# DEEPDIP-project/IncompressibleNavierStokes.jl

Measured on AMD Instinct MI355X. Metric: M lattice-cell updates/sec (RK4 step incl. Poisson), 3D TGV fp64, higher is better.
Workload: dtype f64; 1 GPU; TaylorGreenVortex3D 256^3 periodic fp64, RK44 + spectral Poisson, dt=0.001, Re=1e3; decomposition=single GPU, loop=timesteps_ (K steps, one native call)

## Files before the change

include/ins_hip.h:

```cpp
#ifndef INS_HIP_H
#define INS_HIP_H

#include <stdint.h>

#ifdef __cplusplus
extern "C" {
#endif

#define INS_OK 0
#define INS_ERR_INVALID (-1)
#define INS_ERR_HIP (-2)
#define INS_ERR_FFT (-3)
#define INS_ERR_UNSUPPORTED (-4)
#define INS_ERR_NOCONV (-5)
#define INS_ERR_COMM (-6)

#define INS_BC_PERIODIC 0
#define INS_BC_DIRICHLET 1
#define INS_BC_SYMMETRIC 2
#define INS_BC_PRESSURE 3
#define INS_BC_HALO 4

typedef struct ins_grid ins_grid_t;
typedef struct ins_poisson ins_poisson_t;
typedef struct ins_rk ins_rk_t;
typedef struct ins_poisson32 ins_poisson32_t;
typedef struct ins_rk32 ins_rk32_t;
typedef struct ins_comm ins_comm_t;

typedef struct ins_grid_desc {
  int32_t D;
  int32_t N[3];
  const double* dx[3];
  const double* dxu[3];
  const double* A1[3][3];
  const double* A2[3][3];
  int32_t iu_lo[3][3];
  int32_t iu_hi[3][3];
  int32_t ip_lo[3];
  int32_t ip_hi[3];
  int32_t bc[3][2];
  double bc_u[3][2][3];
} ins_grid_desc_t;

int ins_version(void);
int ins_fft_reset_count(void);
const char* ins_last_error(void);
int ins_set_option(const char* name, int64_t value);
int ins_get_option(const char* name, int64_t* value);
int ins_option_count(void);
const char* ins_option_name(int i);
int ins_set_device(int device);
int ins_sync(void* stream);

int ins_grid_create(const ins_grid_desc_t* desc, ins_grid_t** out);
int ins_grid_destroy(ins_grid_t* grid);
int ins_grid_is_uniform_exact(const ins_grid_t* grid);

int ins_apply_bc_u_f64(const ins_grid_t* grid, double* u, int dudt, const double* const* planes, void* stream);
int ins_apply_bc_p_f64(const ins_grid_t* grid, double* p, void* stream);

int ins_scalewithvolume_f64(const ins_grid_t* grid, double* p, void* stream);
int ins_divergence_f64(const ins_grid_t* grid, const double* u, double* div, void* stream);
int ins_pressuregradient_f64(const ins_grid_t* grid, const double* p, double* G, void* stream);
int ins_applypressure_f64(const ins_grid_t* grid, double* u, const double* p, void* stream);
int ins_laplacian_f64(const ins_grid_t* grid, const double* p, double* L, void* stream);
int ins_convection_f64(const ins_grid_t* grid, const double* u, double* F, void* stream);
int ins_diffusion_f64(const ins_grid_t* grid, double visc, const double* u, double* F, void* stream);
int ins_convectiondiffusion_f64(const ins_grid_t* grid, double visc, const double* u, double* F, void* stream);
int ins_momentum_f64(const ins_grid_t* grid, double visc, const double* u, double* F, void* stream);
int ins_kinetic_energy_f64(const ins_grid_t* grid, const double* u, double* ke, int interpolate_first, void* stream);
int ins_total_kinetic_energy_f64(const ins_grid_t* grid, const double* u, int interpolate_first, double* out, void* stream);
int ins_cfl_timestep_f64(const ins_grid_t* grid, double Re, const double* u, double* out, void* stream);
int ins_max_abs_divergence_f64(const ins_grid_t* grid, const double* u, double* out, void* stream);

int ins_poisson_spectral_create(const ins_grid_t* grid, ins_poisson_t** out);
int ins_poisson_cg_create(const ins_grid_t* grid, double abstol, double reltol, int64_t maxiter, ins_poisson_t** out);
int ins_poisson_cg_bordered(ins_poisson_t* ps, int enable);
int ins_poisson_cg_set_comm(ins_poisson_t* ps, ins_comm_t* comm);
int ins_poisson_fdm_create(const ins_grid_t* grid, const double* const* V, const double* const* lam, ins_poisson_t** out);
int ins_poisson_destroy(ins_poisson_t* ps);
int ins_poisson_fft_engine(const ins_poisson_t* ps, int32_t* engine);
int ins_poisson_yz_partitions(const ins_poisson_t* ps, int32_t* partitions);
int ins_poisson_solve_f64(ins_poisson_t* ps, double* p, void* stream);
int ins_poisson_last_info(const ins_poisson_t* ps, int64_t* iterations, double* residual);
int ins_project_f64(const ins_grid_t* grid, ins_poisson_t* ps, double* u, double* p, void* stream);

int ins_divergence_adjoint_f64(const ins_grid_t* grid, const double* phi, double* ubar, void* stream);
int ins_pressuregradient_adjoint_f64(const ins_grid_t* grid, const double* phi, double* pbar, void* stream);
int ins_convection_adjoint_f64(const ins_grid_t* grid, const double* u, const double* phibar, double* ubar, void* stream);
int ins_diffusion_adjoint_f64(const ins_grid_t* grid, double visc, const double* phibar, double* ubar, void* stream);
int ins_momentum_pullback_f64(const ins_grid_t* grid, double visc, const double* u, const double* phibar, double* ubar, int accumulate, void* stream);
int ins_apply_bc_u_pullback_f64(const ins_grid_t* grid, double* phibar, void* stream);
int ins_apply_bc_p_pullback_f64(const ins_grid_t* grid, double* phibar, void* stream);
int ins_project_pullback_f64(const ins_grid_t* grid, ins_poisson_t* ps, double* phibar, double* pwork, void* stream);

int ins_filter_face_f64(const ins_grid_t* les, const ins_grid_t* dns, int comp, const double* u, double* v, void* stream);
int ins_filter_volume_f64(const ins_grid_t* les, const ins_grid_t* dns, int comp, const double* u, double* v, void* stream);
int ins_reconstruct_f64(const ins_grid_t* dns, const ins_grid_t* les, int comp, const double* v, double* u, void* stream);
int ins_filter_face_pullback_f64(const ins_grid_t* les, const ins_grid_t* dns, int comp, const double* w, double* ubar, void* stream);
int ins_filter_volume_pullback_f64(const ins_grid_t* les, const ins_grid_t* dns, int comp, const double* w, double* ubar, void* stream);

int ins_rk_create(const ins_grid_t* grid, ins_poisson_t* ps, int nstage, const double* A, const double* c, ins_rk_t** out);
int ins_rk_destroy(ins_rk_t* rk);
int ins_rk_step_f64(ins_rk_t* rk, double visc, double* u, double t, double dt, const double* const* planes, void* stream);
int ins_rk_step_bc_f64(ins_rk_t* rk, double visc, double* u, double t, double dt, const double* const* planes_by_time, void* stream);
int ins_rk_steps_f64(ins_rk_t* rk, double visc, double* u, double t, double dt, int nsteps, void* stream);
int ins_combine_f64(const ins_grid_t* grid, const double* base, double* out, int nterms, const double* coefs,
                    const double* const* ks, void* stream);
int ins_rk_profile_enable(ins_rk_t* rk, int enable);
int ins_rk_profile_read(ins_rk_t* rk, double* momentum_ms, int64_t* momentum_launches);
int ins_rk_set_bodyforce(ins_rk_t* rk, const double* force);

int ins_dbg_stage_rhs_used(const ins_rk_t* rk, int64_t* launches);
int ins_dbg_stage_rhs(ins_rk_t* rk, double visc, const double* u_in, const double* pI, const double* ustart, const double* kterm, double coef_k,
                      double self_in, double coef_self, double* ustar, double* rhs, int32_t* used, void* stream);
int ins_dbg_stage_carry_used(const ins_rk_t* rk, int64_t* launches);
int ins_rk_pressure(const ins_rk_t* rk, double** p);
int ins_rk_stage_force(const ins_rk_t* rk, int i, double** ku);

int ins_vorticity_f64(const ins_grid_t* grid, const double* u, double* w, void* stream);
int ins_interpolate_u_p_f64(const ins_grid_t* grid, const double* u, double* up, void* stream);
int ins_interpolate_w_p_f64(const ins_grid_t* grid, const double* w, double* wp, void* stream);
int ins_dfield_f64(const ins_grid_t* grid, const double* p, double* G, double* d, double eps, void* stream);
int ins_qfield_f64(const ins_grid_t* grid, const double* u, double* Q, void* stream);
int ins_dissipation_from_strain_f64(const ins_grid_t* grid, double visc, const double* u, double* eps_out, void* stream);
int ins_eig2field_f64(const ins_grid_t* grid, const double* u, double* lam, void* stream);
int ins_apply_bc_temp_f64(const ins_grid_t* grid, const int32_t* bc, const double* val, const double* const* planes, double* temp, void* stream);
int ins_convection_diffusion_temp_f64(const ins_grid_t* grid, double a4, const double* u, const double* temp, double* c, void* stream);
int ins_dissipation_f64(const ins_grid_t* grid, double visc, double coef, const double* u, double* diff, double* diss, void* stream);
int ins_gravity_f64(const ins_grid_t* grid, int gdir, double a2, const double* temp, double* F, void* stream);
int ins_smagtensor_f64(const ins_grid_t* grid, double theta, const double* u, double* sigma, void* stream);
int ins_divoftensor_f64(const ins_grid_t* grid, const double* sigma, double* s, void* stream);
int ins_smagorinsky_force_f64(const ins_grid_t* grid, double theta, const double* u, double* sigma, double* s, void* stream);
int ins_smagorinsky_force_needs_sigma(const ins_grid_t* grid);
int ins_tensorbasis_f64(const ins_grid_t* grid, const double* u, double* B, double* V, void* stream);

int ins_tensorbasis_pullback_f64(const ins_grid_t* grid, const double* u, const double* Bbar, const double* Vbar, double* ubar, int accumulate,
                                 void* stream);
int ins_divoftensor_adjoint_f64(const ins_grid_t* grid, const double* sbar, double* sigmabar, void* stream);
int ins_tensorinvariants_f64(const ins_grid_t* grid, const double* u, double* V, void* stream);
int ins_tensorclosure_stress_f64(const ins_grid_t* grid, const double* u, const double* a, double* tau, void* stream);
int ins_tensorclosure_pullback_f64(const ins_grid_t* grid, const double* u, const double* a, const double* taubar, const double* Vbar, double* abar,
                                   double* ubar, int accumulate, void* stream);
int ins_combine_scalar_f64(const ins_grid_t* grid, const double* base, double* out, int nterms, const double* coefs,
                           const double* const* ks, void* stream);

typedef struct ins_temperature_desc {
  double a2;
  double a4;
  double diss_coef;
  int32_t gdir;
  int32_t dodissipation;
  int32_t bc[6];
  double val[6];
} ins_temperature_desc_t;
int ins_rk_set_temperature(ins_rk_t* rk, const ins_temperature_desc_t* desc);
int ins_rk_set_closure(ins_rk_t* rk, int32_t kind, double theta);
int ins_rk_step_ext_f64(ins_rk_t* rk, double visc, double* u, double* temp, double t, double dt, void* stream);

int ins_apply_bc_temp_pullback_f64(const ins_grid_t* grid, const int32_t* bc, double* tempbar, void* stream);
int ins_gravity_adjoint_f64(const ins_grid_t* grid, int gdir, double a2, const double* phibar, double* tempbar, void* stream);
int ins_convection_diffusion_temp_adjoint_f64(const ins_grid_t* grid, double a4, const double* u, const double* temp, const double* cbar,
                                              double* ubar, double* tempbar, void* stream);
int ins_dissipation_adjoint_f64(const ins_grid_t* grid, double visc, double coef, const double* u, const double* cbar, double* ubar, void* stream);
int ins_temperature_pullback_f64(const ins_grid_t* grid, const ins_temperature_desc_t* desc, double visc, const double* u, const double* temp,
                                 const double* Fbar, const double* cbar, double* ubar, double* tempbar, void* stream);

typedef struct ins_spectrum ins_spectrum_t;
int ins_spectrum_create(const ins_grid_t* grid, int nbin, const int64_t* offsets, const int64_t* inds, ins_spectrum_t** out);
int ins_spectrum_create_weighted(const ins_grid_t* grid, int nbin, const int64_t* offsets, const int64_t* inds, const double* weights,
                                 ins_spectrum_t** out);
int ins_spectrum_destroy(ins_spectrum_t* spectrum);
int ins_spectrum_f64(ins_spectrum_t* spectrum, const double* u, double* ehat, void* stream);

typedef struct ins_slab_fft ins_slab_fft_t;
int ins_stage_momentum_f64(const ins_grid_t* grid, double visc, const double* u_in, double* k_out, const double* ustart,
                           double* ustar, int nterms, const double* coefs, const double* const* ks, double coef_self, void* stream);
int ins_stage_momentum_corr_f64(const ins_grid_t* grid, double visc, const double* ustar_prev, const double* p_ext, double* k_out,
                                const double* ustart, double* ustar, int nterms, const double* coefs, const double* const* ks,
                                double coef_self, void* stream);
int ins_stage_momentum_corr_part_f64(const ins_grid_t* grid, double visc, const double* ustar_prev, const double* p_ext, double* k_out,
                                     const double* ustart, double* ustar, int nterms, const double* coefs, const double* const* ks,
                                     double coef_self, double c0m1, double self_in, double* ustart_out, int part, void* stream);
int ins_slab_divergence_f64(const ins_grid_t* grid, const double* u, double* pI, void* stream);
int ins_slab_applypressure_f64(const ins_grid_t* grid, double* u, const double* pI, const double* p_top, void* stream);
int ins_slab_fft_create(const int32_t np[3], const double h[3], int rank, int nranks, ins_slab_fft_t** out);
int ins_slab_fft_destroy(ins_slab_fft_t* fft);
int ins_slab_fft_sizes(const ins_slab_fft_t* fft, int64_t* real_elems, int64_t* complex_elems);
int ins_slab_fft_forward_xy(ins_slab_fft_t* fft, double* pI, double* work, double* sendbuf, void* stream);
int ins_slab_fft_solve_z(ins_slab_fft_t* fft, double* buf, void* stream);
int ins_slab_fft_inverse_xy(ins_slab_fft_t* fft, double* recvbuf, double* work, double* pI, void* stream);

int ins_slab_fft_can_chunk(const ins_slab_fft_t* fft);
int ins_slab_fft_xy_forward_only(ins_slab_fft_t* fft, double* pI, double* work, void* stream);
int ins_slab_fft_pack_chunk(ins_slab_fft_t* fft, double* work, double* sendbuf, int kx0, int kxc, void* stream);
int ins_slab_fft_solve_z_chunk(ins_slab_fft_t* fft, double* buf, int kx0, int kxc, void* stream);
int ins_slab_fft_unpack_chunk(ins_slab_fft_t* fft, double* recvbuf, double* work, int kx0, int kxc, void* stream);
int ins_slab_fft_xy_inverse_only(ins_slab_fft_t* fft, double* work, double* pI, void* stream);
int ins_slab_fft_is_own(const ins_slab_fft_t* fft);
int ins_slab_fft_forward_packed(ins_slab_fft_t* fft, const ins_grid_t* grid, const double* src, int from_u, double* work, double* sendbuf,
                                int cw, void* stream);
int ins_slab_fft_inverse_packed(ins_slab_fft_t* fft, double* recvbuf, double* work, double* pI, int cw, void* stream);

int ins_slab_ztri_edge_elems(const ins_slab_fft_t* S, int64_t* doubles);
int ins_slab_ztri_forward(ins_slab_fft_t* S, const ins_grid_t* grid, const double* src, int from_u, double* work, double* edge, void* stream);
int ins_slab_ztri_finish(ins_slab_fft_t* S, double* work, const double* edges_all, double* pI, void* stream);
int ins_slab_ztri_chunk(const ins_slab_fft_t* S, int c, int nchunks, int64_t* line_lo, int64_t* line_cnt, int64_t* edge_doubles);
int ins_slab_ztri_transform(ins_slab_fft_t* S, const ins_grid_t* grid, const double* src, int from_u, double* work, void* stream);
int ins_slab_ztri_sweep_forward(ins_slab_fft_t* S, double* work, double* edge, int c, int nchunks, void* stream);
int ins_slab_ztri_sweep_backward(ins_slab_fft_t* S, double* work, const double* edges_all, int c, int nchunks, void* stream);
int ins_slab_ztri_inverse(ins_slab_fft_t* S, double* work, double* pI, void* stream);
int ins_slab_xfwd_planes(ins_slab_fft_t* S, const ins_grid_t* grid, const double* u, double* work, int kz0, int nkz, void* stream);

#define INS_COMM_ID_BYTES 128
int ins_comm_unique_id(void* id128);
int ins_comm_create(int nranks, int rank, const void* id128, ins_comm_t** out);
int ins_comm_create_local(int ngpu, const int* devices, ins_comm_t** out);
int ins_comm_group_begin(void);
int ins_comm_group_end(void);
int ins_comm_destroy(ins_comm_t* comm);
int ins_comm_rank(const ins_comm_t* comm, int* rank, int* nranks);
int ins_comm_sendrecv_f64(ins_comm_t* comm, int nsend, const double* const* sendbufs, const int64_t* sendcounts, const int32_t* dsts, int nrecv,
                          double* const* recvbufs, const int64_t* recvcounts, const int32_t* srcs, void* stream);
int ins_halo_exchange_f64(ins_comm_t* comm, const ins_grid_t* slab_grid, double* u, int comp_mask, int down_only, void* stream);
int ins_halo_exchange_scalar_f64(ins_comm_t* comm, const ins_grid_t* slab_grid, double* p, void* stream);
int ins_halo_exchange_p_f64(ins_comm_t* comm, double* p_ext, int64_t plane_elems, int nzl, void* stream);
int ins_ztri_allgather_f64(ins_comm_t* comm, const double* edge, double* edges_all, int64_t count, int direct, void* stream);
int ins_comm_allreduce_f64(ins_comm_t* comm, double* buf, int64_t count, int op, void* stream);
int ins_comm_alltoall_f64(ins_comm_t* comm, const double* send, double* recv, int64_t count, void* stream);

int ins_apply_bc_u_f32(const ins_grid_t* grid, float* u, void* stream);
int ins_apply_bc_p_f32(const ins_grid_t* grid, float* p, void* stream);
int ins_momentum_f32(const ins_grid_t* grid, float visc, const float* u, float* F, void* stream);
int ins_poisson_spectral_create_f32(const ins_grid_t* grid, ins_poisson32_t** out);
int ins_poisson_wrap_f32(const ins_grid_t* grid, ins_poisson_t* ps64, ins_poisson32_t** out);
int ins_poisson_destroy_f32(ins_poisson32_t* ps);
int ins_poisson_solve_f32(ins_poisson32_t* ps, float* p, void* stream);
int ins_project_f32(const ins_grid_t* grid, ins_poisson32_t* ps, float* u, float* p, void* stream);
int ins_rk_create_f32(const ins_grid_t* grid, ins_poisson32_t* ps, int nstage, const double* A, const double* c, ins_rk32_t** out);
int ins_rk_destroy_f32(ins_rk32_t* rk);
int ins_rk_step_f32(ins_rk32_t* rk, float visc, float* u, float dt, void* stream);
int ins_rk_steps_f32(ins_rk32_t* rk, float visc, float* u, float dt, int nsteps, void* stream);
int ins_max_abs_divergence_f32(const ins_grid_t* grid, ins_poisson32_t* ps, const float* u, float* out, void* stream);

int ins_divergence_adjoint_f32(const ins_grid_t* grid, const float* phi, float* ubar, void* stream);
int ins_pressuregradient_adjoint_f32(const ins_grid_t* grid, const float* phi, float* pbar, void* stream);
int ins_momentum_pullback_f32(const ins_grid_t* grid, float visc, const float* u, const float* phibar, float* ubar, int accumulate, void* stream);
int ins_apply_bc_u_pullback_f32(const ins_grid_t* grid, float* phibar, void* stream);
int ins_apply_bc_p_pullback_f32(const ins_grid_t* grid, float* phibar, void* stream);
int ins_project_pullback_f32(const ins_grid_t* grid, ins_poisson32_t* ps, float* phibar, float* pwork, void* stream);

int ins_tensorinvariants_f32(const ins_grid_t* grid, const float* u, float* V, void* stream);
int ins_tensorclosure_stress_f32(const ins_grid_t* grid, const float* u, const float* a, float* tau, void* stream);
int ins_tensorclosure_pullback_f32(const ins_grid_t* grid, const float* u, const float* a, const float* taubar, const float* Vbar, float* abar,
                                   float* ubar, int accumulate, void* stream);
int ins_divoftensor_f32(const ins_grid_t* grid, const float* sigma, float* s, void* stream);
int ins_divoftensor_adjoint_f32(const ins_grid_t* grid, const float* sbar, float* sigmabar, void* stream);

int ins_apply_bc_temp_f32(const ins_grid_t* grid, const int32_t* bc, const float* val, float* temp, void* stream);
int ins_convection_diffusion_temp_f32(const ins_grid_t* grid, float a4, const float* u, const float* temp, float* c, void* stream);
int ins_dissipation_f32(const ins_grid_t* grid, float visc, float coef, const float* u, float* diff, float* diss, void* stream);
int ins_gravity_f32(const ins_grid_t* grid, int gdir, float a2, const float* temp, float* F, void* stream);
int ins_rk_set_temperature_f32(ins_rk32_t* rk, const ins_temperature_desc_t* desc);
int ins_rk_step_ext_f32(ins_rk32_t* rk, float visc, float* u, float* temp, float dt, void* stream);
int ins_rk_steps_ext_f32(ins_rk32_t* rk, float visc, float* u, float* temp, float dt, int nsteps, void* stream);

#ifdef __cplusplus
}
// ... 3 lines not shown
```

incompressiblenavierstokes.jl_amd/_lib.py:

```python
import ctypes as C
import os

_HERE = os.path.dirname(os.path.abspath(__file__))
LIB_PATH = os.environ.get("INS_HIP_LIB") or os.path.join(_HERE, "libinship.so")

INS_BC_PERIODIC, INS_BC_DIRICHLET, INS_BC_SYMMETRIC, INS_BC_PRESSURE, INS_BC_HALO = range(5)

c_double_p = C.POINTER(C.c_double)
vp = C.c_void_p


class GridDesc(C.Structure):

    _fields_ = [
        ("D", C.c_int32),
        ("N", C.c_int32 * 3),
        ("dx", c_double_p * 3),
        ("dxu", c_double_p * 3),
        ("A1", (c_double_p * 3) * 3),
        ("A2", (c_double_p * 3) * 3),
        ("iu_lo", (C.c_int32 * 3) * 3),
        ("iu_hi", (C.c_int32 * 3) * 3),
        ("ip_lo", C.c_int32 * 3),
        ("ip_hi", C.c_int32 * 3),
        ("bc", (C.c_int32 * 2) * 3),
        ("bc_u", ((C.c_double * 3) * 2) * 3),
    ]


SIGNATURES = {
    "ins_version": (C.c_int, []),
    "ins_fft_reset_count": (C.c_int, []),
    "ins_last_error": (C.c_char_p, []),
    "ins_set_option": (C.c_int, [C.c_char_p, C.c_int64]),
    "ins_get_option": (C.c_int, [C.c_char_p, C.POINTER(C.c_int64)]),
    "ins_option_count": (C.c_int, []),
    "ins_option_name": (C.c_char_p, [C.c_int]),
    "ins_set_device": (C.c_int, [C.c_int]),
    "ins_sync": (C.c_int, [vp]),
    "ins_grid_create": (C.c_int, [C.POINTER(GridDesc), C.POINTER(vp)]),
    "ins_grid_destroy": (C.c_int, [vp]),
    "ins_grid_is_uniform_exact": (C.c_int, [vp]),
    "ins_apply_bc_u_f64": (C.c_int, [vp, vp, C.c_int, C.POINTER(vp), vp]),
    "ins_apply_bc_p_f64": (C.c_int, [vp, vp, vp]),
    "ins_scalewithvolume_f64": (C.c_int, [vp, vp, vp]),
    "ins_divergence_f64": (C.c_int, [vp, vp, vp, vp]),
    "ins_pressuregradient_f64": (C.c_int, [vp, vp, vp, vp]),
    "ins_applypressure_f64": (C.c_int, [vp, vp, vp, vp]),
    "ins_laplacian_f64": (C.c_int, [vp, vp, vp, vp]),
    "ins_convection_f64": (C.c_int, [vp, vp, vp, vp]),
    "ins_diffusion_f64": (C.c_int, [vp, C.c_double, vp, vp, vp]),
    "ins_convectiondiffusion_f64": (C.c_int, [vp, C.c_double, vp, vp, vp]),
    "ins_momentum_f64": (C.c_int, [vp, C.c_double, vp, vp, vp]),
    "ins_kinetic_energy_f64": (C.c_int, [vp, vp, vp, C.c_int, vp]),
    "ins_total_kinetic_energy_f64": (C.c_int, [vp, vp, C.c_int, c_double_p, vp]),
    "ins_cfl_timestep_f64": (C.c_int, [vp, C.c_double, vp, c_double_p, vp]),
    "ins_max_abs_divergence_f64": (C.c_int, [vp, vp, c_double_p, vp]),
    "ins_vorticity_f64": (C.c_int, [vp, vp, vp, vp]),
    "ins_interpolate_u_p_f64": (C.c_int, [vp, vp, vp, vp]),
    "ins_interpolate_w_p_f64": (C.c_int, [vp, vp, vp, vp]),
    "ins_dfield_f64": (C.c_int, [vp, vp, vp, vp, C.c_double, vp]),
    "ins_qfield_f64": (C.c_int, [vp, vp, vp, vp]),
    "ins_dissipation_from_strain_f64": (C.c_int, [vp, C.c_double, vp, vp, vp]),
    "ins_eig2field_f64": (C.c_int, [vp, vp, vp, vp]),
    "ins_apply_bc_temp_f64": (C.c_int, [vp, C.POINTER(C.c_int32), c_double_p, C.POINTER(vp), vp, vp]),
    "ins_convection_diffusion_temp_f64": (C.c_int, [vp, C.c_double, vp, vp, vp, vp]),
    "ins_dissipation_f64": (C.c_int, [vp, C.c_double, C.c_double, vp, vp, vp, vp]),
    "ins_gravity_f64": (C.c_int, [vp, C.c_int, C.c_double, vp, vp, vp]),
    "ins_smagtensor_f64": (C.c_int, [vp, C.c_double, vp, vp, vp]),
    "ins_divoftensor_f64": (C.c_int, [vp, vp, vp, vp]),
    "ins_smagorinsky_force_f64": (C.c_int, [vp, C.c_double, vp, vp, vp, vp]),
    "ins_smagorinsky_force_needs_sigma": (C.c_int, [vp]),
    "ins_tensorbasis_f64": (C.c_int, [vp, vp, vp, vp, vp]),
    "ins_combine_scalar_f64": (C.c_int, [vp, vp, vp, C.c_int, c_double_p, C.POINTER(vp), vp]),
    "ins_spectrum_create": (C.c_int, [vp, C.c_int, C.POINTER(C.c_int64), C.POINTER(C.c_int64), C.POINTER(vp)]),
    "ins_spectrum_create_weighted": (C.c_int, [vp, C.c_int, C.POINTER(C.c_int64), C.POINTER(C.c_int64), c_double_p, C.POINTER(vp)]),
    "ins_spectrum_destroy": (C.c_int, [vp]),
    "ins_spectrum_f64": (C.c_int, [vp, vp, vp, vp]),
    "ins_poisson_spectral_create": (C.c_int, [vp, C.POINTER(vp)]),
    "ins_poisson_cg_create": (C.c_int, [vp, C.c_double, C.c_double, C.c_int64, C.POINTER(vp)]),
    "ins_poisson_cg_bordered": (C.c_int, [vp, C.c_int]),
    "ins_poisson_cg_set_comm": (C.c_int, [vp, vp]),
    "ins_poisson_fdm_create": (C.c_int, [vp, C.POINTER(c_double_p), C.POINTER(c_double_p), C.POINTER(vp)]),
    "ins_poisson_destroy": (C.c_int, [vp]),
    "ins_poisson_fft_engine": (C.c_int, [vp, C.POINTER(C.c_int32)]),
    "ins_poisson_yz_partitions": (C.c_int, [vp, C.POINTER(C.c_int32)]),
    "ins_poisson_solve_f64": (C.c_int, [vp, vp, vp]),
    "ins_poisson_last_info": (C.c_int, [vp, C.POINTER(C.c_int64), c_double_p]),
    "ins_project_f64": (C.c_int, [vp, vp, vp, vp, vp]),
    "ins_divergence_adjoint_f64": (C.c_int, [vp, vp, vp, vp]),
    "ins_pressuregradient_adjoint_f64": (C.c_int, [vp, vp, vp, vp]),
    "ins_convection_adjoint_f64": (C.c_int, [vp, vp, vp, vp, vp]),
    "ins_diffusion_adjoint_f64": (C.c_int, [vp, C.c_double, vp, vp, vp]),
    "ins_momentum_pullback_f64": (C.c_int, [vp, C.c_double, vp, vp, vp, C.c_int, vp]),
    "ins_apply_bc_u_pullback_f64": (C.c_int, [vp, vp, vp]),
    "ins_apply_bc_p_pullback_f64": (C.c_int, [vp, vp, vp]),
    "ins_project_pullback_f64": (C.c_int, [vp, vp, vp, vp, vp]),
    "ins_tensorbasis_pullback_f64": (C.c_int, [vp, vp, vp, vp, vp, C.c_int, vp]),
    "ins_divoftensor_adjoint_f64": (C.c_int, [vp, vp, vp, vp]),
    "ins_tensorinvariants_f64": (C.c_int, [vp, vp, vp, vp]),
    "ins_tensorclosure_stress_f64": (C.c_int, [vp, vp, vp, vp, vp]),
    "ins_tensorclosure_pullback_f64": (C.c_int, [vp, vp, vp, vp, vp, vp, vp, C.c_int, vp]),
    "ins_apply_bc_temp_pullback_f64": (C.c_int, [vp, C.POINTER(C.c_int32), vp, vp]),
    "ins_gravity_adjoint_f64": (C.c_int, [vp, C.c_int, C.c_double, vp, vp, vp]),
    "ins_convection_diffusion_temp_adjoint_f64": (C.c_int, [vp, C.c_double, vp, vp, vp, vp, vp, vp]),
    "ins_dissipation_adjoint_f64": (C.c_int, [vp, C.c_double, C.c_double, vp, vp, vp, vp]),
    "ins_temperature_pullback_f64": (C.c_int, [vp, vp, C.c_double, vp, vp, vp, vp, vp, vp, vp]),
    "ins_filter_face_f64": (C.c_int, [vp, vp, C.c_int, vp, vp, vp]),
    "ins_filter_volume_f64": (C.c_int, [vp, vp, C.c_int, vp, vp, vp]),
    "ins_reconstruct_f64": (C.c_int, [vp, vp, C.c_int, vp, vp, vp]),
    "ins_filter_face_pullback_f64": (C.c_int, [vp, vp, C.c_int, vp, vp, vp]),
    "ins_filter_volume_pullback_f64": (C.c_int, [vp, vp, C.c_int, vp, vp, vp]),
    "ins_rk_create": (C.c_int, [vp, vp, C.c_int, c_double_p, c_double_p, C.POINTER(vp)]),
    "ins_rk_destroy": (C.c_int, [vp]),
    "ins_rk_step_f64": (C.c_int, [vp, C.c_double, vp, C.c_double, C.c_double, C.POINTER(vp), vp]),
    "ins_rk_step_bc_f64": (C.c_int, [vp, C.c_double, vp, C.c_double, C.c_double, C.POINTER(vp), vp]),
    "ins_rk_steps_f64": (C.c_int, [vp, C.c_double, vp, C.c_double, C.c_double, C.c_int, vp]),
    "ins_combine_f64": (C.c_int, [vp, vp, vp, C.c_int, c_double_p, C.POINTER(vp), vp]),
    "ins_rk_profile_enable": (C.c_int, [vp, C.c_int]),
    "ins_rk_profile_read": (C.c_int, [vp, c_double_p, C.POINTER(C.c_int64)]),
    "ins_rk_set_bodyforce": (C.c_int, [vp, vp]),
    "ins_dbg_stage_rhs_used": (C.c_int, [vp, C.POINTER(C.c_int64)]),
    "ins_dbg_stage_carry_used": (C.c_int, [vp, C.POINTER(C.c_int64)]),
    "ins_dbg_stage_rhs": (C.c_int, [vp, C.c_double, vp, vp, vp, vp, C.c_double, C.c_double, C.c_double, vp, vp, C.POINTER(C.c_int32), vp]),
    "ins_rk_pressure": (C.c_int, [vp, C.POINTER(vp)]),
    "ins_rk_stage_force": (C.c_int, [vp, C.c_int, C.POINTER(vp)]),
    "ins_rk_set_temperature": (C.c_int, [vp, vp]),
    "ins_rk_set_closure": (C.c_int, [vp, C.c_int32, C.c_double]),
    "ins_rk_step_ext_f64": (C.c_int, [vp, C.c_double, vp, vp, C.c_double, C.c_double, vp]),
    "ins_stage_momentum_f64": (C.c_int, [vp, C.c_double, vp, vp, vp, vp, C.c_int, c_double_p, C.POINTER(vp), C.c_double, vp]),
    "ins_stage_momentum_corr_f64": (C.c_int, [vp, C.c_double, vp, vp, vp, vp, vp, C.c_int, c_double_p, C.POINTER(vp), C.c_double, vp]),
    "ins_stage_momentum_corr_part_f64": (C.c_int, [vp, C.c_double, vp, vp, vp, vp, vp, C.c_int, c_double_p, C.POINTER(vp), C.c_double, C.c_double, C.c_double, vp, C.c_int, vp]),
    "ins_slab_divergence_f64": (C.c_int, [vp, vp, vp, vp]),
    "ins_slab_applypressure_f64": (C.c_int, [vp, vp, vp, vp, vp]),
    "ins_slab_fft_create": (C.c_int, [C.POINTER(C.c_int32), c_double_p, C.c_int, C.c_int, C.POINTER(vp)]),
    "ins_slab_fft_destroy": (C.c_int, [vp]),
    "ins_slab_fft_sizes": (C.c_int, [vp, C.POINTER(C.c_int64), C.POINTER(C.c_int64)]),
    "ins_slab_fft_forward_xy": (C.c_int, [vp, vp, vp, vp, vp]),
    "ins_slab_fft_solve_z": (C.c_int, [vp, vp, vp]),
    "ins_slab_fft_inverse_xy": (C.c_int, [vp, vp, vp, vp, vp]),
    "ins_slab_fft_can_chunk": (C.c_int, [vp]),
    "ins_slab_fft_xy_forward_only": (C.c_int, [vp, vp, vp, vp]),
    "ins_slab_fft_pack_chunk": (C.c_int, [vp, vp, vp, C.c_int, C.c_int, vp]),
    "ins_slab_fft_solve_z_chunk": (C.c_int, [vp, vp, C.c_int, C.c_int, vp]),
    "ins_slab_fft_unpack_chunk": (C.c_int, [vp, vp, vp, C.c_int, C.c_int, vp]),
    "ins_slab_fft_xy_inverse_only": (C.c_int, [vp, vp, vp, vp]),
    "ins_slab_fft_is_own": (C.c_int, [vp]),
    "ins_slab_ztri_edge_elems": (C.c_int, [vp, C.POINTER(C.c_int64)]),
    "ins_slab_ztri_forward": (C.c_int, [vp, vp, vp, C.c_int, vp, vp, vp]),
    "ins_slab_ztri_finish": (C.c_int, [vp, vp, vp, vp, vp]),
    "ins_slab_xfwd_planes": (C.c_int, [vp, vp, vp, vp, C.c_int, C.c_int, vp]),
    "ins_slab_ztri_chunk": (C.c_int, [vp, C.c_int, C.c_int, C.POINTER(C.c_int64), C.POINTER(C.c_int64), C.POINTER(C.c_int64)]),
    "ins_slab_ztri_transform": (C.c_int, [vp, vp, vp, C.c_int, vp, vp]),
    "ins_slab_ztri_sweep_forward": (C.c_int, [vp, vp, vp, C.c_int, C.c_int, vp]),
    "ins_slab_ztri_sweep_backward": (C.c_int, [vp, vp, vp, C.c_int, C.c_int, vp]),
    "ins_slab_ztri_inverse": (C.c_int, [vp, vp, vp, vp]),
    "ins_slab_fft_forward_packed": (C.c_int, [vp, vp, vp, C.c_int, vp, vp, C.c_int, vp]),
    "ins_slab_fft_inverse_packed": (C.c_int, [vp, vp, vp, vp, C.c_int, vp]),
    "ins_apply_bc_u_f32": (C.c_int, [vp, vp, vp]),
    "ins_apply_bc_p_f32": (C.c_int, [vp, vp, vp]),
    "ins_momentum_f32": (C.c_int, [vp, C.c_float, vp, vp, vp]),
    "ins_poisson_spectral_create_f32": (C.c_int, [vp, C.POINTER(vp)]),
    "ins_poisson_wrap_f32": (C.c_int, [vp, vp, C.POINTER(vp)]),
    "ins_poisson_destroy_f32": (C.c_int, [vp]),
    "ins_poisson_solve_f32": (C.c_int, [vp, vp, vp]),
    "ins_project_f32": (C.c_int, [vp, vp, vp, vp, vp]),
    "ins_rk_create_f32": (C.c_int, [vp, vp, C.c_int, c_double_p, c_double_p, C.POINTER(vp)]),
    "ins_rk_destroy_f32": (C.c_int, [vp]),
    "ins_rk_step_f32": (C.c_int, [vp, C.c_float, vp, C.c_float, vp]),
    "ins_rk_steps_f32": (C.c_int, [vp, C.c_float, vp, C.c_float, C.c_int, vp]),
    "ins_max_abs_divergence_f32": (C.c_int, [vp, vp, vp, C.POINTER(C.c_float), vp]),
    "ins_divergence_adjoint_f32": (C.c_int, [vp, vp, vp, vp]),
    "ins_pressuregradient_adjoint_f32": (C.c_int, [vp, vp, vp, vp]),
    "ins_momentum_pullback_f32": (C.c_int, [vp, C.c_float, vp, vp, vp, C.c_int, vp]),
    "ins_apply_bc_u_pullback_f32": (C.c_int, [vp, vp, vp]),
    "ins_apply_bc_p_pullback_f32": (C.c_int, [vp, vp, vp]),
    "ins_project_pullback_f32": (C.c_int, [vp, vp, vp, vp, vp]),
    "ins_tensorinvariants_f32": (C.c_int, [vp, vp, vp, vp]),
    "ins_tensorclosure_stress_f32": (C.c_int, [vp, vp, vp, vp, vp]),
    "ins_tensorclosure_pullback_f32": (C.c_int, [vp, vp, vp, vp, vp, vp, vp, C.c_int, vp]),
    "ins_divoftensor_f32": (C.c_int, [vp, vp, vp, vp]),
    "ins_divoftensor_adjoint_f32": (C.c_int, [vp, vp, vp, vp]),
    "ins_apply_bc_temp_f32": (C.c_int, [vp, vp, vp, vp, vp]),
    "ins_convection_diffusion_temp_f32": (C.c_int, [vp, C.c_float, vp, vp, vp, vp]),
    "ins_dissipation_f32": (C.c_int, [vp, C.c_float, C.c_float, vp, vp, vp, vp]),
    "ins_gravity_f32": (C.c_int, [vp, C.c_int, C.c_float, vp, vp, vp]),
    "ins_rk_set_temperature_f32": (C.c_int, [vp, vp]),
    "ins_rk_step_ext_f32": (C.c_int, [vp, C.c_float, vp, vp, C.c_float, vp]),
    "ins_rk_steps_ext_f32": (C.c_int, [vp, C.c_float, vp, vp, C.c_float, C.c_int, vp]),
    "ins_comm_unique_id": (C.c_int, [vp]),
    "ins_comm_create": (C.c_int, [C.c_int, C.c_int, vp, C.POINTER(vp)]),
    "ins_comm_create_local": (C.c_int, [C.c_int, C.POINTER(C.c_int), C.POINTER(vp)]),
    "ins_comm_group_begin": (C.c_int, []),
    "ins_comm_group_end": (C.c_int, []),
    "ins_comm_destroy": (C.c_int, [vp]),
    "ins_comm_rank": (C.c_int, [vp, C.POINTER(C.c_int), C.POINTER(C.c_int)]),
    "ins_comm_sendrecv_f64": (C.c_int, [vp, C.c_int, C.POINTER(vp), C.POINTER(C.c_int64), C.POINTER(C.c_int32), C.c_int, C.POINTER(vp),
                                        C.POINTER(C.c_int64), C.POINTER(C.c_int32), vp]),
    "ins_halo_exchange_f64": (C.c_int, [vp, vp, vp, C.c_int, C.c_int, vp]),
    "ins_halo_exchange_scalar_f64": (C.c_int, [vp, vp, vp, vp]),
    "ins_halo_exchange_p_f64": (C.c_int, [vp, vp, C.c_int64, C.c_int, vp]),
    "ins_ztri_allgather_f64": (C.c_int, [vp, vp, vp, C.c_int64, C.c_int, vp]),
    "ins_comm_allreduce_f64": (C.c_int, [vp, vp, C.c_int64, C.c_int, vp]),
    "ins_comm_alltoall_f64": (C.c_int, [vp, vp, vp, C.c_int64, vp]),
}

_lib = None


class INSHipError(RuntimeError):
    pass


def load():
    global _lib
    if _lib is not None:
        return _lib
    if not os.path.exists(LIB_PATH):
        raise INSHipError(
            f"{LIB_PATH} not found: build it with `python -c 'import __graft_entry__ as g; g.build()'` "
            "(or `make -C incompressiblenavierstokes.jl_amd/csrc`).  There is no CPU fallback."
        )
    lib = C.CDLL(LIB_PATH, mode=C.RTLD_GLOBAL)
    for name, (res, args) in SIGNATURES.items():
        fn = getattr(lib, name)
        fn.restype = res
        fn.argtypes = args
    _lib = lib
    return lib


def check(rc):
    if rc != 0:
        msg = load().ins_last_error()
        raise INSHipError(f"libinship error {rc}: {msg.decode() if msg else ''}")


def call(name, *args):
    check(getattr(load(), name)(*args))


def set_option(name, value):
    call("ins_set_option", name.encode(), int(value))


def get_option(name):
    v = C.c_int64()
    call("ins_get_option", name.encode(), C.byref(v))
    return int(v.value)


class options:

    def __init__(self, **kw):
        self.kw = kw

    def __enter__(self):
        self.old = {k: get_option(k) for k in self.kw}
        for k, v in self.kw.items():
            set_option(k, v)
        return self

    def __exit__(self, *exc):
        for k, v in self.old.items():
            set_option(k, v)
        return False


_fft_resets_seen = 0


def sync_fft_plan_caches():
    global _fft_resets_seen
    n = load().ins_fft_reset_count()
    if n != _fft_resets_seen:
        _fft_resets_seen = n
        import torch
# ... 4 lines not shown
```

incompressiblenavierstokes.jl_amd/csrc/ins_flux64.hip:

```cpp
#include <algorithm>
#include <cstdlib>
#include <cstring>

#include "ins_internal.h"
#include "ins_wave64.h"
#include "ins_flux_common.h"

namespace {

template <typename T, int R>
struct Plane {
  T v[3][R + 2];
  T h[3];
  T raw[3][R];
  T vm2;
  T rawv0;
};

template <typename T, int R>
struct TExt {
  T t[R + 2];
  T th;
  T vm1;
};

template <typename T, int R, int XW, bool FUSE, int CORR, bool SKEL = false, int NW = 4, bool EXTRA = false, bool RHS = false, bool CARRY = false>
__global__ __launch_bounds__(64 * NW, NW == 16 ? 4 : 2) void k_flux64(FluxArgs a) {
  static_assert(!RHS || (FUSE && CORR <= 1 && !SKEL && !EXTRA), "right-hand side in the stage kernel: fused epilogue, periodic box, no extra terms");
  static_assert(!CARRY || (FUSE && CORR == 1 && !SKEL && !EXTRA && NW <= 8 && sizeof(T) == 8), "carried combination: the fp64 periodic correcting stage kernel");
  constexpr unsigned EB = (unsigned)sizeof(T);
  const T* const a_u = static_cast<const T*>(a.u);
  const T* const a_pI = static_cast<const T*>(a.pI);
  T* const a_F = static_cast<T*>(a.F);
  static_assert(R + 2 + (CORR ? 1 : 0) <= 8, "packed halo rows live in 8-lane groups");
  int txi, tyi, tzi;
  {
    const int nty_local = (a.nty + 7) >> 3;
    int seq = (int)(blockIdx.x >> 3);
    if (seq >= a.ntx * nty_local * a.ntz) return;
    txi = seq % a.ntx;
    seq /= a.ntx;
    tyi = (int)(blockIdx.x & 7) * nty_local + seq % nty_local;
    tzi = seq / nty_local;
    if (tyi >= a.nty) return;
  }
  __shared__ T rhs_lds_s[RHS ? 2 * NW * R : 1];
  T* const rhs_lds = rhs_lds_s;
  const int lane = threadIdx.x;
  const int wave = __builtin_amdgcn_readfirstlane(threadIdx.y);
  const int wx = wave % XW, wy = wave / XW;
  const int N0 = a.N0, N1 = a.N1, N2 = a.N2;
  const int n0 = N0 - 2, n1 = N1 - 2, n2 = N2 - 2;
  const int x0 = (txi * XW + wx) * 64;
  const int jb0 = (tyi * (NW / XW) + wy) * R;
  const int k0 = a.kB ? (tzi ? a.kB : a.k_lo) : a.k_lo + tzi * a.zc;
  const int k1 = a.kB ? k0 + a.zc : min(k0 + a.zc, a.k_hi);
  const int kw0 = RHS ? k0 - 1 : k0;
  if (x0 >= n0 || jb0 >= n1) {
    if (a.bar || RHS)
      for (int k = kw0; k < k1; ++k) __builtin_amdgcn_s_barrier();
    return;
  }
  const long long sz = (long long)N0 * N1;
  const int ci = x0 + lane;
  const bool xout = ci < n0;
  const DirT<T> X(a.X), Y(a.Y), Z(a.Z);

  auto prow_of = [&](int jr) { return CORR ? wrapi(jr, n1) + 1 : min(jr + 1, N1 - 1); };
  auto pcol_of = [&](int c) { return CORR ? wrapi(c, n0) + 1 : min(c + 1, N0 - 1); };

  unsigned urow[R + 2];
  unsigned qrow[R + 3];
#pragma unroll
  for (int rr = 0; rr < R + 2; ++rr) urow[rr] = (unsigned)(prow_of(jb0 - 1 + rr) * N0) * EB;
  if (CORR) {
#pragma unroll
    for (int rr = 0; rr < R + 3; ++rr) qrow[rr] = (unsigned)((prow_of(jb0 - 1 + rr) - 1) * n0) * EB;
  }
  const unsigned ubytes = (unsigned)sz * EB, qbytes = (unsigned)(n0 * n1) * EB;
  const unsigned urowm2 = (unsigned)((wrapi(jb0 - 2, n1) + 1) * N0) * EB, qrowm2 = (unsigned)(wrapi(jb0 - 2, n1) * n0) * EB;
  const unsigned orowm1 = (unsigned)((wrapi(jb0 - 1, n1) + 1) * N0) * EB;
  const unsigned ucol = (unsigned)pcol_of(ci) * EB;
  const unsigned qcol = CORR ? (unsigned)(pcol_of(ci) - 1) * EB : 0u;
  unsigned uhoff, qhoff = 0;
  {
    const int r = lane & 7, grp = (lane >> 3) & 3;
    const int ru = r <= R + 1 ? r : 0;
    const int colu = (grp == 2) ? pcol_of(x0 + 64) : ((EXTRA && grp == 1) ? pcol_of(x0 - 2) : pcol_of(x0 - 1));
    uhoff = (unsigned)(prow_of(jb0 - 1 + ru) * N0 + colu) * EB;
    if (CORR) {
      const int rq = r <= R + 2 ? r : 0;
      const int cq = grp == 0 ? x0 - 1 : (grp == 1 ? x0 : (grp == 2 ? x0 + 64 : x0 + 65));
      qhoff = (unsigned)((prow_of(jb0 - 1 + rq) - 1) * n0 + (pcol_of(cq) - 1)) * EB;
    }
  }

  auto uplane = [&](int kk) {
    return CORR == 1 ? wrapi(kk - 1, n2) + 1 : (CORR == 2 ? min(kk, N2 - 1) : ((RHS && kk < 0) ? kk + n2 : kk));
  };
  auto load_plane = [&](Plane<T, R>& P, int kk) {
    const T* base = a_u + (long long)uplane(kk) * sz;
#pragma unroll
    for (int c = 0; c < 3; ++c) {
      const rsrc_t rs = plane_rsrc(base + c * a.sc, ubytes);
#pragma unroll
      for (int rr = 0; rr < R + 2; ++rr) P.v[c][rr] = ldb<T>(rs, ucol, urow[rr]);
      P.h[c] = ldb<T>(rs, uhoff, 0);
      if (RHS && c == 1) P.vm2 = ldb<T>(rs, ucol, urowm2);
    }
  };
  const unsigned urowm1 = (unsigned)(prow_of(jb0 - 2) * N0) * EB;
  auto load_text = [&](TExt<T, R>& E, int kk) {
    const long long po = (long long)uplane(kk) * sz;
    const rsrc_t rt = plane_rsrc(static_cast<const T*>((const void*)a.te.temp) + po, ubytes);
#pragma unroll
    for (int rr = 0; rr < R + 2; ++rr) E.t[rr] = ldb<T>(rt, ucol, urow[rr]);
    E.th = ldb<T>(rt, uhoff, 0);
    E.vm1 = ldb<T>(plane_rsrc(a_u + po + a.sc, ubytes), ucol, urowm1);
  };
  constexpr int NPR = R + 3 + (RHS ? 1 : 0);
  auto load_p = [&](T (&P)[NPR], T& PH, int kk) {
    const rsrc_t rs = plane_rsrc(a_pI + (long long)(CORR == 2 ? min(kk, N2) : wrapi(kk - 1, n2)) * n0 * n1, qbytes);
#pragma unroll
    for (int rr = 0; rr < R + 3; ++rr) P[rr] = ldb<T>(rs, qcol, qrow[rr]);
    PH = ldb<T>(rs, qhoff, 0);
    if constexpr (RHS) P[R + 3] = ldb<T>(rs, qcol, qrowm2);
  };
  auto correct = [&](Plane<T, R>& P, const T (&Pc)[NPR], T PHc, const T (&Pn)[NPR], T PHn) {
    if (CARRY || a.epi.self_in != 0.0) {
#pragma unroll
      for (int c = 0; c < 3; ++c)
#pragma unroll
        for (int rr = 0; rr < R; ++rr) P.raw[c][rr] = P.v[c][rr + 1];
      if constexpr (RHS) P.rawv0 = P.v[1][0];
    }
    if constexpr (RHS) P.vm2 -= (Pc[0] - Pc[R + 3]) * Y.gs;
#pragma unroll
    for (int rr = 0; rr < R + 2; ++rr) {
      const T pc = Pc[rr];
      P.v[0][rr] -= (next_h(pc, rdlane(PHc, 16 + rr)) - pc) * X.gs;
      P.v[1][rr] -= (Pc[rr + 1] - pc) * Y.gs;
      P.v[2][rr] -= (Pn[rr] - pc) * Z.gs;
    }
    P.h[0] -= (dpp_old<0x108>(PHc, PHc) - PHc) * X.gs;
    P.h[1] -= (dpp_old<0x101>(PHc, PHc) - PHc) * Y.gs;
    P.h[2] -= (PHn - PHc) * Z.gs;
  };

  T zprev[3][R];
  T zprevV0 = 0;
  T wsprev[R] = {};
  auto zflux0 = [&](const Plane<T, R>& C, const Plane<T, R>& Nx) {
    if constexpr (RHS) zprevV0 = flux(C.v[1][0], Nx.v[1][0], C.v[2][0], C.v[2][1], Z.vo);
#pragma unroll
    for (int rr = 1; rr <= R; ++rr) {
      const T Wc = C.v[2][rr];
      zprev[0][rr - 1] = flux(C.v[0][rr], Nx.v[0][rr], Wc, next_h(Wc, rdlane(C.h[2], 16 + rr)), Z.vo);
      zprev[1][rr - 1] = flux(C.v[1][rr], Nx.v[1][rr], Wc, C.v[2][rr + 1], Z.vo);
      zprev[2][rr - 1] = flux(Wc, Nx.v[2][rr], Wc, Nx.v[2][rr], Z.vs);
    }
  };

  unsigned orow[R];
#pragma unroll
  for (int rr = 0; rr < R; ++rr) orow[rr] = (unsigned)((min(jb0 + rr, n1 - 1) + 1) * N0) * EB;
  const unsigned ocol = (unsigned)(min(ci, n0 - 1) + 1) * EB;

  T eacc[3][EXTRA ? R : 1];
  T gacc[EXTRA ? R : 1];
  T Pz[3][EXTRA ? R : 1];
  const T nux = X.vs * X.rs, nuy = Y.vs * Y.rs, nuz = Z.vs * Z.rs;
  T sV0 = 0;
  auto epi_load = [&](const Plane<T, R>& C, int k, T (&sacc)[3][R]) {
    const long long pk = (long long)((RHS && k < 1) ? k + n2 : k) * sz;
    if constexpr (EXTRA) {
      if (a.epi.extra) {
        const T* b = static_cast<const T*>((const void*)a.epi.extra) + pk;
#pragma unroll
        for (int c = 0; c < 3; ++c) {
          const rsrc_t rs = plane_rsrc(b + c * a.sc, ubytes);
#pragma unroll
          for (int rr = 0; rr < R; ++rr) eacc[c][rr] = ldb<T>(rs, ocol, orow[rr]);
        }
      } else {
#pragma unroll
        for (int c = 0; c < 3; ++c)
#pragma unroll
          for (int rr = 0; rr < R; ++rr) eacc[c][rr] = 0;
      }
      if (a.epi.gtemp) {
        const T* tb = static_cast<const T*>((const void*)a.epi.gtemp) + pk;
        const int gd = a.epi.gdir;
        const rsrc_t r0 = plane_rsrc(tb, ubytes), r1 = plane_rsrc(gd == 2 ? tb + sz : tb, ubytes);
        const unsigned dcol = gd == 0 ? EB : 0u, drow = gd == 1 ? (unsigned)N0 * EB : 0u;
#pragma unroll
        for (int rr = 0; rr < R; ++rr) gacc[rr] = (T)a.epi.ga2 * ((T)0.5 * (ldb<T>(r0, ocol, orow[rr]) + ldb<T>(r1, ocol + dcol, orow[rr] + drow)));
      }
    }
    const bool ntl = (a.nt & 8) != 0;
    if (a.epi.ustart) {
      const T* b = static_cast<const T*>((const void*)a.epi.ustart) + pk;
      const T c0 = (T)(1.0 + a.epi.c0m1);
#pragma unroll
      for (int c = 0; c < 3; ++c) {
        const rsrc_t rs = plane_rsrc(b + c * a.sc, ubytes);
#pragma unroll
        for (int rr = 0; rr < R; ++rr) sacc[c][rr] = c0 * (ntl ? ldb_aux<2>(rs, ocol, orow[rr], (T)0) : ldb<T>(rs, ocol, orow[rr]));
        if (RHS && c == 1) sV0 = c0 * ldb<T>(rs, ocol, orowm1);
      }
    } else {
#pragma unroll
      for (int c = 0; c < 3; ++c)
#pragma unroll
        for (int rr = 0; rr < R; ++rr) sacc[c][rr] = C.v[c][rr + 1];
      if constexpr (RHS) sV0 = C.v[1][0];
    }
    if (a.epi.self_in != 0.0) {
#pragma unroll
      for (int c = 0; c < 3; ++c)
#pragma unroll
        for (int rr = 0; rr < R; ++rr) sacc[c][rr] += (T)a.epi.self_in * (CORR ? C.raw[c][rr] : C.v[c][rr + 1]);
      if constexpr (RHS) sV0 += (T)a.epi.self_in * (CORR ? C.rawv0 : C.v[1][0]);
    }
    for (int q = 0; q < a.epi.n; ++q) {
      const T* kq = static_cast<const T*>((const void*)a.epi.k[q]) + pk;
      const T cq = (T)a.epi.coef[q];
#pragma unroll
      for (int c = 0; c < 3; ++c) {
        const rsrc_t rs = plane_rsrc(kq + c * a.sc, ubytes);
        T kv[R];
#pragma unroll
        for (int rr = 0; rr < R; ++rr) kv[rr] = ntl ? ldb_aux<2>(rs, ocol, orow[rr], (T)0) : ldb<T>(rs, ocol, orow[rr]);
#pragma unroll
        for (int rr = 0; rr < R; ++rr) sacc[c][rr] += cq * kv[rr];
        if (RHS && c == 1) sV0 += cq * ldb<T>(rs, ocol, orowm1);
      }
    }
  };
  auto st3 = [&](T* o, unsigned co, unsigned rowb, T v0, T v1, T v2) {
    const rsrc_t r0 = plane_rsrc(o, ubytes), r1 = plane_rsrc(o + a.sc, ubytes), r2 = plane_rsrc(o + 2 * a.sc, ubytes);
    const int snt = a.nt & 7;
    if (snt == 0) {
      stb(r0, co, rowb, v0);
      stb(r1, co, rowb, v1);
      stb(r2, co, rowb, v2);
    } else if (snt == 1) {
      stb_aux<2>(r0, co, rowb, v0);
      stb_aux<2>(r1, co, rowb, v1);
      stb_aux<2>(r2, co, rowb, v2);
    } else if (snt == 2) {
      stb_aux<17>(r0, co, rowb, v0);
      stb_aux<17>(r1, co, rowb, v1);
      stb_aux<17>(r2, co, rowb, v2);
    } else {
      stb_aux<19>(r0, co, rowb, v0);
      stb_aux<19>(r1, co, rowb, v1);
      stb_aux<19>(r2, co, rowb, v2);
    }
  };
  auto emit = [&](int rr, int k, T fu, T fv, T fw, T s0, T s1, T s2, bool st) {
    const long long pk = (long long)k * sz;
    if constexpr (EXTRA) {
      fu += eacc[0][rr - 1];
      fv += eacc[1][rr - 1];
      fw += eacc[2][rr - 1];
      if (a.epi.gtemp) {
        const T gv = gacc[rr - 1];
        if (a.epi.gdir == 0) fu += gv;
        if (a.epi.gdir == 1) fv += gv;
        if (a.epi.gdir == 2) fw += gv;
      }
    }
    const int j = jb0 + rr - 1;
    if (xout && j < n1 && st) {
      const unsigned rowb = orow[rr - 1], co = ocol;
      if (FUSE) {
        if (CORR && a.epi.ustart_out) {
          T* w = static_cast<T*>((void*)a.epi.ustart_out) + pk;
          stb(plane_rsrc(w, ubytes), co, rowb, s0);
          stb(plane_rsrc(w + a.sc, ubytes), co, rowb, s1);
          stb(plane_rsrc(w + 2 * a.sc, ubytes), co, rowb, s2);
        }
        T* o = static_cast<T*>((void*)a.epi.ustar) + pk;
        st3(o, co, rowb, s0 + (T)a.epi.coef_self * fu, s1 + (T)a.epi.coef_self * fv, s2 + (T)a.epi.coef_self * fw);
      }
      if (!FUSE || a.epi.write_k) st3(a_F + pk, co, rowb, fu, fv, fw);
    }
  };

  constexpr bool TMK = EXTRA && CORR == 0;
  T Tz[TMK ? R : 1];
  T wwprev[TMK ? R : 1];
  T PzV0 = 0;
  T hU_prev = 0;
  auto body = [&](Plane<T, R>& C, const Plane<T, R>& Nx, TExt<T, R>& CT, const TExt<T, R>& NT, int k, int kload, bool st_) {
    const bool st = RHS ? st_ : true;
    const T* nb = a_u + (long long)uplane(kload) * sz;
    const rsrc_t n0r = plane_rsrc(nb, ubytes), n1r = plane_rsrc(nb + a.sc, ubytes), n2r = plane_rsrc(nb + 2 * a.sc, ubytes);
    const T ch0 = C.h[0], ch1 = C.h[1], ch2 = C.h[2];
    T sacc[3][R];
    if (FUSE) epi_load(C, k, sacc);
    const bool tm = TMK && a.tm;
    const rsrc_t ntr = plane_rsrc(static_cast<const T*>((const void*)a.te.temp) + (long long)uplane(kload) * sz, ubytes);
    T tacc[TMK ? R : 1];
    const T cth = CT.th;
    if constexpr (TMK) {
      if (tm) {
        const long long pk = (long long)k * sz;
        const rsrc_t rs0 = plane_rsrc(static_cast<const T*>((const void*)a.te.tempstart) + pk, ubytes);
#pragma unroll
        for (int rr = 0; rr < R; ++rr) tacc[rr] = ldb<T>(rs0, ocol, orow[rr]);
        for (int q = 0; q < a.te.n; ++q) {
          const rsrc_t rq = plane_rsrc(static_cast<const T*>((const void*)a.te.k[q]) + pk, ubytes);
#pragma unroll
          for (int rr = 0; rr < R; ++rr) tacc[rr] += (T)a.te.coef[q] * ldb<T>(rq, ocol, orow[rr]);
        }
      }
    }
    T fyu_o = 0, fyv_o = 0, fyw_o = 0;
    T Uo = 0, Vo = 0, Wo = 0;
    T To = 0, wv_o = 0;
    T us_u[RHS ? R : 1], dvs[RHS ? R : 1], dws[RHS ? R : 1];
    T vs_o = 0;
    T cvm2 = 0;
    if constexpr (RHS) cvm2 = C.vm2;
#pragma unroll
    for (int rr = 0; rr <= R; ++rr) {
      const T Uc = C.v[0][rr], Vc = C.v[1][rr], Wc = C.v[2][rr];
      if (SKEL) {
        if (rr >= 1) {
          const T fu = Uc + fyu_o + C.v[0][rr + 1] + Nx.v[0][rr] + zprev[0][rr - 1] + ch0;
          const T fv = Vc + fyv_o + C.v[1][rr + 1] + Nx.v[1][rr] + zprev[1][rr - 1] + ch1;
          const T fw = Wc + fyw_o + C.v[2][rr + 1] + Nx.v[2][rr] + zprev[2][rr - 1] + ch2;
          emit(rr, k, fu, fv, fw, FUSE ? sacc[0][rr - 1] : (T)0, FUSE ? sacc[1][rr - 1] : (T)0, FUSE ? sacc[2][rr - 1] : (T)0, st);
        }
        fyu_o = Uc;
        fyv_o = Vc;
        fyw_o = Wc;
        C.v[0][rr] = ldb<T>(n0r, ucol, urow[rr]);
        C.v[1][rr] = ldb<T>(n1r, ucol, urow[rr]);
        C.v[2][rr] = ldb<T>(n2r, ucol, urow[rr]);
        continue;
      }
      const T Vn = next_h(Vc, rdlane(ch1, 16 + rr));
      const T fyu = flux(Uc, C.v[0][rr + 1], Vc, Vn, Y.vo);
      const T fyv = flux(Vc, C.v[1][rr + 1], Vc, C.v[1][rr + 1], Y.vs);
      const T fyw = flux(Wc, C.v[2][rr + 1], Vc, Nx.v[1][rr], Y.vo);
      if (rr >= 1) {
        const T Un = next_h(Uc, rdlane(ch0, 16 + rr)), Wn = next_h(Wc, rdlane(ch2, 16 + rr));
        const T fxu = flux(Uc, Un, Uc, Un, X.vs);
        const T fxv = flux(Vc, Vn, Uc, C.v[0][rr + 1], X.vo);
        const T fxw = flux(Wc, Wn, Uc, Nx.v[0][rr], X.vo);
        const T sU = rdlane(ch0, rr), sV = rdlane(ch1, rr), sW = rdlane(ch2, rr);
        const T sUu = rdlane(ch0, rr + 1), sUn = rdlane(Nx.h[0], rr);
        const T lxu = flux(sU, Uc, sU, Uc, X.vs);
        const T lxv = flux(sV, Vc, sU, sUu, X.vo);
        const T lxw = flux(sW, Wc, sU, sUn, X.vo);
        T fu = (fxu - prev_h(fxu, lxu)) * X.rs;
        T fv = (fxv - prev_h(fxv, lxv)) * X.ro;
        T fw = (fxw - prev_h(fxw, lxw)) * X.ro;
        fu += (fyu - fyu_o) * Y.ro;
        fv += (fyv - fyv_o) * Y.rs;
        fw += (fyw - fyw_o) * Y.ro;
        const T zu = flux(Uc, Nx.v[0][rr], Wc, Wn, Z.vo);
        const T zv = flux(Vc, Nx.v[1][rr], Wc, C.v[2][rr + 1], Z.vo);
        const T zw = flux(Wc, Nx.v[2][rr], Wc, Nx.v[2][rr], Z.vs);
        fu += (zu - zprev[0][rr - 1]) * Z.ro;
        fv += (zv - zprev[1][rr - 1]) * Z.ro;
        fw += (zw - zprev[2][rr - 1]) * Z.rs;
        zprev[0][rr - 1] = zu;
        zprev[1][rr - 1] = zv;
        zprev[2][rr - 1] = zw;
        if constexpr (EXTRA) {
          if (a.epi.wout || tm) {
            const T Up = prev_h(Uc, sU), Vp = prev_h(Vc, sV), Wp = prev_h(Wc, sW);
            const T wu = Uc * ((Un + Up - 2 * Uc) * nux + (C.v[0][rr + 1] + Uo - 2 * Uc) * nuy + (Nx.v[0][rr] + Pz[0][rr - 1] - 2 * Uc) * nuz);
            const T wv = Vc * ((Vn + Vp - 2 * Vc) * nux + (C.v[1][rr + 1] + Vo - 2 * Vc) * nuy + (Nx.v[1][rr] + Pz[1][rr - 1] - 2 * Vc) * nuz);
            const T ww = Wc * ((Wn + Wp - 2 * Wc) * nux + (C.v[2][rr + 1] + Wo - 2 * Wc) * nuy + (Nx.v[2][rr] + Pz[2][rr - 1] - 2 * Wc) * nuz);
            const int j = jb0 + rr - 1;
            if (a.epi.wout && xout && j < n1) {
              T* w = static_cast<T*>((void*)a.epi.wout) + (long long)k * sz;
              stb(plane_rsrc(w, ubytes), ocol, orow[rr - 1], wu);
              stb(plane_rsrc(w + a.sc, ubytes), ocol, orow[rr - 1], wv);
              stb(plane_rsrc(w + 2 * a.sc, ubytes), ocol, orow[rr - 1], ww);
            }
            if constexpr (TMK) if (tm) {
              T wuL = 0;
              if (x0 > 0) {
                const T U0 = rdlane(Uc, 0), Um2 = rdlane(ch0, 8 + rr), sUd = rdlane(ch0, rr - 1), sUp = rdlane(hU_prev, rr);
                wuL = sU * ((U0 + Um2 - 2 * sU) * nux + (sUu + sUd - 2 * sU) * nuy + (sUn + sUp - 2 * sU) * nuz);
              }
              const T dc = (T)a.te.dcoef;
              const T dd = dc * (prev_h(wu, wuL) + wu) / 2 + dc * (wv_o + wv) / 2 + dc * (wwprev[rr - 1] + ww) / 2;
              const T Tc = CT.t[rr];
              const T Txp = next_h(Tc, rdlane(cth, 16 + rr)), Txm = prev_h(Tc, rdlane(cth, rr));
              const T Typ = CT.t[rr + 1], Tym = To, Tzp = NT.t[rr], Tzm = Tz[rr - 1];
              const T a4 = (T)a.te.a4;
              T cd = (-(Uc * ((Tc + Txp) / 2) - Up * ((Txm + Tc) / 2)) + a4 * ((Txp - Tc) * X.gs - (Tc - Txm) * X.gs)) * X.gs;
              cd += (-(Vc * ((Tc + Typ) / 2) - Vo * ((Tym + Tc) / 2)) + a4 * ((Typ - Tc) * Y.gs - (Tc - Tym) * Y.gs)) * Y.gs;
              cd += (-(Wc * ((Tc + Tzp) / 2) - Pz[2][rr - 1] * ((Tzm + Tc) / 2)) + a4 * ((Tzp - Tc) * Z.gs - (Tc - Tzm) * Z.gs)) * Z.gs;
              const T kt = cd + dd;
              if (xout && j < n1) {
                const long long pk = (long long)k * sz;
                if (a.te.ktemp_out) stb(plane_rsrc(static_cast<T*>((void*)a.te.ktemp_out) + pk, ubytes), ocol, orow[rr - 1], kt);
                stb(plane_rsrc(static_cast<T*>((void*)a.te.temp_out) + pk, ubytes), ocol, orow[rr - 1], tacc[rr - 1] + (T)a.te.c_self * kt);
              }
              wv_o = wv;
              wwprev[rr - 1] = ww;
              Tz[rr - 1] = Tc;
            }
          }
          Pz[0][rr - 1] = Uc;
          Pz[1][rr - 1] = Vc;
          Pz[2][rr - 1] = Wc;
        }
        emit(rr, k, fu, fv, fw, FUSE ? sacc[0][rr - 1] : (T)0, FUSE ? sacc[1][rr - 1] : (T)0, FUSE ? sacc[2][rr - 1] : (T)0, st);
        if constexpr (CARRY) {
          if (xout && jb0 + rr - 1 < n1 && st) {
            const T ca0 = (T)a.epi.ca[0], ca1 = (T)a.epi.ca[1], ca2 = (T)a.epi.ca[2], cs = (T)a.epi.coef_self;
            const T s0 = sacc[0][rr - 1], s1 = sacc[1][rr - 1], s2 = sacc[2][rr - 1];
            st3(static_cast<T*>((void*)a.epi.carry_out) + (long long)k * sz, ocol, orow[rr - 1], ca0 * s0 + ca1 * C.raw[0][rr - 1] + ca2 * (s0 + cs * fu),
                ca0 * s1 + ca1 * C.raw[1][rr - 1] + ca2 * (s1 + cs * fv), ca0 * s2 + ca1 * C.raw[2][rr - 1] + ca2 * (s2 + cs * fw));
          }
        }
        if constexpr (RHS) {
          const T su = sacc[0][rr - 1] + (T)a.epi.coef_self * fu, sv = sacc[1][rr - 1] + (T)a.epi.coef_self * fv, sw = sacc[2][rr - 1] + (T)a.epi.coef_self * fw;
          us_u[rr - 1] = su;
          dvs[rr - 1] = sv - vs_o;
          dws[rr - 1] = sw - wsprev[rr - 1];
          vs_o = sv;
          wsprev[rr - 1] = sw;
          if (lane == 63) rhs_lds[((k & 1) * NW + wave) * R + rr - 1] = su;
        }
      } else if constexpr (RHS) {
        const T fyv_m = flux(cvm2, Vc, cvm2, Vc, Y.vs);
        const T fxv = flux(Vc, Vn, Uc, C.v[0][rr + 1], X.vo);
        const T lxv = flux(rdlane(ch1, rr), Vc, rdlane(ch0, rr), rdlane(ch0, rr + 1), X.vo);
        T fv = (fxv - prev_h(fxv, lxv)) * X.ro;
        fv += (fyv - fyv_m) * Y.rs;
        const T zv = flux(Vc, Nx.v[1][rr], Wc, C.v[2][rr + 1], Z.vo);
        fv += (zv - zprevV0) * Z.ro;
        zprevV0 = zv;
        vs_o = sV0 + (T)a.epi.coef_self * fv;
      }
      fyu_o = fyu;
      fyv_o = fyv;
      fyw_o = fyw;
      if constexpr (TMK) {
        if (tm) {
          if (rr == 0) {
            const T Vp = prev_h(Vc, rdlane(ch1, 0));
            wv_o = jb0 > 0 ? Vc * ((Vn + Vp - 2 * Vc) * nux + (C.v[1][1] + CT.vm1 - 2 * Vc) * nuy + (Nx.v[1][0] + PzV0 - 2 * Vc) * nuz) : (T)0;
            PzV0 = Vc;
          }
          To = CT.t[rr];
          CT.t[rr] = ldb<T>(ntr, ucol, urow[rr]);
        }
      }
      if constexpr (EXTRA) {
        Uo = Uc;
        Vo = Vc;
        Wo = Wc;
      }
      C.v[0][rr] = ldb<T>(n0r, ucol, urow[rr]);
      C.v[1][rr] = ldb<T>(n1r, ucol, urow[rr]);
      C.v[2][rr] = ldb<T>(n2r, ucol, urow[rr]);
    }
    C.v[0][R + 1] = ldb<T>(n0r, ucol, urow[R + 1]);
    C.v[1][R + 1] = ldb<T>(n1r, ucol, urow[R + 1]);
    C.v[2][R + 1] = ldb<T>(n2r, ucol, urow[R + 1]);
    C.h[0] = ldb<T>(n0r, uhoff, 0);
    C.h[1] = ldb<T>(n1r, uhoff, 0);
    C.h[2] = ldb<T>(n2r, uhoff, 0);
    if constexpr (RHS) {
      C.vm2 = ldb<T>(n1r, ucol, urowm2);
      __builtin_amdgcn_fence(__ATOMIC_RELEASE, "workgroup", "local");
      __builtin_amdgcn_s_barrier();
      __builtin_amdgcn_fence(__ATOMIC_ACQUIRE, "workgroup", "local");
      const int lw = wy * XW + (wx + XW - 1) % XW;
      T* ro = static_cast<T*>((void*)a.epi.rhs_out) + (long long)(k - 1) * n0 * n1;
      const rsrc_t rr_ = plane_rsrc(ro, qbytes);
      const T om = (T)a.om;
#pragma unroll
      for (int r = 0; r < R; ++r) {
        const T ul = rhs_lds[((k & 1) * NW + lw) * R + r];
        T d = 0;
        d += (us_u[r] - prev_h(us_u[r], ul)) * (T)a.rdiv[0];
        d += dvs[r] * (T)a.rdiv[1];
        d += dws[r] * (T)a.rdiv[2];
        if (st && xout && jb0 + r < n1) stb(rr_, (unsigned)min(ci, n0 - 1) * EB, (unsigned)(min(jb0 + r, n1 - 1) * n0) * EB, d * om);
      }
    }
    if constexpr (TMK) {
      if (tm) {
        hU_prev = ch0;
        CT.t[R + 1] = ldb<T>(ntr, ucol, urow[R + 1]);
        CT.th = ldb<T>(ntr, uhoff, 0);
        CT.vm1 = ldb<T>(n1r, ucol, urowm1);
      }
    }
  };

  Plane<T, R> P0, P1;
  TExt<T, R> TE0, TE1;
  if (!CORR) {
    load_plane(P0, kw0 - 1);
    load_plane(P1, kw0);
    zflux0(P0, P1);
    if constexpr (EXTRA) {
#pragma unroll
      for (int c = 0; c < 3; ++c)
#pragma unroll
        for (int rr = 0; rr < R; ++rr) Pz[c][rr] = P0.v[c][rr + 1];
      if (a.tm) {
        load_text(TE0, k0 - 1);
        load_text(TE1, k0);
        PzV0 = P0.v[1][0];
        hU_prev = P0.h[0];
        const rsrc_t rw = plane_rsrc(a_u + (long long)uplane(max(k0 - 2, 0)) * sz + 2 * a.sc, ubytes);
#pragma unroll
        for (int rr = 1; rr <= R; ++rr) {
          const T Wc = P0.v[2][rr], Wm2 = ldb<T>(rw, ucol, urow[rr]);
          const T Wn = next_h(Wc, rdlane(P0.h[2], 16 + rr)), Wp = prev_h(Wc, rdlane(P0.h[2], rr));
          wwprev[rr - 1] = k0 > 1 ? Wc * ((Wn + Wp - 2 * Wc) * nux + (P0.v[2][rr + 1] + P0.v[2][rr - 1] - 2 * Wc) * nuy + (P1.v[2][rr] + Wm2 - 2 * Wc) * nuz) : (T)0;
          Tz[rr - 1] = TE0.t[rr];
        }
      }
    }
    load_plane(P0, min(kw0 + 1, k1));
    if constexpr (EXTRA) {
      if (a.tm) load_text(TE0, min(k0 + 1, k1));
    }
    int k = kw0;
    while (true) {
      if (!RHS && a.bar) __builtin_amdgcn_s_barrier();
      body(P1, P0, TE1, TE0, k, min(k + 2, k1), k >= k0);
      if (++k >= k1) break;
      if (!RHS && a.bar) __builtin_amdgcn_s_barrier();
      body(P0, P1, TE0, TE1, k, min(k + 2, k1), k >= k0);
      if (++k >= k1) break;
    }
  } else {
    T Pa[NPR], Pb[NPR], Ha, Hb;
    load_p(Pa, Ha, kw0 - 1);
    load_p(Pb, Hb, kw0);
    load_plane(P0, kw0 - 1);
    load_plane(P1, kw0);
    correct(P0, Pa, Ha, Pb, Hb);
    load_p(Pa, Ha, kw0 + 1);
    correct(P1, Pb, Hb, Pa, Ha);
    zflux0(P0, P1);
    if constexpr (EXTRA) {
#pragma unroll
      for (int c = 0; c < 3; ++c)
#pragma unroll
        for (int rr = 0; rr < R; ++rr) Pz[c][rr] = P0.v[c][rr + 1];
    }
    load_plane(P0, min(kw0 + 1, k1));
    load_p(Pb, Hb, min(kw0 + 2, k1 + 1));
    int k = kw0;
    while (true) {
      if (!RHS && a.bar) __builtin_amdgcn_s_barrier();
      correct(P0, Pa, Ha, Pb, Hb);
      load_p(Pa, Ha, min(k + 3, k1 + 1));
      body(P1, P0, TE1, TE0, k, min(k + 2, k1), k >= k0);
      if (++k >= k1) break;
      if (!RHS && a.bar) __builtin_amdgcn_s_barrier();
      correct(P1, Pb, Hb, Pa, Ha);
      load_p(Pb, Hb, min(k + 3, k1 + 1));
      body(P0, P1, TE0, TE1, k, min(k + 2, k1), k >= k0);
      if (++k >= k1) break;
    }
  }
}

#define g_disable ((int)ins_opt(OPT_INS_DISABLE_FLUX64))
#define g_rows ((int)ins_opt(OPT_INS_FLUX64_ROWS))
#define g_rows_corr ((int)ins_opt(OPT_INS_FLUX64_ROWS_CORR))
#define g_zchunk ((int)ins_opt(OPT_INS_FLUX64_ZC))
#define g_zchunk_corr ((int)ins_opt(OPT_INS_FLUX64_ZC_CORR))
#define g_xw ((int)ins_opt(OPT_INS_FLUX64_XW))
#define g_lds ((int)ins_opt(OPT_INS_FLUX64_LDS))
#define g_skel ((int)ins_opt(OPT_INS_FLUX64_SKEL))

template <typename T, int R, int XW, bool FUSE, int NW>
int launch_range(const ins_grid* G, FluxArgs& a, int corr_mode, hipStream_t s) {
  const unsigned nb = (unsigned)(8LL * a.ntx * ((a.nty + 7) / 8) * a.ntz);
  if (nb == 0) return INS_OK;
  const dim3 block(64, NW, 1);
  if constexpr (NW <= 8 && R == 4 && sizeof(T) == 8) {
    if (g_skel && corr_mode == 0) {
      hipLaunchKernelGGL((k_flux64<T, R, XW, FUSE, 0, true, NW>), dim3(nb), block, (size_t)g_lds, s, a);
      INS_LAUNCH_CHECK();
      return INS_OK;
    }
  }
  if (a.tm && corr_mode != 0) {
    ins_set_error("temperature stage inside the stage kernel: no in-kernel pressure correction");
    return INS_ERR_UNSUPPORTED;
  }
  if (a.epi.extra || a.epi.gtemp || a.epi.wout || a.tm) {
    if constexpr (FUSE && R == 2 && NW == 4 && sizeof(T) == 8) {
      if (corr_mode == 0) {
        hipLaunchKernelGGL((k_flux64<T, R, XW, true, 0, false, NW, true>), dim3(nb), block, (size_t)g_lds, s, a);
        INS_LAUNCH_CHECK();
        return INS_OK;
      }
      if (corr_mode == 1) {
        hipLaunchKernelGGL((k_flux64<T, R, XW, true, 1, false, NW, true>), dim3(nb), block, (size_t)g_lds, s, a);
        INS_LAUNCH_CHECK();
        return INS_OK;
      }
    }
    ins_set_error("stage kernel with an extra force term: fp64, fused epilogue, 2 rows, 4 wavefronts, no slab correction");
    return INS_ERR_UNSUPPORTED;
  }
  if (corr_mode == 0)
    hipLaunchKernelGGL((k_flux64<T, R, XW, FUSE, 0, false, NW>), dim3(nb), block, (size_t)g_lds, s, a);
  else if constexpr (FUSE && R <= 5) {
    if (corr_mode == 1 && a.epi.carry_out) {
      if constexpr (R == 2 && NW <= 8 && sizeof(T) == 8) {
        hipLaunchKernelGGL((k_flux64<T, R, XW, true, 1, false, NW, false, false, true>), dim3(nb), block, (size_t)g_lds, s, a);
      } else {
        ins_set_error("stage kernel asked to carry a combination forward on a tile shape it does not do it for");
        return INS_ERR_UNSUPPORTED;
      }
    } else if (corr_mode == 1)
      hipLaunchKernelGGL((k_flux64<T, R, XW, true, 1, false, NW>), dim3(nb), block, (size_t)g_lds, s, a);
    else
      hipLaunchKernelGGL((k_flux64<T, R, XW, true, 2, false, NW>), dim3(nb), block, (size_t)g_lds, s, a);
  } else {
    ins_set_error("in-kernel pressure correction needs the fused epilogue and <= 5 rows per thread");
    return INS_ERR_UNSUPPORTED;
  }
  INS_LAUNCH_CHECK();
  return INS_OK;
}

constexpr int ZB = 4;
template <typename T, int R, int XW, bool FUSE, int NW = 4>
int launch(const ins_grid* G, FluxArgs& a, int corr_mode, int part, hipStream_t s) {
  const GridDev& g = G->g;
  a.ntx = cdiv(g.N[0] - 2, 64 * XW);
  a.nty = cdiv(g.N[1] - 2, (NW / XW) * R);
  const int nzl = g.N[2] - 2;
  a.k_lo = 1;
  a.k_hi = nzl + 1;
  a.kB = 0;
  if (part != 0 && nzl <= 2 * ZB) {
    if (part == 1) return INS_OK;
    part = 0;
  }
  if (part == 1) {
    a.k_lo = 1 + ZB;
    a.k_hi = nzl + 1 - ZB;
  } else if (part == 2) {
    a.zc = ZB;
    a.kB = nzl + 1 - ZB;
  }
  a.ntz = part == 2 ? 2 : cdiv(a.k_hi - a.k_lo, a.zc);
  return launch_range<T, R, XW, FUSE, NW>(G, a, corr_mode, s);
}

template <int R, int XW, int NW, int CORR, bool CARRY = false>
int launch_rhs(const ins_grid* G, FluxArgs& a, hipStream_t s) {
  const GridDev& g = G->g;
  a.ntx = 1;
  a.nty = cdiv(g.N[1] - 2, (NW / XW) * R);
  a.k_lo = 1;
  a.k_hi = g.N[2] - 1;
  a.kB = 0;
  a.ntz = cdiv(a.k_hi - a.k_lo, a.zc);
  const unsigned nb = (unsigned)(8LL * ((a.nty + 7) / 8) * a.ntz);
  hipLaunchKernelGGL((k_flux64<double, R, XW, true, CORR, false, NW, false, true, CARRY>), dim3(nb), dim3(64, NW, 1), 0, s, a);
  INS_LAUNCH_CHECK();
  return INS_OK;
}

}

extern "C" void ins_tune_flux64(int disable, int rows, int rows_corr, int zchunk, int xw, int skel, int burst_unused, int lds) {
  if (disable >= 0) ins_set_option("INS_DISABLE_FLUX64", disable);
  if (rows >= 0) ins_set_option("INS_FLUX64_ROWS", rows);
  if (rows_corr >= 0) ins_set_option("INS_FLUX64_ROWS_CORR", rows_corr);
  if (zchunk >= 0) ins_set_option("INS_FLUX64_ZC", zchunk);
  if (xw >= 0) ins_set_option("INS_FLUX64_XW", xw);
  if (skel >= 0) ins_set_option("INS_FLUX64_SKEL", skel);
  (void)burst_unused;
  if (lds >= 0) ins_set_option("INS_FLUX64_LDS", lds);
}

bool ins_flux64_supported(const ins_grid* G) {
  const GridDev& g = G->g;
  return !g_disable && g.D == 3 && G->all_dof && G->uniform_exact && g.N[0] - 2 >= 66 && g.N[1] - 2 >= 8 && g.N[2] - 2 >= 4;
}

struct TileShape {
  int xw, rows, nw, zc;
};
static TileShape tile_shape(const ins_grid* G, int corr_mode, bool f32, bool ext, bool rhs) {
  const GridDev& g = G->g;
  const int n2 = g.N[2] - 2;
  const int waves_x = cdiv(g.N[0] - 2, 64);
  const int xwo = (corr_mode && ins_opt(OPT_INS_FLUX64_XW_CORR)) ? (int)ins_opt(OPT_INS_FLUX64_XW_CORR) : g_xw;
  int xw = xwo ? xwo : (waves_x >= 8 ? 2 : (waves_x >= 4 ? 4 : (waves_x >= 2 ? 2 : 1)));
  if (!xwo)
    while (xw > 1 && cdiv(waves_x, xw) * xw > waves_x) xw >>= 1;
  const bool three = rhs && corr_mode == 1 && !xwo && waves_x == 3 && !ins_opt(OPT_INS_FLUX64_NW);
  if (three) xw = 3;
  int rows = corr_mode ? (g_rows_corr ? g_rows_corr : 2) : (g_rows ? g_rows : 4);
  rows = std::min(std::max(rows, 2), corr_mode ? 5 : 6);
  if (f32) rows = corr_mode ? (ins_opt(OPT_INS_F32_CORR_ROWS) == 4 ? 4 : 2) : 4;
  const int nwo = (int)ins_opt(OPT_INS_FLUX64_NW);
  const int zco = (corr_mode && g_zchunk_corr) ? g_zchunk_corr : g_zchunk;
  auto tiles = [&](int nw_, int zc_) {
    return (long long)cdiv(g.N[0] - 2, 64 * xw) * cdiv(g.N[1] - 2, (nw_ / xw) * rows) * cdiv(n2, zc_);
  };
  const long long mintiles = ins_opt(OPT_INS_FLUX64_MINTILES) > 0 ? ins_opt(OPT_INS_FLUX64_MINTILES) : 256;
  int nw = three ? 6 : (nwo == 16 ? 16 : (nwo == 8 ? 8 : (nwo == 4 ? 4 : 0)));
  int zc = zco;
  if (!nw) {
    nw = 4;
    if (xw <= 8 && !g_lds) {
      for (int z : {64}) {
        const int zt = zco ? zco : z;
        if (n2 >= zt && tiles(8, zt) >= mintiles) {
          nw = 8;
          zc = zt;
          break;
        }
      }
    }
  }
  if (!zc) {
    const bool small_plane = (long long)(g.N[0] - 2) * (g.N[1] - 2) <= 256LL * 256;
    zc = n2 >= 256 && small_plane ? 64 : (n2 >= 128 ? 32 : (n2 >= 64 ? 16 : (n2 >= 32 ? 8 : 4)));
    if (n2 < 256)
      while (zc > 4 && tiles(nw, zc) < 2 * mintiles) zc >>= 1;
  }
  if (rows != 2 && nw == 16) nw = 8;
  if (ext) {
    rows = 2;
    nw = 4;
    if (!zco) zc = n2 >= 128 ? 32 : (n2 >= 64 ? 16 : (n2 >= 32 ? 8 : 4));
  }
  return TileShape{xw, rows, nw, zc};
}

bool ins_flux128_supported(const ins_grid* G, const RkEpi* epi, int corr_mode, bool f32);
bool ins_flux64_stage_rhs_supported(const ins_grid* G, int corr_mode) {
  if (ins_opt(OPT_INS_DISABLE_STAGE_RHS) || corr_mode < 0 || corr_mode > 1 || !ins_flux64_supported(G) || g_skel || g_lds) return false;
  if (ins_flux128_supported(G, nullptr, corr_mode, false)) return false;
  const TileShape t = tile_shape(G, corr_mode, false, false, true);
  if (64 * t.xw != G->g.N[0] - 2) return false;
  if (corr_mode == 0) return t.rows == 4 && t.xw == 2 && t.nw == 4;
  return t.rows == 2 && ((t.xw == 3 && t.nw == 6) || ((t.xw == 2 || t.xw == 4) && (t.nw == 4 || t.nw == 8)));
}

bool ins_flux64_stage_carry_supported(const ins_grid* G) {
  if (ins_opt(OPT_INS_DISABLE_STAGE_CARRY) || !ins_flux64_supported(G) || g_skel) return false;
  if (ins_flux128_supported(G, nullptr, 1, false)) return false;
  const TileShape t = tile_shape(G, 1, false, false, false);
  return t.rows == 2 && t.nw <= 8;
}

template <typename T>
static int flux64_dispatch(const ins_grid* G, double visc, const T* u, T* F, const RkEpi* epi, const T* pI, int corr_mode, hipStream_t s, int part) {
  const GridDev& g = G->g;
  FluxArgs a;
  memset(&a, 0, sizeof(a));
  a.u = u;
  a.pI = pI;
  a.F = F;
  a.sc = g.sc;
  a.N0 = g.N[0];
  a.N1 = g.N[1];
  a.N2 = g.N[2];
  a.X = make_dir(G, 0, visc);
  a.Y = make_dir(G, 1, visc);
  a.Z = make_dir(G, 2, visc);
  if (epi) a.epi = *epi;
  if (epi && epi->tstage) {
    a.te = *epi->tstage;
    a.tm = 1;
    a.epi.tstage = nullptr;
  }
  const bool ext = epi && (epi->extra || epi->gtemp || epi->wout || epi->tstage);
  const bool want_rhs = epi && epi->rhs_out;
  const TileShape ts = tile_shape(G, corr_mode, sizeof(T) == 4, ext, want_rhs);
  const int xw = ts.xw, rows = ts.rows, nw = ts.nw, zc = ts.zc;
  constexpr bool F32 = sizeof(T) == 4;
  a.zc = zc;
  a.bar = ins_opt(OPT_INS_FLUX64_NOBAR) ? 0 : 1;
  {
    const long long o = ins_opt(OPT_INS_FLUX64_NT);
    a.nt = o == 0 ? ((epi && !F32) ? 9 : 0) : (o == 16 ? 0 : (int)o);
  }
#define INS_F64_CASE(RR, FUSE)                                                        \
  if constexpr (!F32 || RR == 2 || RR == 4) {                                         \
    if (rows == RR) {                                                                 \
      if constexpr (RR == 2 && !F32) {                                                \
        if (nw == 16) {                                                               \
          if (xw == 4) return launch<T, RR, 4, FUSE, 16>(G, a, corr_mode, part, s);   \
          if (xw == 2) return launch<T, RR, 2, FUSE, 16>(G, a, corr_mode, part, s);   \
          return launch<T, RR, 1, FUSE, 16>(G, a, corr_mode, part, s);                \
        }                                                                             \
      }                                                                               \
      if (nw >= 8) {                                                                  \
        if (xw == 4) return launch<T, RR, 4, FUSE, 8>(G, a, corr_mode, part, s);      \
        if (xw == 2) return launch<T, RR, 2, FUSE, 8>(G, a, corr_mode, part, s);      \
        return launch<T, RR, 1, FUSE, 8>(G, a, corr_mode, part, s);                   \
      }                                                                               \
      if (xw == 4) return launch<T, RR, 4, FUSE>(G, a, corr_mode, part, s);           \
      if (xw == 2) return launch<T, RR, 2, FUSE>(G, a, corr_mode, part, s);           \
      return launch<T, RR, 1, FUSE>(G, a, corr_mode, part, s);                        \
    }                                                                                 \
  }
  const bool carry = epi && epi->carry_out;
  if (carry) {
    if (ins_stage_carry_aliases(*epi, u) || ins_stage_out_aliases_input(*epi, u)) {
      ins_set_error("stage kernel asked to carry a combination forward into, or to store u* over, one of its inputs");
      return INS_ERR_INVALID;
    }
    if (F32 || corr_mode != 1 || part != 0 || !ins_flux64_stage_carry_supported(G)) {
      ins_set_error("stage kernel asked to carry a combination forward on a path that does not do it");
      return INS_ERR_UNSUPPORTED;
    }
  }
  if (want_rhs) {
    if (ins_stage_out_aliases_input(*epi, u)) {
      ins_set_error("stage kernel asked for the Poisson right-hand side while u* overwrites one of its inputs");
      return INS_ERR_INVALID;
    }
    if constexpr (!F32) {
      if (part == 0 && ins_flux64_stage_rhs_supported(G, corr_mode)) {
        a.rdiv[0] = 1.0 / G->desc.dx[0][1];
        a.rdiv[1] = 1.0 / G->desc.dx[1][1];
        a.rdiv[2] = 1.0 / G->desc.dx[2][1];
        a.om = G->desc.dx[0][1] * G->desc.dx[1][1] * G->desc.dx[2][1];
        if (corr_mode == 0) return launch_rhs<4, 2, 4, 0>(G, a, s);
        if (carry) {
          if (xw == 3) return launch_rhs<2, 3, 6, 1, true>(G, a, s);
          if (xw == 4) return nw == 8 ? launch_rhs<2, 4, 8, 1, true>(G, a, s) : launch_rhs<2, 4, 4, 1, true>(G, a, s);
          return nw == 8 ? launch_rhs<2, 2, 8, 1, true>(G, a, s) : launch_rhs<2, 2, 4, 1, true>(G, a, s);
        }
        if (xw == 3) return launch_rhs<2, 3, 6, 1>(G, a, s);
        if (xw == 4) return nw == 8 ? launch_rhs<2, 4, 8, 1>(G, a, s) : launch_rhs<2, 4, 4, 1>(G, a, s);
        return nw == 8 ? launch_rhs<2, 2, 8, 1>(G, a, s) : launch_rhs<2, 2, 4, 1>(G, a, s);
      }
    }
    ins_set_error("stage kernel asked for the Poisson right-hand side on a box or tile shape it does not write it for");
    return INS_ERR_UNSUPPORTED;
  }
  if (epi) {
    INS_F64_CASE(2, true)
    INS_F64_CASE(3, true)
    INS_F64_CASE(4, true)
    INS_F64_CASE(5, true)
    INS_F64_CASE(6, true)
  } else {
    INS_F64_CASE(2, false)
    INS_F64_CASE(3, false)
    INS_F64_CASE(4, false)
    INS_F64_CASE(5, false)
    INS_F64_CASE(6, false)
  }
#undef INS_F64_CASE
  return INS_ERR_INVALID;
}

bool ins_flux128_supported(const ins_grid* G, const RkEpi* epi, int corr_mode, bool f32);
int ins_k_flux128(const ins_grid* G, double visc, const double* u, double* F, const RkEpi* epi, const double* pI, int corr_mode, hipStream_t s, int part);
int ins_k_flux128_f32(const ins_grid* G, double visc, const float* u, float* F, const RkEpi* epi, const float* pI, int corr_mode, hipStream_t s, int part);

int ins_k_flux64(const ins_grid* G, double visc, const double* u, double* F, const RkEpi* epi, const double* pI, int corr_mode, hipStream_t s,
                 int part) {
  if (ins_flux128_supported(G, epi, corr_mode, false)) {
    if (epi && epi->carry_out) {
      ins_set_error("stage kernel asked to carry a combination forward on a path that does not do it");
      return INS_ERR_UNSUPPORTED;
    }
    return ins_k_flux128(G, visc, u, F, epi, pI, corr_mode, s, part);
  }
  return flux64_dispatch<double>(G, visc, u, F, epi, pI, corr_mode, s, part);
}
int ins_k_flux64_f32(const ins_grid* G, double visc, const float* u, float* F, const RkEpi* epi, const float* pI, int corr_mode, hipStream_t s,
                     int part) {
  if (ins_flux128_supported(G, epi, corr_mode, true) && !ins_opt(OPT_INS_F32_ONE_COLUMN)) return ins_k_flux128_f32(G, visc, u, F, epi, pI, corr_mode, s, part);
  return flux64_dispatch<float>(G, visc, u, F, epi, pI, corr_mode, s, part);
}
```

incompressiblenavierstokes.jl_amd/csrc/ins_internal.h:

```cpp
#pragma once

#include <hip/hip_runtime.h>
#include <hipfft/hipfft.h>

#include <cstdint>
#include <cstdio>
#include <cstring>
#include <string>
#include <vector>

#include "ins_hip.h"

#define INS_EPS 2.220446049250313e-16
#define INS_MAX_STAGES 16

void ins_set_error(const char* fmt, ...);

#define INS_HIP_TRY(expr)                                                                   \
  do {                                                                                      \
    hipError_t _e = (expr);                                                                 \
    if (_e != hipSuccess) {                                                                 \
      ins_set_error("%s:%d: %s -> %s", __FILE__, __LINE__, #expr, hipGetErrorString(_e));   \
      return INS_ERR_HIP;                                                                   \
    }                                                                                       \
  } while (0)

#define INS_FFT_TRY(expr)                                                         \
  do {                                                                            \
    hipfftResult _r = (expr);                                                     \
    if (_r != HIPFFT_SUCCESS) {                                                   \
      ins_set_error("%s:%d: %s -> hipfftResult %d", __FILE__, __LINE__, #expr, (int)_r); \
      return INS_ERR_FFT;                                                         \
    }                                                                             \
  } while (0)

#define INS_REQUIRE(cond, msg)                                        \
  do {                                                                \
    if (!(cond)) {                                                    \
      ins_set_error("%s:%d: %s (%s)", __FILE__, __LINE__, msg, #cond); \
      return INS_ERR_INVALID;                                         \
    }                                                                 \
  } while (0)

#define INS_LAUNCH_CHECK() INS_HIP_TRY(hipGetLastError())

#define INS_OPT_LIST(X)          \
  X(INS_DISABLE_FAST3D)          \
  X(INS_K1_LDS)                  \
  X(INS_FLUX_ROWS)               \
  X(INS_FLUX_ZC)                 \
  X(INS_FLUX_XW)                 \
  X(INS_FLUX_BAR)                \
  X(INS_FLUX64_62_FROM)          \
  X(INS_DISABLE_FLUX128)         \
  X(INS_DISABLE_YZ_FUSED)        \
  X(INS_YZ_FUSED)                \
  X(INS_YZ_SKEL)                 \
  X(INS_YZ_PARTITIONS)           \
  X(INS_F32_ONE_COLUMN)          \
  X(INS_FLUX128_CORR)            \
  X(INS_FLUX128_XW)              \
  X(INS_FLUX128_ROWS)            \
  X(INS_FLUX128_ROWS_CORR)       \
  X(INS_FLUX128_NW)              \
  X(INS_FLUX128_ZC)              \
  X(INS_DISABLE_FDM_ZDCT)        \
  X(INS_DISABLE_FDM_ZFFT)        \
  X(INS_DISABLE_FDM_XFFT)        \
  X(INS_DISABLE_FDM_XYFFT)       \
  X(INS_DISABLE_OWNFFT)          \
  X(INS_OWNFFT_POW2_ONLY)        \
  X(INS_FIELDS_NO_MARCH)         \
  X(INS_FIELDS_ROWS)             \
  X(INS_FIELDS_NOBAR)            \
  X(INS_FIELDS_ZC)               \
  X(INS_DISABLE_FLUX2D)          \
  X(INS_DISABLE_FLUX64M)         \
  X(INS_DISABLE_SMAGFORCE)       \
  X(INS_DISABLE_SMAGFORCE_GEN)   \
  X(INS_SMAGFORCE_FORCE_GEN)     \
  X(INS_SMAGFORCE_ZC)            \
  X(INS_SMAGFORCE_BAR)         \
  X(INS_FLUX64M_ZC)              \
  X(INS_FLUX64M_NOBAR)           \
  X(INS_FLUX64M_XW)              \
  X(INS_FLUX64M_ROWS)            \
  X(INS_FLUX64M_SKIP_FIRST)      \
  X(INS_DISABLE_FLUX64)          \
  X(INS_FLUX64_ROWS)             \
  X(INS_FLUX64_ROWS_CORR)        \
  X(INS_FLUX64_ZC)               \
  X(INS_FLUX64_ZC_CORR)          \
  X(INS_FLUX64_XW)               \
  X(INS_FLUX64_LDS)              \
  X(INS_FLUX64_SKEL)             \
  X(INS_FLUX64_NW)               \
  X(INS_FLUX64_NT)               \
  X(INS_FLUX64_NOBAR)            \
  X(INS_FLUX64_MINTILES)         \
  X(INS_FLUX64_XW_CORR)          \
  X(INS_UNIFORM_BITWISE)         \
  X(INS_PHAT_DENSE)              \
  X(INS_DISABLE_FDM_FUSED)       \
  X(INS_DISABLE_FDM_FOLD)        \
  X(INS_DISABLE_FDM_UNFOLD4)     \
  X(INS_DISABLE_FDM_FOLDFUSE)    \
  X(INS_DISABLE_INKERNEL_CORR)   \
  X(INS_DISABLE_STAGE_RHS)       \
  X(INS_DISABLE_STAGE_CARRY)     \
  X(INS_RK_KEEP_K)               \
  X(INS_DISABLE_EXT_FUSED)       \
  X(INS_EXT_TEMP_SPLIT)          \
  X(INS_DISABLE_FUSED_RK)        \
  X(INS_DISABLE_STEP_CHAIN)      \
  X(INS_DISABLE_STEP_GRAPH)      \
  X(INS_DISABLE_LINE3)           \
  X(INS_DISABLE_XYFUSED)         \
  X(INS_DISABLE_CORR2D)          \
  X(INS_SPECTRUM_ROCFFT)         \
  X(INS_X_SKEL)                  \
  X(INS_LINE3_TK)                \
  X(INS_LINE3_WGS)               \
  X(INS_STEP_GRAPH)              \
  X(INS_ZSOLVE_SKEL)             \
  X(INS_ZSOLVE_TK)               \
  X(INS_ZSOLVE_RADIX4)           \
  X(INS_ZSOLVE_NT)               \
  X(INS_ZSOLVE_WGS)              \
  X(INS_DISABLE_ZSOLVE)          \
  X(INS_ZTRI_SKEL)               \
  X(INS_CG_HOSTSYNC)             \
  X(INS_CG_BATCH)                \
  X(INS_F32_CORR_ROWS)           \
  X(INS_F32_FP64_SPECTRA)        \
  X(INS_F32_HIPFFT_PROJECT)      \
  X(INS_F32_SPLIT_GRADIENT)      \
  X(INS_DISABLE_TEMP32_STAGE)    \
  X(INS_FFT_ALLOW_RESET)         \
  X(INS_DISABLE_ADJ_TILED)     \
  X(INS_DISABLE_FILTER_TILED)
#define INS_OPT_ENUM(id) OPT_##id,
enum InsOptId { INS_OPT_LIST(INS_OPT_ENUM) INS_OPT_COUNT };
#undef INS_OPT_ENUM
long long ins_opt(int id);
long long ins_opt_epoch();

struct GridDev {
  int D;
  int N[3];
  long long sx[3];
  long long sc;
  const double* dx[3];
  const double* dxu[3];
  const double* rdx[3];
  const double* rdxu[3];
  const double* mdx[3];
  const double* mdxu[3];
  const double* A1[3][3];
  const double* A2[3][3];
  int iu_lo[3][3], iu_hi[3][3];
  int ip_lo[3], ip_hi[3];
  int bc[3][2];
  double bc_u[3][2][3];
};

struct ins_grid {
  ins_grid_desc_t desc;
  std::vector<double> host;
  double* dev = nullptr;
  size_t dev_count = 0;
  GridDev g;
  bool all_periodic = false;
  bool uniform = false;
  double h[3] = {0, 0, 0};
  long long ncell = 0;
  bool all_dof = false;
  bool uniform_exact = false;
  void* rec_dev = nullptr;
  double rec_visc = -1.0;
  void* rec_diff_dev = nullptr;
  double rec_diff_visc = -1.0;
  double* red_dev = nullptr;
  double* red_host = nullptr;
  double* gradbar_dev = nullptr;
  size_t gradbar_count = 0;
};

enum PoissonKind { POISSON_SPECTRAL = 0, POISSON_CG = 1, POISSON_FDM = 2 };

struct ins_fdm;
int ins_fdm_create(int D, const int n[3], const double* const V[3], const double* const lam[3], int singular, ins_fdm** out);
int ins_fdm_destroy(ins_fdm* F);
int ins_fdm_enable_zfft(ins_fdm* F, double hz, const double* lam_z_host);
int ins_fdm_enable_zdct(ins_fdm* F, double hz, const double* lam_z_host);
int ins_fdm_enable_xfft(ins_fdm* F, double hx, const double* lam_x_host);
int ins_fdm_enable_xyfft(ins_fdm* F, double hx, double hy, const double* lam_x_host, const double* lam_y_host);
int ins_fdm_solve(ins_fdm* F, hipStream_t s, const ins_grid* G = nullptr, const double* u = nullptr, bool folded_io = false);
int ins_fdm_fold_mask(const ins_fdm* F);
bool ins_fdm_takes_u(const ins_fdm* F);
double* ins_fdm_buffer(ins_fdm* F);
const double* ins_fdm_mean(ins_fdm* F);

enum SpectralRoute {
  ROUTE_ROCFFT = 0,
  ROUTE_ROCFFT_ZFUSED,
  ROUTE_OWN2D,
  ROUTE_OWN2D_ONE,
  ROUTE_OWN_LDS,
  ROUTE_OWN_LINE3,
  ROUTE_OWN_XY,
  ROUTE_OWN_YZ,
};
enum KyOrder { KY_NATURAL = 0, KY_DIGITREV, KY_LINE3 };

struct ins_poisson {
  PoissonKind kind;
  const ins_grid* grid;
  hipfftHandle plan_fwd = 0, plan_inv = 0;
  SpectralRoute route = ROUTE_ROCFFT;
  KyOrder ky_order = KY_NATURAL;
  double* pI = nullptr;
  double* rhs = nullptr;
  hipfftDoubleComplex* phat = nullptr;
  double* ahat[3] = {nullptr, nullptr, nullptr};
  int np[3] = {1, 1, 1};
  int kmax[3] = {1, 1, 1};
  void* work = nullptr;
  size_t work_bytes = 0;
  hipStream_t plan_stream = nullptr;
  int kxs = 0;
  double* tw = nullptr;
  double* tw_x = nullptr;
  double* tw_y = nullptr;
  int yz_P = 0;
  double* yz_scratch = nullptr;
  double abstol = 0, reltol = 0;
  long long maxiter = 0;
  double *r = nullptr, *L = nullptr, *q = nullptr, *dinv = nullptr;
  bool bordered = false;
  bool singular = true;
  long long ndof = 0;
  long long last_iter = 0;
  double last_res = 0;
  double* cg_scal = nullptr;
  double* cg_host = nullptr;
  struct ins_comm* comm = nullptr;
  ins_fdm* fdm = nullptr;
};

struct ins_rk_ext;
void ins_rk_ext_free(ins_rk_ext* e);
struct ins_rk {
  const ins_grid* grid;
  ins_poisson* ps;
  int nstage;
  std::vector<double> A, c;
  double* ustart = nullptr;
  std::vector<double*> ku;
  double* p = nullptr;
  double* ub[2] = {nullptr, nullptr};
  std::vector<double*> vb;
  const double* force = nullptr;
  ins_rk_ext* ext = nullptr;
  long long stage_carry_launches = 0;
  long long stage_rhs_launches = 0;
  bool profiling = false;
  std::vector<hipEvent_t> prof_events;
  void* step_graph = nullptr;
};

struct Rec {
  double vs, vo, a0, b0, a1, b1, a2, b2, rs, ro, pad[6];
};

struct RkEpi {
  int n;
  int write_k;
  double coef[INS_MAX_STAGES + 1];
  const double* k[INS_MAX_STAGES + 1];
  double coef_self;
  double self_in;
  double c0m1;
  const double* ustart;
  double* ustar;
  double* ustart_out;
  double* carry_out;
  double ca[3];
  double* rhs_out;
  const double* extra;
  const double* gtemp;
  double ga2;
  int gdir;
  double* wout;
  const struct TempEpi* tstage;
};

static inline bool ins_stage_out_aliases_input(const RkEpi& epi, const void* in) {
  bool a = (const void*)epi.ustar == in || epi.ustar == epi.ustart;
  for (int q = 0; q < epi.n; ++q) a = a || epi.ustar == epi.k[q];
  return a;
}
static inline bool ins_stage_carry_aliases(const RkEpi& epi, const void* in) {
  bool a = (const void*)epi.carry_out == in || epi.carry_out == epi.ustart || epi.carry_out == epi.ustar;
  for (int q = 0; q < epi.n; ++q) a = a || epi.carry_out == epi.k[q];
  return a;
}

struct TempEpi {
  const double* temp;
  const double* tempstart;
  double* temp_out;
  double* ktemp_out;
  int n;
  double coef[INS_MAX_STAGES];
  const double* k[INS_MAX_STAGES];
  double c_self, a4, dcoef;
};


int ins_k_apply_bc_u(const ins_grid* grid, double* u, int dudt, const double* const* planes, hipStream_t s);
int ins_k_apply_bc_p(const ins_grid* grid, double* p, hipStream_t s);
int ins_k_apply_bc_p_fields(const ins_grid* grid, double* p, int nf, hipStream_t s);
int ins_k_momentum(const ins_grid* grid, double visc, const double* u, double* F, hipStream_t s);
int ins_k_divergence(const ins_grid* grid, const double* u, double* div, hipStream_t s);
int ins_k_diffusion_overwrite(const ins_grid* grid, double visc, const double* u, double* F, hipStream_t s);
int ins_k_scalewithvolume(const ins_grid* grid, double* p, hipStream_t s);
int ins_k_applypressure(const ins_grid* grid, double* u, const double* p, hipStream_t s);
int ins_k_laplacian(const ins_grid* grid, const double* p, double* L, hipStream_t s);
int ins_k_project(const ins_grid* grid, ins_poisson* ps, double* u, double* p, hipStream_t s);
int ins_k_momentum_rk_fused(const ins_grid* G, double visc, const double* u_in, double* k_out, const RkEpi& epi, hipStream_t s);
bool ins_flux2d_supported(const ins_grid* G);
int ins_k_flux2d(const ins_grid* G, double visc, const double* u, double* F, const RkEpi* epi, hipStream_t s, const double* pI = nullptr);
int ins_k_project_periodic_solve_only_2d(const ins_grid* G, ins_poisson* ps, const double* u, hipStream_t s);
int ins_k_momentum_rk_fused_generic(const ins_grid* G, double visc, const double* u_in, double* k_out, const RkEpi& epi, hipStream_t s);
int ins_k_momentum_rk_fused_corr(const ins_grid* G, double visc, const double* ustar_prev, const double* pI, double* k_out, const RkEpi& epi,
                                 hipStream_t s);
int ins_k_momentum_rk_fused_corr_slab(const ins_grid* G, double visc, const double* ustar_prev, const double* p_ext, double* k_out,
                                      const RkEpi& epi, hipStream_t s, int part = 0);
bool ins_corr3_supported(const ins_grid* G);
int ins_k_momentum_rk_fused_corr3(const ins_grid* G, double visc, const double* ustar_prev, const double* p_padded, double* k_out, const RkEpi& epi,
                                  hipStream_t s);
bool ins_k_project_fdm_fused(const ins_poisson* ps);
int ins_k_project_fdm_solve_only(const ins_grid* G, ins_poisson* ps, const double* u, double* p, hipStream_t s);
int ins_k_project_periodic_fused_2d(const ins_grid* G, ins_poisson* ps, double* u, double* p, bool keep_p, hipStream_t s);
bool ins_poisson_own2d(const ins_poisson* ps);
int ins_k_project_periodic_solve_only(const ins_grid* G, ins_poisson* ps, const double* u, hipStream_t s, const double* rhs = nullptr);
bool ins_flux64_stage_rhs_supported(const ins_grid* G, int corr_mode);
bool ins_flux64_stage_carry_supported(const ins_grid* G);
double* ins_poisson_stage_rhs(ins_poisson* ps);
int ins_k_poisson_solve(ins_poisson* ps, double* p, hipStream_t s);
bool ins_fast3d_supported(const ins_grid* G);

static inline bool ins_rk_fused3d(const ins_rk* rk) {
  const ins_grid* G = rk->grid;
  bool ok = !ins_opt(OPT_INS_DISABLE_FUSED_RK) && G->g.D == 3 && G->all_periodic && G->all_dof && rk->ps->kind == POISSON_SPECTRAL && ins_fast3d_supported(G);
  for (int a = 0; ok && a < 3; ++a) ok = rk->ps->np[a] >= 2;
  return ok;
}
static inline bool ins_rk_fused2d(const ins_rk* rk) {
  return !ins_opt(OPT_INS_DISABLE_FUSED_RK) && rk->grid->g.D == 2 && ins_poisson_own2d(rk->ps) && ins_flux2d_supported(rk->grid);
}
static inline bool ins_rk_inkernel3d(const ins_rk* rk) {
  const ins_grid* G = rk->grid;
  return !ins_opt(OPT_INS_DISABLE_INKERNEL_CORR) && G->uniform_exact && rk->nstage > 1 && G->g.N[0] >= 8 && G->g.N[1] >= 8 && G->g.N[2] >= 8;
}
static inline bool ins_rk_inkernel2d(const ins_rk* rk) {
  return rk->nstage > 1 && !ins_opt(OPT_INS_DISABLE_INKERNEL_CORR) && !ins_opt(OPT_INS_DISABLE_CORR2D) && rk->grid->g.N[0] >= 6 && rk->grid->g.N[1] >= 6;
}
static inline bool ins_rk_chainable(const ins_rk* rk) {
  return !ins_opt(OPT_INS_DISABLE_STEP_CHAIN) && ((ins_rk_fused3d(rk) && ins_rk_inkernel3d(rk)) || (ins_rk_fused2d(rk) && ins_rk_inkernel2d(rk)));
}
int ins_rk_ensure_ub(ins_rk* rk, size_t bytes, hipStream_t s, const double* init_from);
int ins_k_reduce(const ins_grid* grid, int op, const double* a, const double* b, const int lo[3], const int hi[3], double* out,
                 hipStream_t s);

int ins_validate_real_plans(hipfftHandle fwd, hipfftHandle inv, int rank, const int* n, int batch);
int ins_fft_make_real_plans(hipfftHandle* fwd, hipfftHandle* inv, int rank, int* n, int batch);
void ins_fft_solver_released();
static inline bool ins_pow2_len(int n) { return n >= 16 && n <= 1024 && !(n & (n - 1)); }
static inline bool ins_mixed_len(int n) {
  return (n == 96 || n == 192 || n == 384 || n == 160 || n == 320 || n == 640) && !ins_opt(OPT_INS_OWNFFT_POW2_ONLY);
}
enum XfwdSrc {
  XSRC_PI = 0,
  XSRC_DIV = 1,
  XSRC_DIV_SLAB = 2,
  XSRC_DIV_2D = 3,
  XSRC_DIV_WALLS = 4,
  XSRC_DIV_U32 = 5,
  XSRC_FIELD = 6,
};
bool ins_zsolve_supported(int nz);
bool ins_ownfft_supported(const int np[3]);
bool ins_ownfft_supported_slab(const int np[3]);
bool ins_ownfft_supported_mixed(const int np[3]);
void ins_ownfft_permute_symbol(int n, const double* ay, double* out);
int ins_k_ownfft_xfwd(const ins_grid* G, const double* src, int from_u, double* phat, int n0, int n1, int n2, const double* tw, hipStream_t s,
                      int kxs = 0, int kz0 = 0);
int ins_k_ownfft_xinv(const double* phat, double* pI, int n0, int n1, int n2, const double* tw, hipStream_t s, int kxs = 0);
int ins_k_ownfft_y(double* phat, int kxn, int n1, int n2, const double* tw, bool inverse, hipStream_t s, int kxs = 0);
bool ins_ownfft_xy_supported(int n0, int n1);
int ins_k_ownfft_xy(const ins_grid* G, const double* src, int from_u, double* phat, double* pI, int n0, int n1, int n2, const double* twx, const double* twy,
                    bool inverse, hipStream_t s, int kxs);
int ins_k_ownfft_xysolve2d(const ins_grid* G, const double* src, int from_u, double* pI, int n0, int n1, const double* twx, const double* twy, const double* ax,
                           const double* ay, hipStream_t s);
bool ins_line3_supported(int n);
void ins_line3_permute_symbol(int n, const double* ay, double* out);
int ins_line3_pos_of_freq(int n, int k);
int ins_k_line3_z(double* phat, int kxn, int n1, int n2, const double* tw, hipStream_t s, int kxs);
int ins_k_line3_y(double* phat, int kxn, int n1, int n2, const double* tw, bool inverse, hipStream_t s, int kxs);
int ins_k_line3_y_f32(float* phat, int kxn, int n1, int n2, const float* tw, bool inverse, hipStream_t s, int kxs);
int ins_ownfft_yz_partitions(int kxn, int n1, int n2);
long long ins_ownfft_yz_scratch(int kxn, int n1, int n2, int P);
int ins_k_ownfft_yz_solve(double* phat, int kxn, int n1, int n2, int kxs, int P, const double* ax, const double* ay, double c, double scale, const double* tw_y,
                          double* scratch, hipStream_t s);
int ins_k_ownfft_y_packed(double* phat, double* packed, int kxn, int n1, int nzl, int nyl, int cw, const double* tw, bool inverse,
                          hipStream_t s);
int ins_zsolve_twiddles(int nz, double** out);
int ins_k_fdm_z(double* data, int n0, int n1, int nz, const double* lx, const double* ly, const double* lz, const double* ox, const double* oy,
                double h, double tol, int singular, const double* meanf, double* partial, const double* tw, int* nblk, hipStream_t s, const double* dct_w = nullptr);
int ins_k_zsolve(double* data, int nz, long long nl, const double* ax, int kxn, const double* ay, const double* az, const double* tw,
                 double inv_n, bool zero_mean, hipStream_t s, int kxs = 0);

int ins_comm_allreduce_internal(struct ins_comm* c, double* buf, long long count, int op, hipStream_t s);
int ins_comm_halo_scalar_internal(struct ins_comm* c, const ins_grid* G, double* p, hipStream_t s);

static inline hipStream_t as_stream(void* s) { return reinterpret_cast<hipStream_t>(s); }
static inline unsigned cdiv(long long a, long long b) { return (unsigned)((a + b - 1) / b); }
```

incompressiblenavierstokes.jl_amd/csrc/ins_poisson.hip:

```cpp
#include <algorithm>
#include <cmath>
#include <cstdlib>

#include "ins_stencil.h"

namespace {

template <int D, bool WRAP = false>
__global__ __launch_bounds__(256) void k_div_to_pI(GridDev g, const double* __restrict__ u, double* __restrict__ pI, int n0, int n1) {
  const int ii = blockIdx.x * 64 + threadIdx.x;
  const int jj = blockIdx.y * 4 + threadIdx.y;
  const int kk = D == 3 ? (int)blockIdx.z : 0;
  if (ii >= n0 || jj >= n1) return;
  const int I[3] = {g.ip_lo[0] + ii, g.ip_lo[1] + jj, D == 3 ? g.ip_lo[2] + kk : 0};
  const long long c = I[0] + I[1] * g.sx[1] + I[2] * g.sx[2];
  double d = 0.0;
#pragma unroll
  for (int a = 0; a < D; ++a) {
    const double* ua = u + a * g.sc;
    const long long cm = (WRAP && I[a] == 1) ? c + (long long)(g.N[a] - 3) * g.sx[a] : c - g.sx[a];
    d += (ua[c] - ua[cm]) * g.rdx[a][I[a]];
  }
  double om = g.dx[0][I[0]] * g.dx[1][I[1]];
  if (D == 3) om = om * g.dx[2][I[2]];
// ... 666 lines not shown
  flat_partial(s, partial);
}
__global__ __launch_bounds__(256) void k_cgd_update(GridDev g, long long n, const double* __restrict__ sc, double* __restrict__ p, double* __restrict__ r,
                                                    const double* __restrict__ q, const double* __restrict__ L, double* __restrict__ partial) {
  if (sc[CG_DONE] != 0.0) return;
  const double alpha = sc[CG_ALPHA];
  double s = 0.0;
  for (long long t = (long long)blockIdx.x * 256 + threadIdx.x; t < n; t += (long long)gridDim.x * 256) {
    bool inp;
    flat_cell(g, t, inp);
    p[t] += alpha * q[t];
    const double rv = r[t] - alpha * L[t];
    r[t] = rv;
    if (inp) s += rv * rv;
  }
  flat_partial(s, partial);
}

struct BoxLaunch {
  dim3 grid, block;
  int nblk;
};

inline BoxLaunch full_box(const GridDev& g) {
  BoxLaunch l;
  l.block = dim3(64, 4, 1);
  l.grid = dim3(cdiv(g.N[0], 64), cdiv(g.N[1], 4), (unsigned)g.N[2]);
  l.nblk = (int)(l.grid.x * l.grid.y * l.grid.z);
  return l;
}

}

static inline bool own_route(SpectralRoute r) { return r >= ROUTE_OWN2D; }

static SpectralRoute ins_spectral_choose(int D, const int np[3], int* yz_P) {
  *yz_P = 0;
  if (D == 2) {
    const int np2[3] = {np[0], 16, np[1]};
    if (!ins_ownfft_supported(np2)) return ROUTE_ROCFFT;
    return ins_ownfft_xy_supported(np[0], np[1]) ? ROUTE_OWN2D_ONE : ROUTE_OWN2D;
  }
  if (!ins_ownfft_supported_mixed(np)) return ins_zsolve_supported(np[2]) ? ROUTE_ROCFFT_ZFUSED : ROUTE_ROCFFT;
  if ((*yz_P = ins_ownfft_yz_partitions(np[0] / 2 + 1, np[1], np[2]))) return ROUTE_OWN_YZ;
  if (ins_line3_supported(np[1])) return ROUTE_OWN_LINE3;
  return ins_ownfft_xy_supported(np[0], np[1]) ? ROUTE_OWN_XY : ROUTE_OWN_LDS;
}

static KyOrder ins_spectral_ky_order(SpectralRoute r) {
  switch (r) {
    case ROUTE_OWN_LDS:
    case ROUTE_OWN_XY:
    case ROUTE_OWN_YZ: return KY_DIGITREV;
    case ROUTE_OWN_LINE3: return KY_LINE3;
    default: return KY_NATURAL;
  }
}

static void permute_ky(KyOrder order, int n, const double* ay, double* out) {
  switch (order) {
    case KY_DIGITREV: return ins_ownfft_permute_symbol(n, ay, out);
    case KY_LINE3: return ins_line3_permute_symbol(n, ay, out);
    case KY_NATURAL: std::copy(ay, ay + n, out);
  }
}

extern "C" int ins_poisson_spectral_create(const ins_grid_t* G, ins_poisson_t** out) {
  INS_REQUIRE(G && out, "null argument");
  INS_REQUIRE(G->all_periodic, "Spectral psolver requires periodic boundary conditions.");
  INS_REQUIRE(G->uniform, "Spectral psolver requires uniform grid spacing.");
  const GridDev& g = G->g;
  for (int a = 0; a < g.D; ++a) INS_REQUIRE(g.N[a] % 2 == 0, "Spectral psolver requires even number of volumes.");
  ins_poisson* ps = new ins_poisson();
  ps->kind = POISSON_SPECTRAL;
  ps->grid = G;
  const int D = g.D;
  long long nreal = 1, ncplx = 1;
  double om = 1.0;
  for (int a = 0; a < D; ++a) {
    ps->np[a] = g.ip_hi[a] - g.ip_lo[a];
    ps->kmax[a] = a == 0 ? ps->np[a] / 2 + 1 : ps->np[a];
    nreal *= ps->np[a];
    ncplx *= ps->kmax[a];
    om *= G->h[a];
  }
  int rc = INS_OK;
  auto fail = [&](int code) {
    ins_poisson_destroy(ps);
    return code;
  };
  ps->route = ins_spectral_choose(D, ps->np, &ps->yz_P);
  ps->ky_order = ins_spectral_ky_order(ps->route);
  const bool own = own_route(ps->route), own2d = ps->route == ROUTE_OWN2D || ps->route == ROUTE_OWN2D_ONE;
  if (own) {
    ps->kxs = ins_opt(OPT_INS_PHAT_DENSE) ? ps->kmax[0] : ((ps->kmax[0] + 7) & ~7);
    ncplx = (long long)ps->kxs * ps->kmax[1] * ps->kmax[2];
  }
  if (hipMalloc(&ps->pI, nreal * sizeof(double)) != hipSuccess || hipMalloc(&ps->phat, ncplx * sizeof(hipfftDoubleComplex)) != hipSuccess ||
      hipMemset(ps->phat, 0, ncplx * sizeof(hipfftDoubleComplex)) != hipSuccess) {
    ins_set_error("hipMalloc(pI/phat) failed for %lld cells", nreal);
    return fail(INS_ERR_HIP);
  }
  for (int a = 0; a < D; ++a) {
    std::vector<double> ah(ps->kmax[a]);
    for (int k = 0; k < ps->kmax[a]; ++k) {
      const double sn = std::sin(M_PI * ((double)k / ps->np[a]));
      ah[k] = 4 * om * sn * sn / (G->h[a] * G->h[a]);
    }
    if (a == 1) {
      std::vector<double> perm(ah.size());
      permute_ky(ps->ky_order, ps->np[1], ah.data(), perm.data());
      ah.swap(perm);
    }
    if (hipMalloc(&ps->ahat[a], ah.size() * sizeof(double)) != hipSuccess ||
        hipMemcpy(ps->ahat[a], ah.data(), ah.size() * sizeof(double), hipMemcpyHostToDevice) != hipSuccess) {
      ins_set_error("ahat upload failed");
      return fail(INS_ERR_HIP);
    }
  }
  if (own2d) {
    if ((rc = ins_zsolve_twiddles(ps->np[0], &ps->tw_x))) return fail(rc);
    if ((rc = ins_zsolve_twiddles(ps->np[1], &ps->tw))) return fail(rc);
    if (hipMalloc(&ps->ahat[2], sizeof(double)) != hipSuccess || hipMemset(ps->ahat[2], 0, sizeof(double)) != hipSuccess) return fail(INS_ERR_HIP);
  } else if (own) {
    if ((rc = ins_zsolve_twiddles(ps->np[0], &ps->tw_x))) return fail(rc);
    if ((rc = ins_zsolve_twiddles(ps->np[1], &ps->tw_y))) return fail(rc);
    if ((rc = ins_zsolve_twiddles(ps->np[2], &ps->tw))) return fail(rc);
    if (ps->route == ROUTE_OWN_YZ) {
      const long long nc = ins_ownfft_yz_scratch(ps->kmax[0], ps->np[1], ps->np[2], ps->yz_P);
      if (hipMalloc(&ps->yz_scratch, nc * 2 * sizeof(double)) != hipSuccess) {
        ins_set_error("hipMalloc(yz scratch) failed");
        return fail(INS_ERR_HIP);
      }
    }
  } else {
    int nfull[3] = {ps->np[2], ps->np[1], ps->np[0]};
    const bool zfused = ps->route == ROUTE_ROCFFT_ZFUSED;
    rc = zfused ? ins_fft_make_real_plans(&ps->plan_fwd, &ps->plan_inv, 2, nfull + 1, ps->np[2])
                : ins_fft_make_real_plans(&ps->plan_fwd, &ps->plan_inv, D, nfull + (3 - D), 1);
    if (rc) {
      ps->plan_fwd = ps->plan_inv = 0;
      return fail(rc);
    }
    if (zfused && (rc = ins_zsolve_twiddles(ps->np[2], &ps->tw))) return fail(rc);
  }
  *out = ps;
  return INS_OK;
}

static SpectralRoute route_for_source(const ins_poisson* ps, int src) {
  return (ps->route == ROUTE_OWN_XY && src != XSRC_PI && src != XSRC_DIV) ? ROUTE_OWN_LDS : ps->route;
}

static int spectral_transform(ins_poisson* ps, hipStream_t s, const double* u = nullptr, int src = XSRC_DIV, const double* rhs = nullptr) {
  const GridDev& g = ps->grid->g;
  const int n0 = ps->np[0], n1 = ps->np[1], n2 = ps->np[2], kxn = ps->kmax[0], kxs = ps->kxs;
  double* ph = reinterpret_cast<double*>(ps->phat);
  if (rhs) u = nullptr;
  const double* f = u ? u : (rhs ? rhs : ps->pI);
  if (!u) src = XSRC_PI;
  const SpectralRoute route = route_for_source(ps, src);
  INS_REQUIRE(!rhs || (own_route(route) && g.D == 3), "spectral solve: a right-hand side outside pI needs an own-FFT 3-D route");
  INS_REQUIRE(ins_spectral_ky_order(route) == ps->ky_order, "spectral solve: the route for this source leaves ky in another order than the solver's symbol");
  const double inv_n = 1.0 / ((double)n0 * n1 * n2);
  auto zpass = [&]() { return ins_k_zsolve(ph, n2, (long long)kxs * n1, ps->ahat[0], kxn, ps->ahat[1], ps->ahat[2], ps->tw, inv_n, true, s, kxs); };
  int rc;
  switch (route) {
    case ROUTE_ROCFFT:
    case ROUTE_ROCFFT_ZFUSED: {
      INS_REQUIRE(!u, "spectral solve: the rocFFT routes take their right-hand side from pI");
      INS_FFT_TRY(hipfftSetStream(ps->plan_fwd, s));
      INS_FFT_TRY(hipfftSetStream(ps->plan_inv, s));
      INS_FFT_TRY(hipfftExecD2Z(ps->plan_fwd, ps->pI, ps->phat));
      double inv_np = 1.0;
      for (int a = 0; a < g.D; ++a) inv_np /= ps->np[a];
      if (route == ROUTE_ROCFFT_ZFUSED) {
        if ((rc = ins_k_zsolve(ph, n2, (long long)kxn * ps->kmax[1], ps->ahat[0], kxn, ps->ahat[1], ps->ahat[2], ps->tw, inv_np, true, s))) return rc;
      } else {
        dim3 block(64, 4, 1), grid(cdiv(kxn, 64), cdiv(ps->kmax[1], 4), g.D == 3 ? ps->kmax[2] : 1);
        INS_LAUNCH_D((k_symbol<D>), (Launch3{grid, block}), s, ps->phat, ps->ahat[0], ps->ahat[1], ps->ahat[2], kxn, ps->kmax[1], inv_np);
      }
      INS_FFT_TRY(hipfftExecZ2D(ps->plan_inv, ps->phat, ps->pI));
      return INS_OK;
    }
    case ROUTE_OWN2D_ONE:
      return ins_k_ownfft_xysolve2d(ps->grid, f, u ? XSRC_DIV : XSRC_PI, ps->pI, n0, n1, ps->tw_x, ps->tw, ps->ahat[0], ps->ahat[1], s);
    case ROUTE_OWN2D:
      if ((rc = ins_k_ownfft_xfwd(ps->grid, f, src, ph, n0, n1, 1, ps->tw_x, s, kxs))) return rc;
      if ((rc = ins_k_zsolve(ph, n1, (long long)kxs, ps->ahat[0], kxn, ps->ahat[2], ps->ahat[1], ps->tw, inv_n, true, s, kxs))) return rc;
      return ins_k_ownfft_xinv(ph, ps->pI, n0, n1, 1, ps->tw_x, s, kxs);
    case ROUTE_OWN_XY:
      if ((rc = ins_k_ownfft_xy(ps->grid, f, src, ph, nullptr, n0, n1, n2, ps->tw_x, ps->tw_y, false, s, kxs))) return rc;
      if ((rc = zpass())) return rc;
      return ins_k_ownfft_xy(nullptr, nullptr, XSRC_PI, ph, ps->pI, n0, n1, n2, ps->tw_x, ps->tw_y, true, s, kxs);
    case ROUTE_OWN_YZ: {
      if ((rc = ins_k_ownfft_xfwd(ps->grid, f, src, ph, n0, n1, n2, ps->tw_x, s, kxs))) return rc;
      const ins_grid* G = ps->grid;
      const double c = G->h[0] * G->h[1] / G->h[2];
      if ((rc = ins_k_ownfft_yz_solve(ph, kxn, n1, n2, kxs, ps->yz_P, ps->ahat[0], ps->ahat[1], c, -1.0 / ((double)n0 * n1), ps->tw_y, ps->yz_scratch, s))) return rc;
      return ins_k_ownfft_xinv(ph, ps->pI, n0, n1, n2, ps->tw_x, s, kxs);
    }
    case ROUTE_OWN_LDS:
    case ROUTE_OWN_LINE3: {
      const auto ypass = route == ROUTE_OWN_LINE3 ? ins_k_line3_y : ins_k_ownfft_y;
      if ((rc = ins_k_ownfft_xfwd(ps->grid, f, src, ph, n0, n1, n2, ps->tw_x, s, kxs))) return rc;
      if ((rc = ypass(ph, kxn, n1, n2, ps->tw_y, false, s, kxs))) return rc;
      if ((rc = zpass())) return rc;
      if ((rc = ypass(ph, kxn, n1, n2, ps->tw_y, true, s, kxs))) return rc;
      return ins_k_ownfft_xinv(ph, ps->pI, n0, n1, n2, ps->tw_x, s, kxs);
    }
  }
  ins_set_error("spectral solve: unknown route %d", (int)route);
  return INS_ERR_INVALID;
}

template <bool PACK>
static int pack_box(const ins_poisson* ps, double* p, double* buf, hipStream_t s, const double* shift = nullptr) {
  const GridDev& g = ps->grid->g;
  dim3 block(64, 4, 1), grid(cdiv(ps->np[0], 64), cdiv(ps->np[1], 4), g.D == 3 ? ps->np[2] : 1);
  INS_LAUNCH_D((k_pack<D, PACK>), (Launch3{grid, block}), s, g, p, buf, ps->np[0], ps->np[1], shift);
  return INS_OK;
}

static int spectral_solve(ins_poisson* ps, double* p, hipStream_t s) {
  int rc;
  if ((rc = pack_box<true>(ps, p, ps->pI, s)) || (rc = spectral_transform(ps, s))) return rc;
  return pack_box<false>(ps, p, ps->pI, s);
}

extern "C" int ins_poisson_cg_create(const ins_grid_t* G, double abstol, double reltol, int64_t maxiter, ins_poisson_t** out) {
  INS_REQUIRE(G && out, "null argument");
  const GridDev& g = G->g;
  for (int a = 0; a < 2 && a < g.D; ++a)
    INS_REQUIRE(g.bc[a][0] != INS_BC_HALO && g.bc[a][1] != INS_BC_HALO, "slabs are cut along z only");
  ins_poisson* ps = new ins_poisson();
  ps->kind = POISSON_CG;
  ps->grid = G;
  ps->abstol = abstol;
  ps->reltol = reltol;
  long long ndof = 1;
  for (int a = 0; a < g.D; ++a) ndof *= g.ip_hi[a] - g.ip_lo[a];
  ps->maxiter = maxiter > 0 ? maxiter : ndof;
  ps->ndof = ndof;
  for (int a = 0; a < g.D; ++a)
    if (g.bc[a][0] == INS_BC_PRESSURE || g.bc[a][1] == INS_BC_PRESSURE) ps->singular = false;
  const size_t bytes = G->ncell * sizeof(double);
  if (hipMalloc(&ps->r, bytes) != hipSuccess || hipMalloc(&ps->L, bytes) != hipSuccess || hipMalloc(&ps->q, bytes) != hipSuccess ||
      hipMalloc(&ps->dinv, bytes) != hipSuccess) {
    ins_set_error("hipMalloc(cg scratch) failed");
    ins_poisson_destroy(ps);
    return INS_ERR_HIP;
  }
  BoxLaunch l = full_box(g);
  if (g.D == 2)
    hipLaunchKernelGGL(k_cg_diag<2>, l.grid, l.block, 0, 0, g, ps->dinv);
  else
    hipLaunchKernelGGL(k_cg_diag<3>, l.grid, l.block, 0, 0, g, ps->dinv);
  if (hipDeviceSynchronize() != hipSuccess) {
    ins_set_error("cg diag kernel failed");
    ins_poisson_destroy(ps);
    return INS_ERR_HIP;
  }
  *out = ps;
  return INS_OK;
}

static int finish_sum(const ins_grid* G, double* partial_dev, int nblk, hipStream_t s, double* out) {
  std::vector<double> h(nblk);
  INS_HIP_TRY(hipMemcpyAsync(h.data(), partial_dev, nblk * sizeof(double), hipMemcpyDeviceToHost, s));
  INS_HIP_TRY(hipStreamSynchronize(s));
  double v = 0.0;
  for (int i = 0; i < nblk; ++i) v += h[i];
  *out = v;
  return INS_OK;
}


static int cg_remove_mean(ins_poisson* ps, double* p, hipStream_t s) {
  const ins_grid* G = ps->grid;
  const GridDev& g = G->g;
  const BoxLaunch l = full_box(g);
  double sum;
  int rc = ins_k_reduce(G, 3, p, nullptr, g.ip_lo, g.ip_hi, &sum, s);
  if (rc) return rc;
  INS_LAUNCH_D((k_shift<D>), l, s, g, p, sum / (double)ps->ndof);
  return INS_OK;
}

static int cg_solve_device(ins_poisson* ps, double* p, hipStream_t s) {
  const ins_grid* G = ps->grid;
  const GridDev& g = G->g;
  const long long n = G->ncell;
  if (!ps->cg_scal) {
    INS_HIP_TRY(hipMalloc(&ps->cg_scal, (CG_NSCAL + CG_NPART) * sizeof(double)));
    INS_HIP_TRY(hipHostMalloc(&ps->cg_host, CG_NSCAL * sizeof(double)));
  }
  double* sc = ps->cg_scal;
  double* partial = sc + CG_NSCAL;
  const unsigned nb = (unsigned)std::min<long long>((n + 255) / 256, CG_NPART);
  int rc;
  const double maxit = (double)ps->maxiter;
  auto fold = [&](int stage) -> int {
    hipLaunchKernelGGL(k_cgd_fold, dim3(1), dim3(1024), 0, s, partial, (int)nb, sc);
    if (ps->comm) {
      int r2 = ins_comm_allreduce_internal(ps->comm, sc + CG_SUM, 1, 0, s);
      if (r2) return r2;
    }
    hipLaunchKernelGGL(k_cgd_scalars, dim3(1), dim3(1), 0, s, sc, stage, ps->reltol, ps->abstol, maxit);
    INS_LAUNCH_CHECK();
    return INS_OK;
  };
  const bool bordered = ps->bordered && ps->singular;
  if (bordered) {
    INS_REQUIRE(!ps->comm, "bordered CG on slabs is not implemented");
    if ((rc = cg_remove_mean(ps, p, s))) return rc;
  }
  hipLaunchKernelGGL(k_cgd_init, dim3(nb), dim3(256), 0, s, g, n, p, ps->r, ps->q, ps->L, partial);
  if ((rc = fold(0))) return rc;
  const long long batch = ins_opt(OPT_INS_CG_BATCH) > 0 ? ins_opt(OPT_INS_CG_BATCH) : 32;
  long long issued = 0;
  while (true) {
    INS_HIP_TRY(hipMemcpyAsync(ps->cg_host, sc, CG_NSCAL * sizeof(double), hipMemcpyDeviceToHost, s));
    INS_HIP_TRY(hipStreamSynchronize(s));
    if (ps->cg_host[CG_DONE] != 0.0 || issued >= ps->maxiter) break;
    for (long long b = 0; b < batch && issued < ps->maxiter; ++b, ++issued) {
      hipLaunchKernelGGL(k_cgd_precond, dim3(nb), dim3(256), 0, s, g, n, sc, ps->r, ps->dinv, ps->L, partial);
      if ((rc = fold(1))) return rc;
      hipLaunchKernelGGL(k_cgd_dir, dim3(nb), dim3(256), 0, s, n, sc, ps->L, ps->q);
      if ((rc = ins_k_apply_bc_p(G, ps->q, s))) return rc;
      if (ps->comm && (rc = ins_comm_halo_scalar_internal(ps->comm, G, ps->q, s))) return rc;
      if ((rc = ins_k_laplacian(G, ps->q, ps->L, s))) return rc;
      hipLaunchKernelGGL(k_cgd_dot, dim3(nb), dim3(256), 0, s, g, n, sc, ps->q, ps->L, partial);
      if ((rc = fold(2))) return rc;
      hipLaunchKernelGGL(k_cgd_update, dim3(nb), dim3(256), 0, s, g, n, sc, p, ps->r, ps->q, ps->L, partial);
      if ((rc = fold(3))) return rc;
    }
  }
  if (bordered && (rc = cg_remove_mean(ps, p, s))) return rc;
  ps->last_iter = (long long)ps->cg_host[CG_ITERS];
  ps->last_res = ps->cg_host[CG_RES];
  return INS_OK;
}

static int cg_solve(ins_poisson* ps, double* p, hipStream_t s) {
  if (!ins_opt(OPT_INS_CG_HOSTSYNC)) return cg_solve_device(ps, p, s);
  INS_REQUIRE(!ps->comm, "the host-synchronising CG has no slab form");
  const ins_grid* G = ps->grid;
  const GridDev& g = G->g;
  BoxLaunch l = full_box(g);
  double* partial = nullptr;
  INS_HIP_TRY(hipMalloc(&partial, l.nblk * sizeof(double)));
  struct Guard {
    double* p;
    ~Guard() { (void)hipFree(p); }
  } guard{partial};
  int rc;
  double ss;
  const bool bordered = ps->bordered && ps->singular;
// ... 133 lines not shown
    ins_poisson_destroy(ps);
    return code;
  };
  if (g.D == 3 && periodic(2) && uniform(2, true)) {
    if ((rc = ins_fdm_enable_zfft(ps->fdm, d.dx[2][1], lam[2]))) return fail(rc);
    if (periodic(0) && uniform(0, true) && (rc = ins_fdm_enable_xfft(ps->fdm, d.dx[0][1], lam[0]))) return fail(rc);
  }
  if (g.D == 3 && periodic(0) && periodic(1) && !periodic(2) && uniform(0, true) && uniform(1, true)) {
    if ((rc = ins_fdm_enable_xyfft(ps->fdm, d.dx[0][1], d.dx[1][1], lam[0], lam[1]))) return fail(rc);
  }
  if (g.D == 3 && g.bc[2][0] != INS_BC_PERIODIC && uniform(2, false) && (rc = ins_fdm_enable_zdct(ps->fdm, d.dx[2][1], lam[2]))) return fail(rc);
  *out = ps;
  return INS_OK;
}

int ins_k_poisson_solve(ins_poisson* ps, double* p, hipStream_t s) {
  switch (ps->kind) {
    case POISSON_SPECTRAL: return spectral_solve(ps, p, s);
    case POISSON_FDM: return fdm_solve(ps, p, s);
    default: return cg_solve(ps, p, s);
  }
}

extern "C" int ins_poisson_solve_f64(ins_poisson_t* ps, double* p, void* stream) {
  INS_REQUIRE(ps && p, "null argument");
  return ins_k_poisson_solve(ps, p, as_stream(stream));
}

int ins_fdm_modes(const ins_fdm* F);
extern "C" int ins_dbg_fdm_modes(const ins_poisson_t* ps) { return (ps && ps->kind == POISSON_FDM) ? ins_fdm_modes(ps->fdm) : -1; }
extern "C" int ins_dbg_spectral_route(const ins_poisson_t* ps, int32_t* ky_order) {
  const bool spectral = ps && ps->kind == POISSON_SPECTRAL;
  if (ky_order) *ky_order = spectral ? (int32_t)ps->ky_order : -1;
  return spectral ? (int)ps->route : -1;
}
extern "C" int ins_dbg_spectral_choose(int D, int n0, int n1, int n2, int32_t* ky_order, int32_t* partitions) {
  const int np[3] = {n0, n1, D == 3 ? n2 : 1};
  int P = 0;
  const SpectralRoute r = ins_spectral_choose(D, np, &P);
  if (ky_order) *ky_order = (int32_t)ins_spectral_ky_order(r);
  if (partitions) *partitions = P;
  return (int)r;
}
extern "C" void ins_dbg_permute_ky(int ky_order, int n, const double* ay, double* out) { permute_ky((KyOrder)ky_order, n, ay, out); }
extern "C" int ins_dbg_line3_pos_of_freq(int n, int k) { return ins_line3_pos_of_freq(n, k); }
extern "C" int ins_dbg_fdm_fold_mask(const ins_poisson_t* ps) { return (ps && ps->kind == POISSON_FDM) ? ins_fdm_fold_mask(ps->fdm) : -1; }

extern "C" int ins_poisson_last_info(const ins_poisson_t* ps, int64_t* iterations, double* residual) {
  INS_REQUIRE(ps, "null argument");
  if (iterations) *iterations = ps->last_iter;
  if (residual) *residual = ps->last_res;
  return INS_OK;
}

bool ins_k_project_fdm_fused(const ins_poisson* ps) { return ps->kind == POISSON_FDM && !ins_opt(OPT_INS_DISABLE_FDM_FUSED); }
static int fdm_rhs(const ins_grid* G, ins_poisson* ps, const double* u, double* buf, int fm, hipStream_t s) {
  const GridDev& g = G->g;
  const dim3 block(64, 4, 1);
  if (fm) {
    const int n0 = ps->np[0], n1 = ps->np[1], n2 = g.D == 3 ? ps->np[2] : 1;
    const dim3 grid(cdiv((fm & 1) ? n0 / 2 : n0, 64), cdiv((fm & 2) ? n1 / 2 : n1, 4), (g.D == 3 && (fm & 4)) ? n2 / 2 : n2);
#define INS_DIVFOLD(DD, MM) \
  case MM: hipLaunchKernelGGL((k_div_to_pI_fold<DD, MM>), grid, block, 0, s, g, u, buf, n0, n1, n2); break;
    if (g.D == 2) {
      switch (fm & 3) {
        INS_DIVFOLD(2, 1)
        INS_DIVFOLD(2, 2)
        INS_DIVFOLD(2, 3)
      }
    } else {
      switch (fm & 7) {
        INS_DIVFOLD(3, 1)
        INS_DIVFOLD(3, 2)
        INS_DIVFOLD(3, 3)
        INS_DIVFOLD(3, 4)
        INS_DIVFOLD(3, 5)
        INS_DIVFOLD(3, 6)
        INS_DIVFOLD(3, 7)
      }
    }
#undef INS_DIVFOLD
  } else {
    const dim3 grid(cdiv(ps->np[0], 64), cdiv(ps->np[1], 4), g.D == 3 ? ps->np[2] : 1);
    INS_LAUNCH_D((k_div_to_pI<D>), (Launch3{grid, block}), s, g, u, buf, ps->np[0], ps->np[1]);
  }
  INS_LAUNCH_CHECK();
  return INS_OK;
}

static int fdm_unpack(const ins_grid* G, ins_poisson* ps, double* u, double* p, const double* buf, int fm, hipStream_t s) {
  const GridDev& g = G->g;
  const dim3 block(64, 4, 1);
  const int n0 = ps->np[0], n1 = ps->np[1], n2 = g.D == 3 ? ps->np[2] : 1;
  bool pressure_side = false;
  for (int a = 0; a < g.D; ++a) pressure_side = pressure_side || g.bc[a][0] == INS_BC_PRESSURE || g.bc[a][1] == INS_BC_PRESSURE;
  if (g.D == 3 && fm && !pressure_side && !((fm & 1) && (n0 & 1)) && !((fm & 2) && (n1 & 1)) && !((fm & 4) && (n2 & 1)) && !ins_opt(OPT_INS_DISABLE_FDM_UNFOLD4)) {
    const dim3 grid(cdiv((fm & 1) ? n0 / 2 : n0, 64), cdiv((fm & 2) ? n1 / 2 : n1, 4), (fm & 4) ? n2 / 2 : n2);
    if (u)
      hipLaunchKernelGGL(k_unfold_grad3<true>, grid, block, 0, s, g, u, p, buf, n0, n1, n2, ins_fdm_mean(ps->fdm), fm);
    else
      hipLaunchKernelGGL(k_unfold_grad3<false>, grid, block, 0, s, g, u, p, buf, n0, n1, n2, ins_fdm_mean(ps->fdm), fm);
    INS_LAUNCH_CHECK();
    return INS_OK;
  }
  const dim3 gridp(cdiv(n0 + 2, 64), cdiv(n1 + 2, 4), g.D == 3 ? n2 + 2 : 1);
  if (g.D == 2) {
    if (u)
      hipLaunchKernelGGL((k_unpack_grad_bc<2, true>), gridp, block, 0, s, g, u, p, buf, n0, n1, ins_fdm_mean(ps->fdm), fm, 1);
    else
      hipLaunchKernelGGL((k_unpack_grad_bc<2, false>), gridp, block, 0, s, g, u, p, buf, n0, n1, ins_fdm_mean(ps->fdm), fm, 1);
  } else {
    if (u)
      hipLaunchKernelGGL((k_unpack_grad_bc<3, true>), gridp, block, 0, s, g, u, p, buf, n0, n1, ins_fdm_mean(ps->fdm), fm, n2);
    else
      hipLaunchKernelGGL((k_unpack_grad_bc<3, false>), gridp, block, 0, s, g, u, p, buf, n0, n1, ins_fdm_mean(ps->fdm), fm, n2);
  }
  INS_LAUNCH_CHECK();
  return INS_OK;
}

static int fdm_project(const ins_grid* G, ins_poisson* ps, const double* u, double* ucorr, double* p, hipStream_t s) {
  int rc, fm = 0;
  double* buf = ins_fdm_buffer(ps->fdm);
  if (ins_fdm_takes_u(ps->fdm)) {
    if ((rc = ins_fdm_solve(ps->fdm, s, G, u))) return rc;
  } else {
    fm = ins_opt(OPT_INS_DISABLE_FDM_FOLDFUSE) ? 0 : ins_fdm_fold_mask(ps->fdm);
    if ((rc = fdm_rhs(G, ps, u, buf, fm, s))) return rc;
    if ((rc = ins_fdm_solve(ps->fdm, s, nullptr, nullptr, fm != 0))) return rc;
  }
  return fdm_unpack(G, ps, ucorr, p, buf, fm, s);
}
int ins_k_project_fdm_solve_only(const ins_grid* G, ins_poisson* ps, const double* u, double* p, hipStream_t s) { return fdm_project(G, ps, u, nullptr, p, s); }

int ins_k_project(const ins_grid* G, ins_poisson* ps, double* u, double* p, hipStream_t s) {
  const GridDev& g = G->g;
  int rc;
  if (ps->kind == POISSON_SPECTRAL) {
    dim3 block(64, 4, 1), grid(cdiv(ps->np[0], 64), cdiv(ps->np[1], 4), g.D == 3 ? ps->np[2] : 1);
    INS_LAUNCH_D((k_div_to_pI<D>), (Launch3{grid, block}), s, g, u, ps->pI, ps->np[0], ps->np[1]);
    if ((rc = spectral_transform(ps, s))) return rc;
    dim3 gridp(cdiv(g.N[0], 64), cdiv(g.N[1], 4), (unsigned)g.N[2]);
    INS_LAUNCH_D((k_grad_from_pI<D>), (Launch3{gridp, block}), s, g, u, p, ps->pI, ps->np[0], ps->np[1], ps->np[2]);
    return INS_OK;
  }
  if (ins_k_project_fdm_fused(ps)) return fdm_project(G, ps, u, u, p, s);
  if ((rc = ins_k_divergence(G, u, p, s))) return rc;
  if ((rc = ins_k_scalewithvolume(G, p, s))) return rc;
  if ((rc = ins_k_poisson_solve(ps, p, s))) return rc;
  if ((rc = ins_k_apply_bc_p(G, p, s))) return rc;
  return ins_k_applypressure(G, u, p, s);
}

int ins_k_project_periodic_solve_only(const ins_grid* G, ins_poisson* ps, const double* u, hipStream_t s, const double* rhs) {
  const GridDev& g = G->g;
  if (own_route(ps->route)) return spectral_transform(ps, s, u, XSRC_DIV, rhs);
  INS_REQUIRE(!rhs, "a right-hand side written by the stage kernel needs an own-FFT route");
  dim3 block(64, 4, 1), grid(cdiv(ps->np[0], 64), cdiv(ps->np[1], 4), ps->np[2]);
  hipLaunchKernelGGL((k_div_to_pI<3, true>), grid, block, 0, s, g, u, ps->pI, ps->np[0], ps->np[1]);
  INS_LAUNCH_CHECK();
  return spectral_transform(ps, s);
}

int ins_k_project_periodic_fused(const ins_grid* G, ins_poisson* ps, double* u, double* p, bool keep_p, hipStream_t s, double* uout, const double* rhs) {
  const GridDev& g = G->g;
  dim3 block(64, 4, 1), grid(cdiv(ps->np[0], 64), cdiv(ps->np[1], 4), ps->np[2]);
  double* dst = uout ? uout : u;
  int rc = ins_k_project_periodic_solve_only(G, ps, u, s, rhs);
  if (rc) return rc;
  if (keep_p)
    hipLaunchKernelGGL(k_grad_ghost3<true>, grid, block, 0, s, g, dst, p, ps->pI, ps->np[0], ps->np[1], ps->np[2], (const double*)u);
  else
    hipLaunchKernelGGL(k_grad_ghost3<false>, grid, block, 0, s, g, dst, p, ps->pI, ps->np[0], ps->np[1], ps->np[2], (const double*)u);
  INS_LAUNCH_CHECK();
  return INS_OK;
}

bool ins_poisson_own2d(const ins_poisson* ps) { return ps->kind == POISSON_SPECTRAL && (ps->route == ROUTE_OWN2D || ps->route == ROUTE_OWN2D_ONE); }
int ins_k_project_periodic_solve_only_2d(const ins_grid* G, ins_poisson* ps, const double* u, hipStream_t s) {
  return spectral_transform(ps, s, u, XSRC_DIV_2D);
}
int ins_k_project_periodic_fused_2d(const ins_grid* G, ins_poisson* ps, double* u, double* p, bool keep_p, hipStream_t s) {
  const GridDev& g = G->g;
  const int n0 = ps->np[0], n1 = ps->np[1];
  int rc = ins_k_project_periodic_solve_only_2d(G, ps, u, s);
  if (rc) return rc;
  dim3 block(64, 4, 1), grid(cdiv(n0, 64), cdiv(n1, 4), 1);
  if (keep_p)
    hipLaunchKernelGGL((k_grad_ghost<2, true>), grid, block, 0, s, g, u, p, ps->pI, n0, n1, 1);
  else
    hipLaunchKernelGGL((k_grad_ghost<2, false>), grid, block, 0, s, g, u, p, ps->pI, n0, n1, 1);
  INS_LAUNCH_CHECK();
  return INS_OK;
}

bool ins_k_spectral_own3d(const ins_poisson* ps) { return ps->kind == POISSON_SPECTRAL && own_route(ps->route) && ps->grid->g.D == 3; }
double* ins_poisson_stage_rhs(ins_poisson* ps) {
  if (!ins_k_spectral_own3d(ps)) return nullptr;
  if (!ps->rhs && hipMalloc(&ps->rhs, (size_t)ps->np[0] * ps->np[1] * ps->np[2] * sizeof(double)) != hipSuccess) {
    (void)hipGetLastError();
    ps->rhs = nullptr;
  }
  return ps->rhs;
}
int ins_k_spectral_solve_from_u32(ins_poisson* ps, const float* u32, hipStream_t s) {
  return spectral_transform(ps, s, reinterpret_cast<const double*>(u32), XSRC_DIV_U32);
}
const double* ins_k_spectral_pI(const ins_poisson* ps) { return ps->pI; }

bool ins_zsolve_f32_supported(int nz);
int ins_k_zsolve_f32(float* data, int nz, long long nl, const double* ax, int kxn, const double* ay, const double* az, const float* tw, double inv_n,
                     bool zero_mean, hipStream_t s, int kxs);
int ins_k_ownfft_xfwd_f32(const ins_grid* G, const float* src, int from_u, float* phat, int n0, int n1, int n2, const float* tw, hipStream_t s, int kxs);
int ins_k_ownfft_xinv_f32(const float* phat, float* pI, int n0, int n1, int n2, const float* tw, hipStream_t s, int kxs);
int ins_k_ownfft_y_f32(float* phat, int kxn, int n1, int n2, const float* tw, bool inverse, hipStream_t s, int kxs);
bool ins_k_spectral_own3d_f32(const ins_poisson* ps) { return ins_k_spectral_own3d(ps) && ins_zsolve_f32_supported(ps->np[2]); }
int ins_k_spectral_solve_f32(ins_poisson* ps, const float* u32, float* pI32, float* phat32, int kxs32, const float* twx, const float* twy,
                             const float* twz, hipStream_t s) {
  const int n0 = ps->np[0], n1 = ps->np[1], n2 = ps->np[2], kxn = ps->kmax[0];
  INS_REQUIRE(ps->ky_order != KY_NATURAL, "float2 spectral solve: the solver has no own y pass");
  const auto ypass = ps->ky_order == KY_LINE3 ? ins_k_line3_y_f32 : ins_k_ownfft_y_f32;
  int rc;
  if ((rc = ins_k_ownfft_xfwd_f32(ps->grid, u32 ? u32 : pI32, u32 ? XSRC_DIV : XSRC_PI, phat32, n0, n1, n2, twx, s, kxs32))) return rc;
  if ((rc = ypass(phat32, kxn, n1, n2, twy, false, s, kxs32))) return rc;
  const double inv_n = 1.0 / ((double)n0 * n1 * n2);
  if ((rc = ins_k_zsolve_f32(phat32, n2, (long long)kxs32 * n1, ps->ahat[0], kxn, ps->ahat[1], ps->ahat[2], twz, inv_n, true, s, kxs32))) return rc;
  if ((rc = ypass(phat32, kxn, n1, n2, twy, true, s, kxs32))) return rc;
  return ins_k_ownfft_xinv_f32(phat32, pI32, n0, n1, n2, twx, s, kxs32);
}

extern "C" int ins_project_f64(const ins_grid_t* G, ins_poisson_t* ps, double* u, double* p, void* stream) {
  INS_REQUIRE(G && ps && u && p, "null argument");
  INS_REQUIRE(ps->grid == G, "psolver was created for a different grid");
  return ins_k_project(G, ps, u, p, as_stream(stream));
}
```

incompressiblenavierstokes.jl_amd/csrc/ins_rk.hip:

```cpp
#include <cstdlib>

#include "ins_internal.h"
#include "ins_rk_terms.h"

int ins_k_momentum_generic(const ins_grid* G, double visc, const double* u, double* F, hipStream_t s);
int ins_k_momentum_fast3d(const ins_grid* G, double visc, const double* u, double* F, hipStream_t s);
int ins_k_momentum_fast3d_opts(const ins_grid* G, double visc, const double* u, double* F, bool zero_shell, hipStream_t s);
bool ins_flux64_supported(const ins_grid* G);

int ins_k_momentum_rk_fused(const ins_grid* G, double visc, const double* u_in, double* k_out, const RkEpi& epi, hipStream_t s);
int ins_k_project_periodic_fused(const ins_grid* G, ins_poisson* ps, double* u, double* p, bool keep_p, hipStream_t s, double* uout = nullptr,
                                 const double* rhs = nullptr);

int ins_k_momentum(const ins_grid* G, double visc, const double* u, double* F, hipStream_t s) {
  if (ins_fast3d_supported(G)) return ins_k_momentum_fast3d(G, visc, u, F, s);
  return ins_k_momentum_generic(G, visc, u, F, s);
}

namespace {

struct Combine {
  int n;
  double coef[INS_MAX_STAGES + 1];
  const double* k[INS_MAX_STAGES + 1];
};

__global__ __launch_bounds__(256) void k_combine(long long n, const double* ustart, double* u, Combine cb) {
  const long long stride = (long long)gridDim.x * 256 * 2;
  for (long long t = ((long long)blockIdx.x * 256 + threadIdx.x) * 2; t < n; t += stride) {
    if (t + 1 < n) {
      double2 v = *reinterpret_cast<const double2*>(ustart + t);
      for (int j = 0; j < cb.n; ++j) {
        const double2 kv = *reinterpret_cast<const double2*>(cb.k[j] + t);
        v.x += cb.coef[j] * kv.x;
        v.y += cb.coef[j] * kv.y;
      }
      *reinterpret_cast<double2*>(u + t) = v;
    } else {
      double v = ustart[t];
      for (int j = 0; j < cb.n; ++j) v += cb.coef[j] * cb.k[j][t];
      u[t] = v;
    }
  }
}

}

static int combine_n(long long nvec, const double* base, double* out, int nterms, const double* coefs, const double* const* ks, void* stream);

extern "C" int ins_combine_f64(const ins_grid_t* G, const double* base, double* out, int nterms, const double* coefs,
                               const double* const* ks, void* stream) {
  INS_REQUIRE(G && base && out, "null argument");
  return combine_n(G->ncell * G->g.D, base, out, nterms, coefs, ks, stream);
}

extern "C" int ins_combine_scalar_f64(const ins_grid_t* G, const double* base, double* out, int nterms, const double* coefs,
                                      const double* const* ks, void* stream) {
  INS_REQUIRE(G && base && out, "null argument");
  return combine_n(G->ncell, base, out, nterms, coefs, ks, stream);
}

static int combine_n(long long nvec, const double* base, double* out, int nterms, const double* coefs, const double* const* ks, void* stream) {
  INS_REQUIRE(nterms >= 0 && nterms <= INS_MAX_STAGES + 1 && (nterms == 0 || (coefs && ks)), "bad stage terms");
  Combine cb;
  cb.n = 0;
  for (int q = 0; q < nterms; ++q) {
    if (coefs[q] == 0.0) continue;
    INS_REQUIRE(ks[q], "null stage field");
    cb.coef[cb.n] = coefs[q];
    cb.k[cb.n] = ks[q];
    ++cb.n;
  }
  const unsigned nblk = (unsigned)std::min<long long>((nvec / 2 + 255) / 256, 8192);
  hipLaunchKernelGGL(k_combine, dim3(nblk), dim3(256), 0, as_stream(stream), nvec, base, out, cb);
  INS_LAUNCH_CHECK();
  return INS_OK;
}

static void step_graph_free(ins_rk* rk);
bool ins_k_spectral_own3d(const ins_poisson* ps);

extern "C" int ins_rk_create(const ins_grid_t* G, ins_poisson_t* ps, int nstage, const double* A, const double* c, ins_rk_t** out) {
  INS_REQUIRE(G && ps && A && c && out, "null argument");
  INS_REQUIRE(ps->grid == G, "psolver was created for a different grid");
  INS_REQUIRE(nstage >= 1 && nstage <= INS_MAX_STAGES, "unsupported number of stages");
  for (int i = 0; i < nstage; ++i)
    for (int j = i + 1; j < nstage; ++j) INS_REQUIRE(A[i * nstage + j] == 0.0, "shifted tableau must be lower triangular (explicit method)");
  ins_rk* rk = new ins_rk();
  rk->grid = G;
  rk->ps = ps;
  rk->nstage = nstage;
  rk->A.assign(A, A + nstage * nstage);
  rk->c.assign(c, c + nstage);
  const size_t vbytes = (size_t)G->ncell * G->g.D * sizeof(double);
  bool ok = hipMalloc(&rk->ustart, vbytes) == hipSuccess && hipMalloc(&rk->p, G->ncell * sizeof(double)) == hipSuccess;
  rk->ku.assign(nstage, nullptr);
  for (int i = 0; ok && i < nstage; ++i) ok = hipMalloc(&rk->ku[i], vbytes) == hipSuccess;
  if (ok) ok = hipMemset(rk->p, 0, G->ncell * sizeof(double)) == hipSuccess && hipMemset(rk->ustart, 0, vbytes) == hipSuccess;
  for (int i = 0; ok && i < nstage; ++i) ok = hipMemset(rk->ku[i], 0, vbytes) == hipSuccess;
  if (!ok) {
    ins_set_error("ins_rk_create: device allocation of %d vector fields failed", nstage + 1);
    ins_rk_destroy(rk);
    return INS_ERR_HIP;
  }
  *out = rk;
  return INS_OK;
}

extern "C" int ins_rk_destroy(ins_rk_t* rk) {
  if (!rk) return INS_OK;
  if (rk->ustart) (void)hipFree(rk->ustart);
  if (rk->p) (void)hipFree(rk->p);
  for (double* k : rk->ku)
    if (k) (void)hipFree(k);
  for (double* v : rk->vb)
    if (v && v != rk->ub[0] && v != rk->ub[1]) (void)hipFree(v);
  for (double* b : rk->ub)
    if (b) (void)hipFree(b);
  for (hipEvent_t e : rk->prof_events) (void)hipEventDestroy(e);
  ins_rk_ext_free(rk->ext);
  step_graph_free(rk);
  delete rk;
  return INS_OK;
}

extern "C" int ins_rk_profile_enable(ins_rk_t* rk, int enable) {
  INS_REQUIRE(rk, "null argument");
  rk->profiling = enable != 0;
  return INS_OK;
}

extern "C" int ins_rk_profile_read(ins_rk_t* rk, double* momentum_ms, int64_t* momentum_launches) {
  INS_REQUIRE(rk && momentum_ms && momentum_launches, "null argument");
  double total = 0.0;
  const size_t n = rk->prof_events.size() / 2;
  for (size_t i = 0; i < n; ++i) {
    float ms = 0.f;
    INS_HIP_TRY(hipEventSynchronize(rk->prof_events[2 * i + 1]));
    INS_HIP_TRY(hipEventElapsedTime(&ms, rk->prof_events[2 * i], rk->prof_events[2 * i + 1]));
    total += ms;
  }
  for (hipEvent_t e : rk->prof_events) (void)hipEventDestroy(e);
  rk->prof_events.clear();
  *momentum_ms = total;
  *momentum_launches = (int64_t)n;
  return INS_OK;
}

extern "C" int ins_rk_pressure(const ins_rk_t* rk, double** p) {
  INS_REQUIRE(rk && p, "null argument");
  *p = rk->p;
  return INS_OK;
}

extern "C" int ins_dbg_stage_rhs_used(const ins_rk_t* rk, int64_t* launches) {
  INS_REQUIRE(rk && launches, "null argument");
  *launches = (int64_t)rk->stage_rhs_launches;
  return INS_OK;
}

extern "C" int ins_dbg_stage_carry_used(const ins_rk_t* rk, int64_t* launches) {
  INS_REQUIRE(rk && launches, "null argument");
  *launches = (int64_t)rk->stage_carry_launches;
  return INS_OK;
}

extern "C" int ins_dbg_rk_carry_plan(int32_t ns, const double* A, double dt, int32_t with_force, int32_t* j, int32_t* i, double* a, double* self_in,
                                     double* coef_self, double* coef_force) {
  INS_REQUIRE(A && j && i && a && self_in && coef_self && coef_force, "null argument");
  INS_REQUIRE(ns >= 1 && ns <= INS_MAX_STAGES, "bad argument");
  const RkCarryPlan pl = ins_rk_carry_plan(A, ns);
  *j = pl.j, *i = pl.i, *self_in = 0.0, *coef_self = 0.0, *coef_force = 0.0;
  for (int q = 0; q < 3; ++q) a[q] = pl.a[q];
  if (pl.j < 0) return INS_OK;
  static double slot[2];
  const RkEpi epi = ins_rk_carry_consumer_terms<double>(A, ns, pl, dt, slot, with_force ? slot + 1 : nullptr);
  INS_REQUIRE(epi.ustart == slot && epi.c0m1 == 0.0 && epi.n == (with_force ? 1 : 0), "consumer terms");
  *self_in = epi.self_in, *coef_self = epi.coef_self;
  if (with_force) *coef_force = epi.coef[0];
  return INS_OK;
}

extern "C" int ins_dbg_stage_rhs(ins_rk_t* rk, double visc, const double* u_in, const double* pI, const double* ustart, const double* kterm, double coef_k,
                                 double self_in, double coef_self, double* ustar, double* rhs, int32_t* used, void* stream) {
  INS_REQUIRE(rk && u_in && ustar && rhs && used, "null argument");
  const ins_grid* G = rk->grid;
  hipStream_t s = as_stream(stream);
  RkEpi epi;
  memset(&epi, 0, sizeof(epi));
  epi.ustart = ustart;
  epi.ustar = ustar;
  epi.coef_self = coef_self;
  if (ustart) {
    epi.self_in = self_in;
    epi.c0m1 = -self_in;
  }
  if (kterm) {
    epi.coef[0] = coef_k;
    epi.k[0] = kterm;
    epi.n = 1;
  }
  *used = 0;
  INS_REQUIRE(!ins_stage_out_aliases_input(epi, u_in), "ustar must be an array of its own");
  if (ins_flux64_stage_rhs_supported(G, pI ? 1 : 0) && (epi.rhs_out = ins_poisson_stage_rhs(rk->ps))) *used = 1;
  int rc = pI ? ins_k_momentum_rk_fused_corr(G, visc, u_in, pI, rk->ku[0], epi, s) : ins_k_momentum_rk_fused(G, visc, u_in, rk->ku[0], epi, s);
  if (rc) return rc;
  if (*used) INS_HIP_TRY(hipMemcpyAsync(rhs, epi.rhs_out, (size_t)rk->ps->np[0] * rk->ps->np[1] * rk->ps->np[2] * sizeof(double), hipMemcpyDeviceToDevice, s));
  return INS_OK;
}

extern "C" int ins_dbg_rk_stage_terms(int32_t ns, const double* A, int32_t i, double dt, int32_t kind, int32_t input_in_regs, int32_t with_force, int32_t order,
                                      int32_t* n, int32_t* stage, double* coef, double* c0m1, double* self_in, double* coef_self, int32_t* write_k,
                                      double* coef_force) {
  INS_REQUIRE(A && n && stage && coef && c0m1 && self_in && coef_self && write_k && coef_force, "null argument");
  INS_REQUIRE(ns >= 1 && ns <= INS_MAX_STAGES && i >= 0 && i < ns && kind >= 0 && kind <= 3, "bad argument");
  INS_REQUIRE(kind != 1 || ins_rk_vbasis_possible(A, ns), "the stage-velocity basis needs a non-zero diagonal");
  static double slot[INS_MAX_STAGES + 1];
  double* prev[INS_MAX_STAGES];
  for (int m = 0; m < ns; ++m) prev[m] = slot + m;
  const double* force = with_force ? slot + ns : nullptr;
  RkEpi epi;
  memset(&epi, 0, sizeof(epi));
  if (kind <= 1) {
    epi = ins_rk_stage_terms(A, ns, i, dt, prev, force, kind ? RK_V_BASIS : RK_K_BASIS, input_in_regs != 0, order ? RK_FORCE_INDEX_ORDER : RK_FORCE_DIAG_FIRST);
  } else if (kind == 2) {
    epi.n = ins_rk_sum_terms(A, ns, i, dt, prev, force, epi.coef, epi.k);
  } else {
    float cf32[INS_MAX_STAGES + 1];
    epi.n = ins_rk_sum_terms(A, ns, i, (float)dt, prev, force, cf32, epi.k);
    for (int q = 0; q < epi.n; ++q) epi.coef[q] = cf32[q];
  }
  *n = epi.n, *c0m1 = epi.c0m1, *self_in = epi.self_in, *coef_self = epi.coef_self, *write_k = epi.write_k, *coef_force = 0.0;
  for (int q = 0; q < epi.n; ++q) {
    stage[q] = (int32_t)(epi.k[q] - slot);
    coef[q] = epi.coef[q];
    if (epi.k[q] == force) *coef_force = epi.coef[q];
  }
  return INS_OK;
}

extern "C" int ins_rk_set_bodyforce(ins_rk_t* rk, const double* force) {
  INS_REQUIRE(rk, "null argument");
  rk->force = force;
  return INS_OK;
}

extern "C" int ins_rk_stage_force(const ins_rk_t* rk, int i, double** ku) {
  INS_REQUIRE(rk && ku, "null argument");
  INS_REQUIRE(i >= 0 && i < rk->nstage, "stage index out of range");
  *ku = rk->ku[i];
  return INS_OK;
}

template <typename F>
static int timed_stage(ins_rk* rk, hipStream_t s, F&& launch) {
  if (!rk->profiling) return launch();
  hipEvent_t e0 = nullptr, e1 = nullptr;
  INS_HIP_TRY(hipEventCreate(&e0));
  INS_HIP_TRY(hipEventCreate(&e1));
  INS_HIP_TRY(hipEventRecord(e0, s));
  const int rc = launch();
  if (rc) return rc;
  INS_HIP_TRY(hipEventRecord(e1, s));
  rk->prof_events.push_back(e0);
  rk->prof_events.push_back(e1);
  return INS_OK;
}

int ins_rk_ensure_ub(ins_rk* rk, size_t bytes, hipStream_t s, const double* init_from) {
  for (int b = 0; b < 2; ++b)
    if (!rk->ub[b]) {
      INS_HIP_TRY(hipMalloc(&rk->ub[b], bytes));
      if (init_from)
        INS_HIP_TRY(hipMemcpyAsync(rk->ub[b], init_from, bytes, hipMemcpyDeviceToDevice, s));
      else
        INS_HIP_TRY(hipMemsetAsync(rk->ub[b], 0, bytes, s));
    }
  return INS_OK;
}

static int rk_step_fused_periodic(ins_rk* rk, double visc, double* u, double dt, hipStream_t s, int chain = 0) {
  const ins_grid* G = rk->grid;
  const int ns = rk->nstage;
  const size_t vbytes = (size_t)G->ncell * 3 * sizeof(double);
  int rc;
  if ((rc = ins_rk_ensure_ub(rk, vbytes, s, nullptr))) return rc;
  const bool raw_in = chain & 1, raw_out = chain & 2;
  if (!raw_in && (rc = ins_k_apply_bc_u(G, u, 0, nullptr, s))) return rc;
  const bool inkernel = ins_rk_inkernel3d(rk);
  const bool vbasis = inkernel && !ins_opt(OPT_INS_RK_KEEP_K) && ins_rk_vbasis_possible(rk->A.data(), ns);
  if (vbasis && (int)rk->vb.size() < ns - 1) {
    rk->vb.resize(ns - 1, nullptr);
    for (int m = 0; m < ns - 1; ++m)
      if (!rk->vb[m]) {
        if (m < 2 && rk->ub[m]) {
          rk->vb[m] = rk->ub[m];
          continue;
        }
        INS_HIP_TRY(hipMalloc(&rk->vb[m], vbytes));
        INS_HIP_TRY(hipMemsetAsync(rk->vb[m], 0, vbytes, s));
      }
  }
  RkCarryPlan pl = {-1, -1, {0.0, 0.0, 0.0}};
  if (vbasis && ins_flux64_stage_carry_supported(G)) pl = ins_rk_carry_plan(rk->A.data(), ns);
  const bool carry = pl.j >= 0;
  const double* in = u;
  for (int i = 0; i < ns; ++i) {
    double* out = (i == ns - 1 && ns > 1) ? u : (vbasis ? rk->vb[(carry && i == pl.j + 1) ? pl.j - 1 : i] : rk->ub[i & 1]);
    RkEpi epi = ins_rk_stage_terms(rk->A.data(), ns, i, dt, vbasis ? rk->vb.data() : rk->ku.data(), rk->force, vbasis ? RK_V_BASIS : RK_K_BASIS,
                                   vbasis && ins_flux64_supported(G), RK_FORCE_DIAG_FIRST);
    epi.ustart = (i == 0) ? nullptr : (raw_in ? rk->ustart : u);
    epi.ustar = out;
    const bool in_place = ins_stage_out_aliases_input(epi, in);
    if (carry && i == pl.j) {
      epi.carry_out = rk->vb[pl.j + 1];
      for (int q = 0; q < 3; ++q) epi.ca[q] = pl.a[q];
      if (ins_stage_carry_aliases(epi, in) || in_place) {
        ins_set_error("carried stage combination: an output of stage %d is one of its inputs", i);
        return INS_ERR_INVALID;
      }
      ++rk->stage_carry_launches;
    }
    if (carry && i == pl.i) {
      epi = ins_rk_carry_consumer_terms(rk->A.data(), ns, pl, dt, rk->vb[pl.j + 1], rk->force);
      epi.ustar = out;
    }
    if (i == 0 && raw_in) epi.ustart_out = rk->ustart;
    const bool corr = inkernel && (i > 0 || raw_in);
    if (!in_place && ins_flux64_stage_rhs_supported(G, corr ? 1 : 0) && (epi.rhs_out = ins_poisson_stage_rhs(rk->ps)))
      ++rk->stage_rhs_launches;
    rc = timed_stage(rk, s, [&] {
      return corr ? ins_k_momentum_rk_fused_corr(G, visc, in, rk->ps->pI, rk->ku[i], epi, s) : ins_k_momentum_rk_fused(G, visc, in, rk->ku[i], epi, s);
    });
    if (rc) return rc;
    rc = (inkernel && (i < ns - 1 || raw_out)) ? ins_k_project_periodic_solve_only(G, rk->ps, out, s, epi.rhs_out)
                                               : ins_k_project_periodic_fused(G, rk->ps, out, rk->p, i == ns - 1, s, nullptr, epi.rhs_out);
    if (rc) return rc;
    in = out;
  }
  if (ns == 1) INS_HIP_TRY(hipMemcpyAsync(u, rk->ub[0], vbytes, hipMemcpyDeviceToDevice, s));
  return INS_OK;
}

static int rk_step_fused_periodic_2d(ins_rk* rk, double visc, double* u, double dt, hipStream_t s, int chain = 0) {
  const ins_grid* G = rk->grid;
  const int ns = rk->nstage;
  const size_t vbytes = (size_t)G->ncell * 2 * sizeof(double);
  int rc;
  if ((rc = ins_rk_ensure_ub(rk, vbytes, s, nullptr))) return rc;
  const bool raw_in = chain & 1, raw_out = chain & 2;
  if (!raw_in && (rc = ins_k_apply_bc_u(G, u, 0, nullptr, s))) return rc;
  const bool incorr = ins_rk_inkernel2d(rk);
  if (chain && !incorr) {
    ins_set_error("chained 2-D steps need the in-register correction");
    return INS_ERR_INVALID;
  }
  const double* in = u;
  for (int i = 0; i < ns; ++i) {
    double* out = (i == ns - 1 && ns > 1) ? u : rk->ub[i & 1];
    RkEpi epi = ins_rk_stage_terms(rk->A.data(), ns, i, dt, rk->ku.data(), rk->force, RK_K_BASIS, false, RK_FORCE_INDEX_ORDER);
    epi.ustart = (i == 0) ? nullptr : (raw_in ? rk->ustart : u);
    epi.ustar = out;
    if (i == 0 && raw_in) epi.ustart_out = rk->ustart;
    rc = timed_stage(rk, s, [&] { return ins_k_flux2d(G, visc, in, rk->ku[i], &epi, s, (incorr && (i > 0 || raw_in)) ? rk->ps->pI : nullptr); });
    if (rc) return rc;
    rc = (incorr && (i < ns - 1 || raw_out)) ? ins_k_project_periodic_solve_only_2d(G, rk->ps, out, s) : ins_k_project_periodic_fused_2d(G, rk->ps, out, rk->p, i == ns - 1, s);
    if (rc) return rc;
    in = out;
  }
  if (ns == 1) INS_HIP_TRY(hipMemcpyAsync(u, rk->ub[0], vbytes, hipMemcpyDeviceToDevice, s));
  return INS_OK;
}

struct StepGraph {
  hipStream_t gs = nullptr;
  hipEvent_t ev_in = nullptr, ev_out = nullptr;
  hipGraphExec_t exec = nullptr;
  double* u = nullptr;
  double dt = 0.0, visc = 0.0;
  const double* force = nullptr;
  int kind = 0;
  long long epoch = -1;
  long long replays = 0;
  bool broken = false;
};

static void step_graph_free(ins_rk* rk) {
  StepGraph* g = static_cast<StepGraph*>(rk->step_graph);
  if (!g) return;
  if (g->exec) (void)hipGraphExecDestroy(g->exec);
  if (g->ev_in) (void)hipEventDestroy(g->ev_in);
  if (g->ev_out) (void)hipEventDestroy(g->ev_out);
  if (g->gs) (void)hipStreamDestroy(g->gs);
  delete g;
  rk->step_graph = nullptr;
}

extern "C" long long ins_dbg_rk_graph_replays(const ins_rk_t* rk) { return (rk && rk->step_graph) ? static_cast<const StepGraph*>(rk->step_graph)->replays : 0; }

static int step_graph_kind(const ins_rk* rk, bool chain_ok) {
  const ins_grid* G = rk->grid;
  if (!ins_opt(OPT_INS_STEP_GRAPH) || ins_opt(OPT_INS_DISABLE_STEP_GRAPH) || rk->profiling || rk->ext) return 0;
  const bool own = G->g.D == 3 ? ins_rk_fused3d(rk) && ins_k_spectral_own3d(rk->ps) : ins_rk_fused2d(rk);
  return own ? (chain_ok ? 1 : 2) : 0;
}

static int chain_step(ins_rk* rk, double visc, double* u, double dt, hipStream_t s, int chain) {
  return rk->grid->g.D == 2 ? rk_step_fused_periodic_2d(rk, visc, u, dt, s, chain) : rk_step_fused_periodic(rk, visc, u, dt, s, chain);
}

template <typename F>
static bool step_graph_capture(StepGraph* g, F&& enqueue) {
  if (g->exec) {
    (void)hipGraphExecDestroy(g->exec);
    g->exec = nullptr;
  }
  if (!g->gs && hipStreamCreateWithFlags(&g->gs, hipStreamNonBlocking) != hipSuccess) return false;
  if (!g->ev_in && hipEventCreateWithFlags(&g->ev_in, hipEventDisableTiming) != hipSuccess) return false;
  if (!g->ev_out && hipEventCreateWithFlags(&g->ev_out, hipEventDisableTiming) != hipSuccess) return false;
  if (hipStreamBeginCapture(g->gs, hipStreamCaptureModeThreadLocal) != hipSuccess) {
    (void)hipGetLastError();
    return false;
  }
  const int rc = enqueue(g->gs);
  hipGraph_t graph = nullptr;
  const hipError_t e = hipStreamEndCapture(g->gs, &graph);
  bool ok = rc == INS_OK && e == hipSuccess && graph != nullptr;
  if (ok) ok = hipGraphInstantiate(&g->exec, graph, nullptr, nullptr, 0) == hipSuccess;
  if (graph) (void)hipGraphDestroy(graph);
  if (!ok) {
    (void)hipGetLastError();
    g->exec = nullptr;
  }
  return ok;
}

extern "C" int ins_rk_steps_f64(ins_rk_t* rk, double visc, double* u, double t, double dt, int nsteps, void* stream) {
  INS_REQUIRE(rk && u && nsteps >= 0, "bad argument");
  const ins_grid* G = rk->grid;
  hipStream_t s = as_stream(stream);
  const bool chain = ins_rk_chainable(rk) && !rk->force && !(G->g.D == 2 && rk->ext);
  const int gkind = step_graph_kind(rk, chain && nsteps >= 2);
  if (gkind && nsteps >= 3) {
    StepGraph* sg = static_cast<StepGraph*>(rk->step_graph);
    if (!sg) rk->step_graph = sg = new StepGraph();
    int rc, done = 0;
    if ((rc = gkind == 1 ? chain_step(rk, visc, u, dt, s, 2) : ins_rk_step_f64(rk, visc, u, t, dt, nullptr, stream))) return rc;
    done = 1;
    const int last_direct = gkind == 1 ? 1 : 0;
    const int nreplay = nsteps - done - last_direct;
    const bool same = sg->exec && sg->u == u && sg->dt == dt && sg->visc == visc && sg->force == rk->force && sg->kind == gkind && sg->epoch == ins_opt_epoch();
    if (!same && !sg->broken) {
      const bool got = step_graph_capture(sg, [&](hipStream_t gs) {
        return gkind == 1 ? chain_step(rk, visc, u, dt, gs, 3) : ins_rk_step_f64(rk, visc, u, t, dt, nullptr, gs);
      });
      sg->u = u, sg->dt = dt, sg->visc = visc, sg->force = rk->force, sg->kind = gkind, sg->epoch = ins_opt_epoch();
      if (!got) sg->broken = true;
    }
    if (sg->exec && !sg->broken && nreplay > 0) {
      INS_HIP_TRY(hipEventRecord(sg->ev_in, s));
      INS_HIP_TRY(hipStreamWaitEvent(sg->gs, sg->ev_in, 0));
      for (int n = 0; n < nreplay; ++n) INS_HIP_TRY(hipGraphLaunch(sg->exec, sg->gs));
      INS_HIP_TRY(hipEventRecord(sg->ev_out, sg->gs));
      INS_HIP_TRY(hipStreamWaitEvent(s, sg->ev_out, 0));
      sg->replays += nreplay;
      done += nreplay;
    }
    for (int n = done; n < nsteps; ++n) {
      if (gkind == 1)
        rc = chain_step(rk, visc, u, dt, s, 1 | (n < nsteps - 1 ? 2 : 0));
      else
        rc = ins_rk_step_f64(rk, visc, u, t + n * dt, dt, nullptr, stream);
      if (rc) return rc;
    }
    return INS_OK;
  }
  if (!chain || nsteps < 2) {
    for (int n = 0; n < nsteps; ++n) {
      int rc = ins_rk_step_f64(rk, visc, u, t + n * dt, dt, nullptr, stream);
      if (rc) return rc;
    }
    return INS_OK;
  }
  for (int n = 0; n < nsteps; ++n) {
    int rc = chain_step(rk, visc, u, dt, s, (n > 0 ? 1 : 0) | (n < nsteps - 1 ? 2 : 0));
    if (rc) return rc;
  }
  return INS_OK;
}
// ... 86 lines not shown
```

incompressiblenavierstokes.jl_amd/csrc/ins_rk_ext.hip:

```cpp
#include <cstring>
#include <vector>

#include "ins_internal.h"
#include "ins_rk_terms.h"

int ins_k_momentum_generic(const ins_grid* G, double visc, const double* u, double* F, hipStream_t s);
int ins_k_momentum_fast3d_opts(const ins_grid* G, double visc, const double* u, double* F, bool zero_shell, hipStream_t s);
int ins_k_momentum_rk_fused(const ins_grid* G, double visc, const double* u_in, double* k_out, const RkEpi& epi, hipStream_t s);
int ins_k_project_periodic_fused(const ins_grid* G, ins_poisson* ps, double* u, double* p, bool keep_p, hipStream_t s, double* uout = nullptr,
                                 const double* rhs = nullptr);
int ins_k_project(const ins_grid* G, ins_poisson* ps, double* u, double* p, hipStream_t s);
bool ins_flux64_supported(const ins_grid* G);
int ins_k_temp_stage(const ins_grid* G, double a4, double coef, const double* u, const double* temp, const double* w, const double* tempstart, int n,
                     const double* coefs, const double* const* ks, double c_self, double* ktemp_out, double* temp_out, hipStream_t s, const double* pI,
                     const double* diff = nullptr);
int ins_k_diffusion_overwrite(const ins_grid* G, double visc, const double* u, double* F, hipStream_t s);
bool ins_flux64m_supported(const ins_grid* G);
bool ins_smagforce_supported(const ins_grid* G);
int ins_k_smagforce(const ins_grid* G, double theta, const double* u, const double* pI, double* sout, hipStream_t s);
int ins_k_diffusion_flux3d(const ins_grid* G, double visc, const double* u, double* F, bool zero_shell, hipStream_t s);
int ins_k_momentum_rk_fused_corr(const ins_grid* G, double visc, const double* ustar_prev, const double* pI, double* k_out, const RkEpi& epi, hipStream_t s);
int ins_k_smagtensor_corr(const ins_grid* G, double theta, const double* ustar, const double* pI, double* sig, hipStream_t s);

struct ins_rk_ext {
  int closure = 0;
  double theta = 0.0;
  bool temp_on = false;
  ins_temperature_desc_t td;
  double* sigma = nullptr;
  double* E = nullptr;
  double* diff = nullptr;
  double* tempstart = nullptr;
  double* w = nullptr;
  double* tb[2] = {nullptr, nullptr};
  std::vector<double*> ktemp;
};

void ins_rk_ext_free(ins_rk_ext* e) {
  if (!e) return;
  for (double* p : {e->sigma, e->E, e->diff, e->tempstart, e->w, e->tb[0], e->tb[1]})
    if (p) (void)hipFree(p);
  for (double* p : e->ktemp)
    if (p) (void)hipFree(p);
  delete e;
}

static ins_rk_ext* ext_of(ins_rk* rk) {
  if (!rk->ext) rk->ext = new ins_rk_ext();
  return rk->ext;
}

extern "C" int ins_rk_set_closure(ins_rk_t* rk, int32_t kind, double theta) {
  INS_REQUIRE(rk, "null argument");
  INS_REQUIRE(kind == 0 || kind == 1, "closure kind: 0 (none) or 1 (Smagorinsky)");
  ins_rk_ext* e = ext_of(rk);
  e->closure = kind;
  e->theta = theta;
  return INS_OK;
}

extern "C" int ins_rk_set_temperature(ins_rk_t* rk, const ins_temperature_desc_t* desc) {
  INS_REQUIRE(rk, "null argument");
  ins_rk_ext* e = ext_of(rk);
  e->temp_on = desc != nullptr;
  if (desc) {
    INS_REQUIRE(desc->gdir >= 0 && desc->gdir < rk->grid->g.D, "gdir out of range");
    e->td = *desc;
  }
  return INS_OK;
}

static long long g_fused_steps = 0, g_tiled_steps = 0;
extern "C" long long ins_dbg_ext_tiled_steps(void) { return g_tiled_steps; }
extern "C" long long ins_dbg_ext_fused_steps(void) { return g_fused_steps; }

static int zalloc(double** p, size_t bytes, hipStream_t s) {
  if (*p) return INS_OK;
  INS_HIP_TRY(hipMalloc(p, bytes));
  INS_HIP_TRY(hipMemsetAsync(*p, 0, bytes, s));
  return INS_OK;
}

extern "C" int ins_rk_step_ext_f64(ins_rk_t* rk, double visc, double* u, double* temp, double t, double dt, void* stream) {
  INS_REQUIRE(rk && u, "null argument");
  ins_rk_ext* e = rk->ext;
  const bool closure = e && e->closure == 1, with_temp = e && e->temp_on;
  INS_REQUIRE(with_temp == (temp != nullptr), "a temperature field needs ins_rk_set_temperature and vice versa");
  if (!closure && !with_temp) return ins_rk_step_f64(rk, visc, u, t, dt, nullptr, stream);
  const ins_grid* G = rk->grid;
  const GridDev& g = G->g;
  hipStream_t s = as_stream(stream);
  const int ns = rk->nstage, D = g.D;
  const size_t sbytes = (size_t)G->ncell * sizeof(double), vbytes = sbytes * D;
  int rc;
  auto need_sigma = [&]() { return zalloc(&e->sigma, sbytes * (D * (D + 1) / 2), s); };
  if (closure && (rc = zalloc(&e->E, vbytes, s))) return rc;
  if (with_temp) {
    if ((rc = zalloc(&e->tempstart, sbytes, s))) return rc;
    if (e->td.dodissipation && (rc = zalloc(&e->diff, vbytes, s))) return rc;
    if ((int)e->ktemp.size() < ns) e->ktemp.resize(ns, nullptr);
    for (int i = 0; i < ns; ++i)
      if ((rc = zalloc(&e->ktemp[i], sbytes, s))) return rc;
    INS_HIP_TRY(hipMemcpyAsync(e->tempstart, temp, sbytes, hipMemcpyDeviceToDevice, s));
  }
  const ins_temperature_desc_t& td = e->td;
  auto bc_temp = [&]() { return with_temp ? ins_apply_bc_temp_f64(G, td.bc, td.val, nullptr, temp, stream) : INS_OK; };
  auto temp_rhs = [&](const double* v, int i) -> int {
    if (!with_temp) return INS_OK;
    int r;
    INS_HIP_TRY(hipMemsetAsync(e->ktemp[i], 0, sbytes, s));
    if ((r = ins_convection_diffusion_temp_f64(G, td.a4, v, temp, e->ktemp[i], stream))) return r;
    if (td.dodissipation && (r = ins_dissipation_f64(G, visc, td.diss_coef, v, e->diff, e->ktemp[i], stream))) return r;
    return INS_OK;
  };
  auto temp_combine = [&](int i) -> int {
    if (!with_temp) return INS_OK;
    double coefs[INS_MAX_STAGES];
    const double* ks[INS_MAX_STAGES];
    int n = 0;
    for (int j = 0; j <= i; ++j) {
      coefs[n] = dt * rk->A[i * ns + j];
      ks[n] = e->ktemp[j];
      ++n;
    }
    return ins_combine_scalar_f64(G, e->tempstart, temp, n, coefs, ks, stream);
  };

  const bool fused = ins_rk_fused3d(rk) && !ins_opt(OPT_INS_DISABLE_EXT_FUSED) && ins_flux64_supported(G);

  if (fused) {
    ++g_fused_steps;
    if ((rc = ins_rk_ensure_ub(rk, vbytes, s, nullptr))) return rc;
    if (with_temp) {
      for (int b = 0; b < 2; ++b)
        if ((rc = zalloc(&e->tb[b], sbytes, s))) return rc;
      if (td.dodissipation && (rc = zalloc(&e->w, vbytes, s))) return rc;
    }
    if ((rc = ins_k_apply_bc_u(G, u, 0, nullptr, s))) return rc;
    if ((rc = bc_temp())) return rc;
    const bool vbasis = ns > 1 && !ins_opt(OPT_INS_RK_KEEP_K) && ins_rk_vbasis_possible(rk->A.data(), ns);
    const bool tin_kernel = with_temp && !ins_opt(OPT_INS_EXT_TEMP_SPLIT);
    const bool smag1 = closure && ins_smagforce_supported(G);
    const bool incorr = vbasis && !tin_kernel && !ins_opt(OPT_INS_DISABLE_INKERNEL_CORR) && g.N[0] >= 34 && g.N[1] >= 8 && g.N[2] >= 8;
    const double* in = u;
    const double* tin = temp;
    for (int i = 0; i < ns; ++i) {
      const bool last = i == ns - 1 && ns > 1;
      double* out = last ? u : (vbasis ? rk->ku[i] : rk->ub[i & 1]);
      double* corrected = (last || incorr) ? out : rk->ub[i & 1];
      double* tout = with_temp ? (last ? temp : e->tb[i & 1]) : nullptr;
      const bool corr_in = incorr && i > 0;
      if (smag1) {
        if ((rc = ins_k_smagforce(G, e->theta, in, corr_in ? rk->ps->pI : nullptr, e->E, s))) return rc;
      } else if (closure) {
        if ((rc = need_sigma())) return rc;
        rc = corr_in ? ins_k_smagtensor_corr(G, e->theta, in, rk->ps->pI, e->sigma, s) : ins_smagtensor_f64(G, e->theta, in, e->sigma, stream);
        if (rc) return rc;
        if ((rc = ins_k_apply_bc_p_fields(G, e->sigma, D * (D + 1) / 2, s))) return rc;
        if ((rc = ins_divoftensor_f64(G, e->sigma, e->E, stream))) return rc;
      }
      RkEpi epi = ins_rk_stage_terms(rk->A.data(), ns, i, dt, rk->ku.data(), rk->force, vbasis ? RK_V_BASIS : RK_K_BASIS, corr_in, RK_FORCE_DIAG_FIRST);
      epi.ustart = (i == 0) ? nullptr : u;
      epi.ustar = out;
// ... 156 lines not shown
```

Before: 6775 M cell-updates/s.

## Fuse the Poisson x-direction forward FFT into the RK stage kernel epilogue

The fused momentum/RK stage kernel now runs a 256-point radix-4 complex FFT along x in LDS on the divergence it computes, treating two y-rows as one complex signal. It separates them into two real-input spectra and writes the x-spectrum straight into the Poisson solver's phat buffer. The spectral solve then skips its own x-forward pass. This removes a full write and re-read of the right-hand side and one FFT kernel launch per stage. In exchange the stage kernel gains LDS buffers, wavefront syncs and two extra pipeline barrier iterations, which may lower occupancy or lengthen the stage kernel.

```diff
diff --git a/include/ins_hip.h b/include/ins_hip.h
--- a/include/ins_hip.h
+++ b/include/ins_hip.h
@@ -115,6 +115,9 @@
 int ins_dbg_stage_rhs_used(const ins_rk_t* rk, int64_t* launches);
 int ins_dbg_stage_rhs(ins_rk_t* rk, double visc, const double* u_in, const double* pI, const double* ustart, const double* kterm, double coef_k,
                       double self_in, double coef_self, double* ustar, double* rhs, int32_t* used, void* stream);
+int ins_dbg_stage_xfwd_used(const ins_rk_t* rk, int64_t* launches);
+int ins_dbg_stage_xfwd(ins_rk_t* rk, double visc, const double* u_in, const double* pI, const double* ustart, const double* kterm, double coef_k,
+                       double self_in, double coef_self, double* ustar, double* spec, int32_t* used, void* stream);
 int ins_dbg_stage_carry_used(const ins_rk_t* rk, int64_t* launches);
 int ins_rk_pressure(const ins_rk_t* rk, double** p);
 int ins_rk_stage_force(const ins_rk_t* rk, int i, double** ku);
diff --git a/incompressiblenavierstokes.jl_amd/_lib.py b/incompressiblenavierstokes.jl_amd/_lib.py
--- a/incompressiblenavierstokes.jl_amd/_lib.py
+++ b/incompressiblenavierstokes.jl_amd/_lib.py
@@ -123,6 +123,8 @@
     "ins_dbg_stage_rhs_used": (C.c_int, [vp, C.POINTER(C.c_int64)]),
     "ins_dbg_stage_carry_used": (C.c_int, [vp, C.POINTER(C.c_int64)]),
     "ins_dbg_stage_rhs": (C.c_int, [vp, C.c_double, vp, vp, vp, vp, C.c_double, C.c_double, C.c_double, vp, vp, C.POINTER(C.c_int32), vp]),
+    "ins_dbg_stage_xfwd_used": (C.c_int, [vp, C.POINTER(C.c_int64)]),
+    "ins_dbg_stage_xfwd": (C.c_int, [vp, C.c_double, vp, vp, vp, vp, C.c_double, C.c_double, C.c_double, vp, vp, C.POINTER(C.c_int32), vp]),
     "ins_rk_pressure": (C.c_int, [vp, C.POINTER(vp)]),
     "ins_rk_stage_force": (C.c_int, [vp, C.c_int, C.POINTER(vp)]),
     "ins_rk_set_temperature": (C.c_int, [vp, vp]),
diff --git a/incompressiblenavierstokes.jl_amd/csrc/ins_flux64.hip b/incompressiblenavierstokes.jl_amd/csrc/ins_flux64.hip
--- a/incompressiblenavierstokes.jl_amd/csrc/ins_flux64.hip
+++ b/incompressiblenavierstokes.jl_amd/csrc/ins_flux64.hip
@@ -24,8 +24,29 @@
   T vm1;
 };
 
-template <typename T, int R, int XW, bool FUSE, int CORR, bool SKEL = false, int NW = 4, bool EXTRA = false, bool RHS = false, bool CARRY = false>
+struct Xc {
+  double x, y;
+};
+__device__ __forceinline__ Xc xc_mul(Xc a, Xc b) { return Xc{a.x * b.x - a.y * b.y, a.x * b.y + a.y * b.x}; }
+__device__ __forceinline__ Xc xc_bfly(Xc a0, Xc a1, Xc a2, Xc a3, int m) {
+  const bool odd = m & 1, neg = m & 2;
+  const double s2 = odd ? -1.0 : 1.0;
+  const Xc p{a0.x + s2 * a2.x, a0.y + s2 * a2.y}, q0{a1.x + s2 * a3.x, a1.y + s2 * a3.y};
+  Xc q = odd ? Xc{q0.y, -q0.x} : q0;
+  const double s1 = neg ? -1.0 : 1.0;
+  return Xc{p.x + s1 * q.x, p.y + s1 * q.y};
+}
+__device__ __forceinline__ int xf_swz(int i) { return (i & ~15) | ((i + ((i >> 4) & 3) + 4 * ((i >> 6) & 3)) & 15); }
+__device__ __forceinline__ int xf_pos(int s) { return ((s & 3) << 6) | (((s >> 2) & 3) << 4) | (((s >> 4) & 3) << 2) | ((s >> 6) & 3); }
+__device__ __forceinline__ void xf_wave_sync() {
+  __builtin_amdgcn_fence(__ATOMIC_RELEASE, "wavefront", "local");
+  __builtin_amdgcn_wave_barrier();
+  __builtin_amdgcn_fence(__ATOMIC_ACQUIRE, "wavefront", "local");
+}
+
+template <typename T, int R, int XW, bool FUSE, int CORR, bool SKEL = false, int NW = 4, bool EXTRA = false, bool RHS = false, bool CARRY = false, bool XF = false>
 __global__ __launch_bounds__(64 * NW, NW == 16 ? 4 : 2) void k_flux64(FluxArgs a) {
+  static_assert(!XF || (RHS && CORR == 1 && sizeof(T) == 8 && R == 2 && XW == 4 && (NW == 4 || NW == 8)), "x-forward transform in the stage kernel: 256-wide rows, fp64");
   static_assert(!RHS || (FUSE && CORR <= 1 && !SKEL && !EXTRA), "right-hand side in the stage kernel: fused epilogue, periodic box, no extra terms");
   static_assert(!CARRY || (FUSE && CORR == 1 && !SKEL && !EXTRA && NW <= 8 && sizeof(T) == 8), "carried combination: the fp64 periodic correcting stage kernel");
   constexpr unsigned EB = (unsigned)sizeof(T);
@@ -46,6 +67,10 @@
   }
   __shared__ T rhs_lds_s[RHS ? 2 * NW * R : 1];
   T* const rhs_lds = rhs_lds_s;
+  constexpr int XSLOT = (NW / 4) * 256;
+  __shared__ __align__(16) Xc xf_x1[XF ? 2 * XSLOT : 1];
+  __shared__ __align__(16) Xc xf_x2[XF ? 2 * XSLOT : 1];
+  __shared__ __align__(16) Xc xf_tw[XF ? 6 * 64 : 1];
   const int lane = threadIdx.x;
   const int wave = __builtin_amdgcn_readfirstlane(threadIdx.y);
   const int wx = wave % XW, wy = wave / XW;
@@ -58,7 +83,7 @@
   const int kw0 = RHS ? k0 - 1 : k0;
   if (x0 >= n0 || jb0 >= n1) {
     if (a.bar || RHS)
-      for (int k = kw0; k < k1; ++k) __builtin_amdgcn_s_barrier();
+      for (int k = kw0; k < k1 + (XF ? 2 : 0); ++k) __builtin_amdgcn_s_barrier();
     return;
   }
   const long long sz = (long long)N0 * N1;
@@ -285,6 +310,70 @@
         st3(o, co, rowb, s0 + (T)a.epi.coef_self * fu, s1 + (T)a.epi.coef_self * fv, s2 + (T)a.epi.coef_self * fw);
       }
       if (!FUSE || a.epi.write_k) st3(a_F + pk, co, rowb, fu, fv, fw);
+    }
+  };
+
+  const int xf_row = wy * 256;
+  if constexpr (XF) {
+    const Xc* twg = static_cast<const Xc*>((const void*)a.epi.spec_tw);
+    auto pw = [](Xc w1, int m) {
+      const Xc w2 = xc_mul(w1, w1), w3 = xc_mul(w2, w1);
+      return m == 0 ? Xc{1.0, 0.0} : (m == 1 ? w1 : (m == 2 ? w2 : w3));
+    };
+    xf_tw[wx * 64 + lane] = pw(twg[lane], wx);
+    xf_tw[256 + lane] = pw(twg[4 * (lane & 15)], lane >> 4);
+    xf_tw[320 + lane] = pw(twg[16 * (lane & 3)], (lane >> 2) & 3);
+  }
+  auto xf_step = [&](int k, T z0, T z1) {
+    if constexpr (XF) {
+      int ln = lane;
+      asm volatile("" : "+v"(ln));
+      if (k >= k0 && k < k1) xf_x1[(k & 1) * XSLOT + xf_row + 64 * wx + ln] = Xc{z0, z1};
+      if (k - 1 >= k0 && k - 1 < k1) {
+        const Xc* x = xf_x1 + ((k - 1) & 1) * XSLOT + xf_row;
+        Xc y = xc_bfly(x[ln], x[ln + 64], x[ln + 128], x[ln + 192], wx);
+        if (wx) y = xc_mul(y, xf_tw[wx * 64 + ln]);
+        Xc* zb = xf_x2 + ((k - 1) & 1) * XSLOT + xf_row + 64 * wx;
+        zb[ln] = y;
+        xf_wave_sync();
+        {
+          const Xc* e = zb + (ln & 15);
+          y = xc_bfly(e[0], e[16], e[32], e[48], ln >> 4);
+          y = xc_mul(y, xf_tw[256 + ln]);
+          zb[ln] = y;
+        }
+        xf_wave_sync();
+        {
+          const Xc* e = zb + (ln & ~12);
+          y = xc_bfly(e[0], e[4], e[8], e[12], (ln >> 2) & 3);
+          y = xc_mul(y, xf_tw[320 + ln]);
+          zb[ln] = y;
+        }
+        xf_wave_sync();
+        {
+          const Xc* e = zb + (ln & ~3);
+          y = xc_bfly(e[0], e[1], e[2], e[3], ln & 3);
+          zb[xf_swz(64 * wx + ln) - 64 * wx] = y;
+        }
+      }
+      if (k - 2 >= k0 && k - 2 < k1) {
+        const Xc* zr = xf_x2 + (k & 1) * XSLOT + xf_row;
+        const int s = (64 * wx + ln) & 127;
+        const bool rowb = wx >= 2;
+        const unsigned kxs = (unsigned)a.epi.spec_kxs;
+        const rsrc_t rs = plane_rsrc(static_cast<double*>((void*)a.epi.spec_out) + 2LL * (k - 3) * kxs * n1, kxs * (unsigned)n1 * 16u);
+        const unsigned soff = (unsigned)(jb0 + (rowb ? 1 : 0)) * kxs * 16u;
+        auto sep_store = [&](int sk, int sm) {
+          const Xc zk = zr[xf_swz(xf_pos(sk))], zm = zr[xf_swz(xf_pos(sm))];
+          const Xc av{0.5 * (zk.x + zm.x), 0.5 * (zk.y - zm.y)}, bv{0.5 * (zk.y + zm.y), -0.5 * (zk.x - zm.x)};
+          const Xc o = rowb ? bv : av;
+          v4u v;
+          v.x = (unsigned)__double2loint(o.x), v.y = (unsigned)__double2hiint(o.x), v.z = (unsigned)__double2loint(o.y), v.w = (unsigned)__double2hiint(o.y);
+          __builtin_amdgcn_raw_buffer_store_b128(v, rs, (unsigned)sk * 16u, soff, 0);
+        };
+        sep_store(s, (256 - s) & 255);
+        if (s == 0) sep_store(128, 128);
+      }
     }
   };
 
@@ -481,6 +570,7 @@
       T* ro = static_cast<T*>((void*)a.epi.rhs_out) + (long long)(k - 1) * n0 * n1;
       const rsrc_t rr_ = plane_rsrc(ro, qbytes);
       const T om = (T)a.om;
+      T zz[R];
 #pragma unroll
       for (int r = 0; r < R; ++r) {
         const T ul = rhs_lds[((k & 1) * NW + lw) * R + r];
@@ -488,8 +578,10 @@
         d += (us_u[r] - prev_h(us_u[r], ul)) * (T)a.rdiv[0];
         d += dvs[r] * (T)a.rdiv[1];
         d += dws[r] * (T)a.rdiv[2];
-        if (st && xout && jb0 + r < n1) stb(rr_, (unsigned)min(ci, n0 - 1) * EB, (unsigned)(min(jb0 + r, n1 - 1) * n0) * EB, d * om);
-      }
+        zz[r] = d * om;
+        if (!XF && st && xout && jb0 + r < n1) stb(rr_, (unsigned)min(ci, n0 - 1) * EB, (unsigned)(min(jb0 + r, n1 - 1) * n0) * EB, zz[r]);
+      }
+      if constexpr (XF) xf_step(k, zz[0], zz[1]);
     }
     if constexpr (TMK) {
       if (tm) {
@@ -571,6 +663,14 @@
       body(P0, P1, TE0, TE1, k, min(k + 2, k1), k >= k0);
       if (++k >= k1) break;
     }
+    if constexpr (XF) {
+      for (int kd = k1; kd < k1 + 2; ++kd) {
+        __builtin_amdgcn_fence(__ATOMIC_RELEASE, "workgroup", "local");
+        __builtin_amdgcn_s_barrier();
+        __builtin_amdgcn_fence(__ATOMIC_ACQUIRE, "workgroup", "local");
+        xf_step(kd, (T)0, (T)0);
+      }
+    }
   }
 }
 
@@ -662,7 +762,7 @@
   return launch_range<T, R, XW, FUSE, NW>(G, a, corr_mode, s);
 }
 
-template <int R, int XW, int NW, int CORR, bool CARRY = false>
+template <int R, int XW, int NW, int CORR, bool CARRY = false, bool XF = false>
 int launch_rhs(const ins_grid* G, FluxArgs& a, hipStream_t s) {
   const GridDev& g = G->g;
   a.ntx = 1;
@@ -672,7 +772,7 @@
   a.kB = 0;
   a.ntz = cdiv(a.k_hi - a.k_lo, a.zc);
   const unsigned nb = (unsigned)(8LL * ((a.nty + 7) / 8) * a.ntz);
-  hipLaunchKernelGGL((k_flux64<double, R, XW, true, CORR, false, NW, false, true, CARRY>), dim3(nb), dim3(64, NW, 1), 0, s, a);
+  hipLaunchKernelGGL((k_flux64<double, R, XW, true, CORR, false, NW, false, true, CARRY, XF>), dim3(nb), dim3(64, NW, 1), 0, s, a);
   INS_LAUNCH_CHECK();
   return INS_OK;
 }
@@ -757,6 +857,13 @@
   return t.rows == 2 && ((t.xw == 3 && t.nw == 6) || ((t.xw == 2 || t.xw == 4) && (t.nw == 4 || t.nw == 8)));
 }
 
+bool ins_flux64_stage_xfwd_supported(const ins_grid* G, int corr_mode) {
+  if (ins_opt(OPT_INS_DISABLE_STAGE_XFWD) || corr_mode != 1 || !ins_flux64_stage_rhs_supported(G, corr_mode)) return false;
+  if (G->g.N[0] - 2 != 256 || (G->g.N[1] & 1)) return false;
+  const TileShape t = tile_shape(G, corr_mode, false, false, true);
+  return t.rows == 2 && t.xw == 4 && (t.nw == 4 || t.nw == 8);
+}
+
 bool ins_flux64_stage_carry_supported(const ins_grid* G) {
   if (ins_opt(OPT_INS_DISABLE_STAGE_CARRY) || !ins_flux64_supported(G) || g_skel) return false;
   if (ins_flux128_supported(G, nullptr, 1, false)) return false;
@@ -786,7 +893,8 @@
     a.epi.tstage = nullptr;
   }
   const bool ext = epi && (epi->extra || epi->gtemp || epi->wout || epi->tstage);
-  const bool want_rhs = epi && epi->rhs_out;
+  const bool want_spec = epi && epi->spec_out;
+  const bool want_rhs = epi && (epi->rhs_out || want_spec);
   const TileShape ts = tile_shape(G, corr_mode, sizeof(T) == 4, ext, want_rhs);
   const int xw = ts.xw, rows = ts.rows, nw = ts.nw, zc = ts.zc;
   constexpr bool F32 = sizeof(T) == 4;
@@ -832,6 +940,11 @@
       ins_set_error("stage kernel asked for the Poisson right-hand side while u* overwrites one of its inputs");
       return INS_ERR_INVALID;
     }
+    if (want_spec && (epi->rhs_out || F32 || part != 0 || !ins_flux64_stage_xfwd_supported(G, corr_mode) || !epi->spec_tw || epi->spec_kxs < 129 ||
+                      (const void*)epi->spec_out == (const void*)pI)) {
+      ins_set_error("stage kernel asked for the x-spectrum of the Poisson right-hand side on a box, tile shape or buffer it does not write it for");
+      return INS_ERR_UNSUPPORTED;
+    }
     if constexpr (!F32) {
       if (part == 0 && ins_flux64_stage_rhs_supported(G, corr_mode)) {
         a.rdiv[0] = 1.0 / G->desc.dx[0][1];
@@ -839,6 +952,10 @@
         a.rdiv[2] = 1.0 / G->desc.dx[2][1];
         a.om = G->desc.dx[0][1] * G->desc.dx[1][1] * G->desc.dx[2][1];
         if (corr_mode == 0) return launch_rhs<4, 2, 4, 0>(G, a, s);
+        if (want_spec) {
+          if (carry) return nw == 8 ? launch_rhs<2, 4, 8, 1, true, true>(G, a, s) : launch_rhs<2, 4, 4, 1, true, true>(G, a, s);
+          return nw == 8 ? launch_rhs<2, 4, 8, 1, false, true>(G, a, s) : launch_rhs<2, 4, 4, 1, false, true>(G, a, s);
+        }
         if (carry) {
           if (xw == 3) return launch_rhs<2, 3, 6, 1, true>(G, a, s);
           if (xw == 4) return nw == 8 ? launch_rhs<2, 4, 8, 1, true>(G, a, s) : launch_rhs<2, 4, 4, 1, true>(G, a, s);
diff --git a/incompressiblenavierstokes.jl_amd/csrc/ins_internal.h b/incompressiblenavierstokes.jl_amd/csrc/ins_internal.h
--- a/incompressiblenavierstokes.jl_amd/csrc/ins_internal.h
+++ b/incompressiblenavierstokes.jl_amd/csrc/ins_internal.h
@@ -107,6 +107,7 @@
   X(INS_DISABLE_FDM_FOLDFUSE)    \
   X(INS_DISABLE_INKERNEL_CORR)   \
   X(INS_DISABLE_STAGE_RHS)       \
+  X(INS_DISABLE_STAGE_XFWD)      \
   X(INS_DISABLE_STAGE_CARRY)     \
   X(INS_RK_KEEP_K)               \
   X(INS_DISABLE_EXT_FUSED)       \
@@ -229,6 +230,7 @@
   size_t work_bytes = 0;
   hipStream_t plan_stream = nullptr;
   int kxs = 0;
+  bool spec_pending = false;
   double* tw = nullptr;
   double* tw_x = nullptr;
   double* tw_y = nullptr;
@@ -264,6 +266,7 @@
   ins_rk_ext* ext = nullptr;
   long long stage_carry_launches = 0;
   long long stage_rhs_launches = 0;
+  long long stage_xfwd_launches = 0;
   bool profiling = false;
   std::vector<hipEvent_t> prof_events;
   void* step_graph = nullptr;
@@ -287,6 +290,9 @@
   double* carry_out;
   double ca[3];
   double* rhs_out;
+  double* spec_out;
+  const double* spec_tw;
+  int spec_kxs;
   const double* extra;
   const double* gtemp;
   double ga2;
@@ -344,10 +350,13 @@
 int ins_k_project_fdm_solve_only(const ins_grid* G, ins_poisson* ps, const double* u, double* p, hipStream_t s);
 int ins_k_project_periodic_fused_2d(const ins_grid* G, ins_poisson* ps, double* u, double* p, bool keep_p, hipStream_t s);
 bool ins_poisson_own2d(const ins_poisson* ps);
-int ins_k_project_periodic_solve_only(const ins_grid* G, ins_poisson* ps, const double* u, hipStream_t s, const double* rhs = nullptr);
+int ins_k_project_periodic_solve_only(const ins_grid* G, ins_poisson* ps, const double* u, hipStream_t s, const double* rhs = nullptr, bool from_spec = false);
 bool ins_flux64_stage_rhs_supported(const ins_grid* G, int corr_mode);
+bool ins_flux64_stage_xfwd_supported(const ins_grid* G, int corr_mode);
 bool ins_flux64_stage_carry_supported(const ins_grid* G);
 double* ins_poisson_stage_rhs(ins_poisson* ps);
+double* ins_poisson_stage_spec(ins_poisson* ps, const void* pI_in, const double** tw, int* kxs);
+bool ins_poisson_stage_spec_possible(const ins_poisson* ps);
 int ins_k_poisson_solve(ins_poisson* ps, double* p, hipStream_t s);
 bool ins_fast3d_supported(const ins_grid* G);
 
@@ -389,6 +398,7 @@
   XSRC_DIV_WALLS = 4,
   XSRC_DIV_U32 = 5,
   XSRC_FIELD = 6,
+  XSRC_SPEC = 7,
 };
 bool ins_zsolve_supported(int nz);
 bool ins_ownfft_supported(const int np[3]);
diff --git a/incompressiblenavierstokes.jl_amd/csrc/ins_poisson.hip b/incompressiblenavierstokes.jl_amd/csrc/ins_poisson.hip
--- a/incompressiblenavierstokes.jl_amd/csrc/ins_poisson.hip
+++ b/incompressiblenavierstokes.jl_amd/csrc/ins_poisson.hip
@@ -842,14 +842,24 @@
   return (ps->route == ROUTE_OWN_XY && src != XSRC_PI && src != XSRC_DIV) ? ROUTE_OWN_LDS : ps->route;
 }
 
+static bool route_starts_with_xfwd(SpectralRoute r) { return r == ROUTE_OWN_LDS || r == ROUTE_OWN_LINE3 || r == ROUTE_OWN_YZ; }
 static int spectral_transform(ins_poisson* ps, hipStream_t s, const double* u = nullptr, int src = XSRC_DIV, const double* rhs = nullptr) {
   const GridDev& g = ps->grid->g;
   const int n0 = ps->np[0], n1 = ps->np[1], n2 = ps->np[2], kxn = ps->kmax[0], kxs = ps->kxs;
   double* ph = reinterpret_cast<double*>(ps->phat);
   if (rhs) u = nullptr;
   const double* f = u ? u : (rhs ? rhs : ps->pI);
-  if (!u) src = XSRC_PI;
-  const SpectralRoute route = route_for_source(ps, src);
+  const bool from_spec = src == XSRC_SPEC;
+  if (!u && !from_spec) src = XSRC_PI;
+  const SpectralRoute route = route_for_source(ps, from_spec ? XSRC_PI : src);
+  if (from_spec) {
+    INS_REQUIRE(ps->spec_pending && !u && !rhs, "spectral solve from the stored x-spectrum: no stage kernel was handed phat since the last solve");
+    INS_REQUIRE(route_starts_with_xfwd(route) && g.D == 3 && (const void*)ps->phat != (const void*)ps->pI, "spectral solve from the stored x-spectrum: route without a separate x pass");
+  } else {
+    INS_REQUIRE(!ps->spec_pending, "spectral solve: phat holds a stage kernel's x-spectrum that no solve has read");
+  }
+  ps->spec_pending = false;
+  auto xfwd = [&]() { return from_spec ? (int)INS_OK : ins_k_ownfft_xfwd(ps->grid, f, src, ph, n0, n1, n2, ps->tw_x, s, kxs); };
   INS_REQUIRE(!rhs || (own_route(route) && g.D == 3), "spectral solve: a right-hand side outside pI needs an own-FFT 3-D route");
   INS_REQUIRE(ins_spectral_ky_order(route) == ps->ky_order, "spectral solve: the route for this source leaves ky in another order than the solver's symbol");
   const double inv_n = 1.0 / ((double)n0 * n1 * n2);
@@ -884,7 +894,7 @@
       if ((rc = zpass())) return rc;
       return ins_k_ownfft_xy(nullptr, nullptr, XSRC_PI, ph, ps->pI, n0, n1, n2, ps->tw_x, ps->tw_y, true, s, kxs);
     case ROUTE_OWN_YZ: {
-      if ((rc = ins_k_ownfft_xfwd(ps->grid, f, src, ph, n0, n1, n2, ps->tw_x, s, kxs))) return rc;
+      if ((rc = xfwd())) return rc;
       const ins_grid* G = ps->grid;
       const double c = G->h[0] * G->h[1] / G->h[2];
       if ((rc = ins_k_ownfft_yz_solve(ph, kxn, n1, n2, kxs, ps->yz_P, ps->ahat[0], ps->ahat[1], c, -1.0 / ((double)n0 * n1), ps->tw_y, ps->yz_scratch, s))) return rc;
@@ -893,7 +903,7 @@
     case ROUTE_OWN_LDS:
     case ROUTE_OWN_LINE3: {
       const auto ypass = route == ROUTE_OWN_LINE3 ? ins_k_line3_y : ins_k_ownfft_y;
-      if ((rc = ins_k_ownfft_xfwd(ps->grid, f, src, ph, n0, n1, n2, ps->tw_x, s, kxs))) return rc;
+      if ((rc = xfwd())) return rc;
       if ((rc = ypass(ph, kxn, n1, n2, ps->tw_y, false, s, kxs))) return rc;
       if ((rc = zpass())) return rc;
       if ((rc = ypass(ph, kxn, n1, n2, ps->tw_y, true, s, kxs))) return rc;
@@ -1333,8 +1343,9 @@
   return ins_k_applypressure(G, u, p, s);
 }
 
-int ins_k_project_periodic_solve_only(const ins_grid* G, ins_poisson* ps, const double* u, hipStream_t s, const double* rhs) {
+int ins_k_project_periodic_solve_only(const ins_grid* G, ins_poisson* ps, const double* u, hipStream_t s, const double* rhs, bool from_spec) {
   const GridDev& g = G->g;
+  if (from_spec) return spectral_transform(ps, s, nullptr, XSRC_SPEC);
   if (own_route(ps->route)) return spectral_transform(ps, s, u, XSRC_DIV, rhs);
   INS_REQUIRE(!rhs, "a right-hand side written by the stage kernel needs an own-FFT route");
   dim3 block(64, 4, 1), grid(cdiv(ps->np[0], 64), cdiv(ps->np[1], 4), ps->np[2]);
@@ -1343,11 +1354,11 @@
   return spectral_transform(ps, s);
 }
 
-int ins_k_project_periodic_fused(const ins_grid* G, ins_poisson* ps, double* u, double* p, bool keep_p, hipStream_t s, double* uout, const double* rhs) {
+int ins_k_project_periodic_fused(const ins_grid* G, ins_poisson* ps, double* u, double* p, bool keep_p, hipStream_t s, double* uout, const double* rhs, bool from_spec) {
   const GridDev& g = G->g;
   dim3 block(64, 4, 1), grid(cdiv(ps->np[0], 64), cdiv(ps->np[1], 4), ps->np[2]);
   double* dst = uout ? uout : u;
-  int rc = ins_k_project_periodic_solve_only(G, ps, u, s, rhs);
+  int rc = ins_k_project_periodic_solve_only(G, ps, u, s, rhs, from_spec);
   if (rc) return rc;
   if (keep_p)
     hipLaunchKernelGGL(k_grad_ghost3<true>, grid, block, 0, s, g, dst, p, ps->pI, ps->np[0], ps->np[1], ps->np[2], (const double*)u);
@@ -1383,6 +1394,16 @@
     ps->rhs = nullptr;
   }
   return ps->rhs;
+}
+bool ins_poisson_stage_spec_possible(const ins_poisson* ps) {
+  return ins_k_spectral_own3d(ps) && route_starts_with_xfwd(ps->route) && ps->phat && ps->tw_x && ps->kxs >= ps->kmax[0];
+}
+double* ins_poisson_stage_spec(ins_poisson* ps, const void* pI_in, const double** tw, int* kxs) {
+  if (!ins_poisson_stage_spec_possible(ps) || (const void*)ps->phat == pI_in || (const void*)ps->phat == (const void*)ps->pI) return nullptr;
+  ps->spec_pending = true;
+  *tw = ps->tw_x;
+  *kxs = ps->kxs;
+  return reinterpret_cast<double*>(ps->phat);
 }
 int ins_k_spectral_solve_from_u32(ins_poisson* ps, const float* u32, hipStream_t s) {
   return spectral_transform(ps, s, reinterpret_cast<const double*>(u32), XSRC_DIV_U32);
diff --git a/incompressiblenavierstokes.jl_amd/csrc/ins_rk.hip b/incompressiblenavierstokes.jl_amd/csrc/ins_rk.hip
--- a/incompressiblenavierstokes.jl_amd/csrc/ins_rk.hip
+++ b/incompressiblenavierstokes.jl_amd/csrc/ins_rk.hip
@@ -10,7 +10,7 @@
 
 int ins_k_momentum_rk_fused(const ins_grid* G, double visc, const double* u_in, double* k_out, const RkEpi& epi, hipStream_t s);
 int ins_k_project_periodic_fused(const ins_grid* G, ins_poisson* ps, double* u, double* p, bool keep_p, hipStream_t s, double* uout = nullptr,
-                                 const double* rhs = nullptr);
+                                 const double* rhs = nullptr, bool from_spec = false);
 
 int ins_k_momentum(const ins_grid* G, double visc, const double* u, double* F, hipStream_t s) {
   if (ins_fast3d_supported(G)) return ins_k_momentum_fast3d(G, visc, u, F, s);
@@ -159,6 +159,12 @@
   return INS_OK;
 }
 
+extern "C" int ins_dbg_stage_xfwd_used(const ins_rk_t* rk, int64_t* launches) {
+  INS_REQUIRE(rk && launches, "null argument");
+  *launches = (int64_t)rk->stage_xfwd_launches;
+  return INS_OK;
+}
+
 extern "C" int ins_dbg_stage_carry_used(const ins_rk_t* rk, int64_t* launches) {
   INS_REQUIRE(rk && launches, "null argument");
   *launches = (int64_t)rk->stage_carry_launches;
@@ -206,6 +212,36 @@
   int rc = pI ? ins_k_momentum_rk_fused_corr(G, visc, u_in, pI, rk->ku[0], epi, s) : ins_k_momentum_rk_fused(G, visc, u_in, rk->ku[0], epi, s);
   if (rc) return rc;
   if (*used) INS_HIP_TRY(hipMemcpyAsync(rhs, epi.rhs_out, (size_t)rk->ps->np[0] * rk->ps->np[1] * rk->ps->np[2] * sizeof(double), hipMemcpyDeviceToDevice, s));
+  return INS_OK;
+}
+
+extern "C" int ins_dbg_stage_xfwd(ins_rk_t* rk, double visc, const double* u_in, const double* pI, const double* ustart, const double* kterm, double coef_k,
+                                  double self_in, double coef_self, double* ustar, double* spec, int32_t* used, void* stream) {
+  INS_REQUIRE(rk && u_in && ustar && spec && used, "null argument");
+  const ins_grid* G = rk->grid;
+  hipStream_t s = as_stream(stream);
+  RkEpi epi;
+  memset(&epi, 0, sizeof(epi));
+  epi.ustart = ustart;
+  epi.ustar = ustar;
+  epi.coef_self = coef_self;
+  if (ustart) {
+    epi.self_in = self_in;
+    epi.c0m1 = -self_in;
+  }
+  if (kterm) {
+    epi.coef[0] = coef_k;
+    epi.k[0] = kterm;
+    epi.n = 1;
+  }
+  *used = 0;
+  INS_REQUIRE(!ins_stage_out_aliases_input(epi, u_in), "ustar must be an array of its own");
+  if (!pI || !ins_flux64_stage_xfwd_supported(G, 1) || !(epi.spec_out = ins_poisson_stage_spec(rk->ps, pI, &epi.spec_tw, &epi.spec_kxs))) return INS_OK;
+  rk->ps->spec_pending = false;
+  *used = 1;
+  int rc = ins_k_momentum_rk_fused_corr(G, visc, u_in, pI, rk->ku[0], epi, s);
+  if (rc) return rc;
+  INS_HIP_TRY(hipMemcpyAsync(spec, epi.spec_out, (size_t)epi.spec_kxs * rk->ps->np[1] * rk->ps->np[2] * 2 * sizeof(double), hipMemcpyDeviceToDevice, s));
   return INS_OK;
 }
 
@@ -327,14 +363,21 @@
     }
     if (i == 0 && raw_in) epi.ustart_out = rk->ustart;
     const bool corr = inkernel && (i > 0 || raw_in);
-    if (!in_place && ins_flux64_stage_rhs_supported(G, corr ? 1 : 0) && (epi.rhs_out = ins_poisson_stage_rhs(rk->ps)))
-      ++rk->stage_rhs_launches;
+    if (!in_place && ins_flux64_stage_rhs_supported(G, corr ? 1 : 0)) {
+      if (ins_flux64_stage_xfwd_supported(G, corr ? 1 : 0) && ins_poisson_stage_spec_possible(rk->ps) &&
+          (epi.spec_out = ins_poisson_stage_spec(rk->ps, corr ? rk->ps->pI : nullptr, &epi.spec_tw, &epi.spec_kxs))) {
+        ++rk->stage_rhs_launches;
+        ++rk->stage_xfwd_launches;
+      } else if ((epi.rhs_out = ins_poisson_stage_rhs(rk->ps))) {
+        ++rk->stage_rhs_launches;
+      }
+    }
     rc = timed_stage(rk, s, [&] {
       return corr ? ins_k_momentum_rk_fused_corr(G, visc, in, rk->ps->pI, rk->ku[i], epi, s) : ins_k_momentum_rk_fused(G, visc, in, rk->ku[i], epi, s);
     });
     if (rc) return rc;
-    rc = (inkernel && (i < ns - 1 || raw_out)) ? ins_k_project_periodic_solve_only(G, rk->ps, out, s, epi.rhs_out)
-                                               : ins_k_project_periodic_fused(G, rk->ps, out, rk->p, i == ns - 1, s, nullptr, epi.rhs_out);
+    rc = (inkernel && (i < ns - 1 || raw_out)) ? ins_k_project_periodic_solve_only(G, rk->ps, out, s, epi.rhs_out, epi.spec_out != nullptr)
+                                               : ins_k_project_periodic_fused(G, rk->ps, out, rk->p, i == ns - 1, s, nullptr, epi.rhs_out, epi.spec_out != nullptr);
     if (rc) return rc;
     in = out;
   }
diff --git a/incompressiblenavierstokes.jl_amd/csrc/ins_rk_ext.hip b/incompressiblenavierstokes.jl_amd/csrc/ins_rk_ext.hip
--- a/incompressiblenavierstokes.jl_amd/csrc/ins_rk_ext.hip
+++ b/incompressiblenavierstokes.jl_amd/csrc/ins_rk_ext.hip
@@ -8,7 +8,7 @@
 int ins_k_momentum_fast3d_opts(const ins_grid* G, double visc, const double* u, double* F, bool zero_shell, hipStream_t s);
 int ins_k_momentum_rk_fused(const ins_grid* G, double visc, const double* u_in, double* k_out, const RkEpi& epi, hipStream_t s);
 int ins_k_project_periodic_fused(const ins_grid* G, ins_poisson* ps, double* u, double* p, bool keep_p, hipStream_t s, double* uout = nullptr,
-                                 const double* rhs = nullptr);
+                                 const double* rhs = nullptr, bool from_spec = false);
 int ins_k_project(const ins_grid* G, ins_poisson* ps, double* u, double* p, hipStream_t s);
 bool ins_flux64_supported(const ins_grid* G);
 int ins_k_temp_stage(const ins_grid* G, double a4, double coef, const double* u, const double* temp, const double* w, const double* tempstart, int n,
```

Measured after the change: 6894 M cell-updates/s, median of 6. 1.8% higher.
